# antbern/slamrs

Measured on NVIDIA B200. Metric: particle_beam_updates_per_s, higher is better.
Workload: dtype f32 geometry, f64 weights, u16x2 hit-counter cells

## Files before the change

slamrs_b200/csrc/api.cu:

```cuda
#include "../../include/slamrs_gpu.h"

#include <cuda_runtime.h>
#include <math.h>
#include <stdio.h>
#include <stdlib.h>
#include <string.h>
#include <unistd.h>

#include <algorithm>
#include <new>
#include <string>
#include <vector>

#include "comm.h"
#include "kernels.cuh"

using namespace slamrs;

struct slamrs_gpu_handle {
    slamrs_gpu_config cfg{};
    int device = 0;
    int num_sms = 148;
    cudaStream_t stream = nullptr;
    cudaStream_t side_stream = nullptr;
// ... 288 lines not shown
    if (h->h_scan_stage) cudaFreeHost(h->h_scan_stage);
    h->d_angle = h->d_dist = nullptr; h->d_valid = nullptr; h->h_scan_stage = nullptr; h->beam_cap = 0;
    h->scan_upload_pending = false;
    const uint32_t cap = (n + 255u) & ~255u;
    unsigned char* base = nullptr;
    CU_TRY(h, cudaMalloc(&base, 9u * (size_t)cap));
    h->d_angle = reinterpret_cast<float*>(base);
    h->d_dist = reinterpret_cast<float*>(base + 4u * (size_t)cap);
    h->d_valid = base + 8u * (size_t)cap;
    CU_TRY(h, cudaMallocHost(&h->h_scan_stage, 9u * (size_t)cap));
    if (!h->ev_scan_uploaded) CU_TRY(h, cudaEventCreateWithFlags(&h->ev_scan_uploaded, cudaEventDisableTiming));
    h->beam_cap = cap;
    return SLAMRS_OK;
}

constexpr uint32_t PROF_RING = 64;
constexpr uint32_t PROF_MARKS = SLAMRS_PHASE_COUNT + 1;

int prof_flush(slamrs_gpu_handle* h) {
    if (h->prof_recorded == 0) return SLAMRS_OK;
    CU_TRY(h, cudaStreamSynchronize(h->stream));
    for (uint32_t r = 0; r < h->prof_recorded; ++r) {
        for (int p = 0; p < SLAMRS_PHASE_COUNT; ++p) {
            float ms = 0.f;
            CU_TRY(h, cudaEventElapsedTime(&ms, h->prof_events[r * PROF_MARKS + p], h->prof_events[r * PROF_MARKS + p + 1]));
            h->prof_ms[p] += ms;
        }
    }
    h->prof_steps += h->prof_recorded;
    h->prof_recorded = 0;
    return SLAMRS_OK;
}

#define PROF_MARK(h, m)                                                                                   \
    do {                                                                                                  \
        if ((h)->profiling) CU_TRY(h, cudaEventRecord((h)->prof_events[(h)->prof_recorded * PROF_MARKS + (m)], (h)->stream)); \
    } while (0)

int materialize_copies(slamrs_gpu_handle* h, bool grouped) {
    launch_copy_boxed(h->stream, h->d_mat_items, grouped ? h->d_mat_leaders : nullptr, &h->d_counters->n_mat,
                      &h->d_counters->n_mat_leaders, h->n_local, h->d_jobs, h->geom, h->d_counters, h->num_sms, !grouped);
    launch_commit_boxes(h->stream, h->d_mat_items, &h->d_counters->n_mat, h->n_local, h->geom, true, h->d_counters, nullptr);
    h->launches += 3;
    return SLAMRS_OK;
}
int unshare_all(slamrs_gpu_handle* h) {
    if (!h->defer) return SLAMRS_OK;
    launch_materialize_list(h->stream, nullptr, h->n_total, h->first, h->n_local, h->d_slot[h->cur], h->d_alias, h->d_cells,
                            h->cells_per_grid, h->d_meta, h->d_bands, h->n_bands, h->d_mat_items, h->d_mat_leaders,
                            h->d_mat_roots, h->d_counters);
    h->launches++;
    int rc = materialize_copies(h, true);
    if (rc) return rc;
    CU_TRY(h, cudaStreamSynchronize(h->stream));
    h->counters_fresh = false;
    h->mirror_by_step = false;
    return SLAMRS_OK;
}

int step_barrier(slamrs_gpu_handle* h) {
    if (h->p2p_exchange) {
        launch_peer_barrier(h->stream, h->d_peer_flags, h->d_flags, h->rank, h->world, ++h->barrier_epoch,
                            h->barrier_timeout_ns, h->d_counters);
        h->launches++;
        return SLAMRS_OK;
    }
    std::string err;
    if (comm_barrier(h->comm, h->d_barrier, h->stream, &err)) return fail(h, SLAMRS_E_NCCL, err);
    return SLAMRS_OK;
}

int fetch_counters(slamrs_gpu_handle* h) {
    if (h->counters_fresh) return SLAMRS_OK;
    if (!h->mirror_by_step) {
        launch_publish_counters(h->stream, h->d_counters, h->h_counters);
        h->launches++;
    }
    CU_TRY(h, cudaStreamSynchronize(h->stream));
    CU_TRY(h, cudaGetLastError());
    h->counters_fresh = true;
    return SLAMRS_OK;
}

int loc_step_async(slamrs_gpu_handle* h, const OdomModel& od, bool caller) {
    cudaStream_t s = h->stream;
    if (h->profiling && h->prof_recorded == PROF_RING) {
        int prc = prof_flush(h);
        if (prc) return prc;
    }
    const int cur = h->cur, nxt = cur ^ 1;
    const ScanDevice scan = h->scan_external ? ScanDevice{h->ext_angle, h->ext_dist, h->ext_valid, h->n_beams, nullptr}
                                             : ScanDevice{h->d_angle, h->d_dist, h->d_valid, h->n_beams, nullptr};
    PROF_MARK(h, 0);
    launch_loc_step(s, h->geom, od, scan, h->d_pose[cur], h->d_results, h->n_total, caller ? h->d_z : nullptr, h->cfg.seed,
                    h->step, h->d_loc_terms, h->loc_outside, h->d_carry, h->d_counters);
    PROF_MARK(h, 1);
    PROF_MARK(h, 2);
    launch_weights(s, h->d_results, h->n_total, h->d_wnorm, h->d_cum, h->d_fold, (double)h->cfg.resample_threshold, h->d_counters);
    launch_resample_indices(s, h->d_results, h->d_cum, h->n_total, caller ? h->d_u : nullptr, h->cfg.seed, h->step, h->d_idx,
                            h->d_pose[nxt], 0, h->n_total, false, nullptr,
                            RayLists{nullptr, nullptr, nullptr, nullptr, nullptr, nullptr, 0u, 0u}, h->d_wnorm, h->d_carry,
                            h->d_counters);
    h->launches += 3;
    for (uint32_t m = 3; m < PROF_MARKS; ++m) PROF_MARK(h, m);
    if (h->profiling) h->prof_recorded++;
    CU_TRY(h, cudaGetLastError());
    h->cur = nxt;
    h->step++;
    h->counters_fresh = false;
    h->mirror_by_step = false;
    return SLAMRS_OK;
}

}

namespace {
template <typename T>
struct DevBuf {
    T* p = nullptr;
    cudaError_t alloc(size_t n) { return cudaMalloc(&p, sizeof(T) * (n ? n : 1)); }
    ~DevBuf() { cudaFree(p); }
};
int debug_device(int device) {
    int n = 0;
    if (cudaGetDeviceCount(&n) != cudaSuccess || n == 0) { cudaGetLastError(); return SLAMRS_E_NO_DEVICE; }
    if (device >= n) return SLAMRS_E_INVALID_ARG;
    return SLAMRS_OK;
}
#define DBG_CU(expr)                                                                     \
    do {                                                                                 \
        cudaError_t _e = (expr);                                                         \
        if (_e != cudaSuccess) return fail(nullptr, SLAMRS_E_CUDA, std::string(#expr) + ": " + cudaGetErrorString(_e)); \
    } while (0)
}

extern "C" {

int slamrs_gpu_grid_cells(float extent, float resolution, uint32_t* out_cells) {
    if (!out_cells) return SLAMRS_E_INVALID_ARG;
    const float c = ceilf(extent / resolution);
    if (!(c == c) || c <= 0.0f) { *out_cells = 0; return SLAMRS_OK; }
    if (c >= 4294967296.0f) return SLAMRS_E_INVALID_ARG;
    *out_cells = (uint32_t)c;
    return SLAMRS_OK;
}

int slamrs_gpu_nccl_unique_id(uint8_t out[SLAMRS_NCCL_ID_BYTES]) {
    if (!out) return SLAMRS_E_INVALID_ARG;
    std::string err;
    if (comm_unique_id(out, &err)) return fail(nullptr, SLAMRS_E_NCCL, err);
    return SLAMRS_OK;
}

int slamrs_gpu_create(const slamrs_gpu_config* cfg, slamrs_gpu_handle** out) {
    if (!cfg || !out) return fail(nullptr, SLAMRS_E_INVALID_ARG, "null config or output pointer");
    *out = nullptr;
    if (cfg->struct_size != sizeof(slamrs_gpu_config) || cfg->abi_version != SLAMRS_GPU_ABI_VERSION)
        return fail(nullptr, SLAMRS_E_INVALID_ARG, "slamrs_gpu_config size/ABI version mismatch");
    if (cfg->n_particles == 0)
        return fail(nullptr, SLAMRS_E_INVALID_ARG, "Must have at least one particle");
    if (cfg->world_size > PEER_MAX_WORLD) return fail(nullptr, SLAMRS_E_INVALID_ARG, "world_size above 64");
    if (cfg->world_size > 32u && (cfg->flags & SLAMRS_FLAG_NCCL_EXCHANGE) == 0)
        return fail(nullptr, SLAMRS_E_INVALID_ARG, "world_size above 32 needs SLAMRS_FLAG_NCCL_EXCHANGE (the peer-store exchange serves 32 GPUs)");
    if (cfg->world_size == 0 || cfg->rank >= cfg->world_size || cfg->n_particles % cfg->world_size != 0)
        return fail(nullptr, SLAMRS_E_INVALID_ARG, "bad rank/world_size or n_particles not divisible by world_size");
    if (cfg->n_particles > 0x7fffffffull) return fail(nullptr, SLAMRS_E_INVALID_ARG, "too many particles");
    if (cfg->grid_w == 0 || cfg->grid_w != cfg->grid_h)
        return fail(nullptr, SLAMRS_E_INVALID_ARG,
                    "grid must be square and non-empty (the reference index row*size.y+column aliases otherwise)");
    if ((uint64_t)cfg->grid_w * cfg->grid_h > 0x7fffffffull) return fail(nullptr, SLAMRS_E_INVALID_ARG, "grid too large");
    if (!(cfg->resolution > 0.0f)) return fail(nullptr, SLAMRS_E_INVALID_ARG, "resolution must be positive");
    if (cfg->rng_mode > SLAMRS_RNG_CALLER) return fail(nullptr, SLAMRS_E_INVALID_ARG, "unknown rng_mode");
    if (!(cfg->resample_threshold >= 0.0f && cfg->resample_threshold <= 1.0f))
        return fail(nullptr, SLAMRS_E_INVALID_ARG, "resample_threshold must be 0 (always resample) or in (0, 1]");
    if (cfg->slot_cells != 0 && (cfg->slot_cells < 256u || (cfg->slot_cells & (cfg->slot_cells - 1u)) != 0u))
        return fail(nullptr, SLAMRS_E_INVALID_ARG, "slot_cells must be 0 (whole grid) or a power of two >= 256");

    int n_dev = 0;
    if (cudaGetDeviceCount(&n_dev) != cudaSuccess || n_dev == 0) {
        cudaGetLastError();
        return fail(nullptr, SLAMRS_E_NO_DEVICE, "no CUDA device visible; this library has no CPU fallback");
    }
    int device = cfg->device;
    if (device < 0) cudaGetDevice(&device);
    if (device >= n_dev) return fail(nullptr, SLAMRS_E_INVALID_ARG, "device ordinal out of range");

    slamrs_gpu_handle* h = new (std::nothrow) slamrs_gpu_handle();
    if (!h) return fail(nullptr, SLAMRS_E_OUT_OF_MEMORY, "host allocation failed");
    h->cfg = *cfg;
    h->device = device;
    h->world = cfg->world_size;
    h->rank = cfg->rank;
    h->n_total = (uint32_t)cfg->n_particles;
    h->n_local = h->n_total / h->world;
    h->first = h->rank * h->n_local;
    h->n_cells = cfg->grid_w * cfg->grid_h;
    h->geom = make_map_geom(cfg->pos_x, cfg->pos_y, cfg->resolution, cfg->grid_w, cfg->grid_h, cfg->slot_cells);
    h->cells_per_grid = ((size_t)h->geom.pw * h->geom.ph + 31u) & ~(size_t)31u;

#define CREATE_TRY(expr)                                  \
    do {                                                  \
        int _rc = (expr);                                 \
        if (_rc != SLAMRS_OK) {                           \
            g_create_error = h->last_error;               \
            free_all(h);                                  \
            return _rc;                                   \
        }                                                 \
    } while (0)
#define CREATE_CU(expr)                                                                                   \
    do {                                                                                                  \
        cudaError_t _e = (expr);                                                                          \
        if (_e != cudaSuccess) {                                                                          \
            const int _code = (_e == cudaErrorMemoryAllocation) ? SLAMRS_E_OUT_OF_MEMORY : SLAMRS_E_CUDA; \
            g_create_error = std::string(#expr) + ": " + cudaGetErrorString(_e);                          \
            cudaGetLastError();                                                                           \
            free_all(h);                                                                                  \
            return _code;                                                                                 \
        }                                                                                                 \
    } while (0)

    DeviceGuard guard(device);
    cudaDeviceProp prop;
    CREATE_CU(cudaGetDeviceProperties(&prop, device));
    h->num_sms = prop.multiProcessorCount;
    if (prop.major < 10) {
        g_create_error = "this library is built for sm_100a (B200) only";
        free_all(h);
        return SLAMRS_E_NO_DEVICE;
    }
    CREATE_CU(cudaStreamCreateWithFlags(&h->stream, cudaStreamNonBlocking));
    CREATE_CU(cudaStreamCreateWithFlags(&h->side_stream, cudaStreamNonBlocking));
    CREATE_CU(cudaEventCreateWithFlags(&h->ev_indices, cudaEventDisableTiming));
    CREATE_CU(cudaEventCreateWithFlags(&h->ev_plan, cudaEventDisableTiming));
    CREATE_CU(cudaEventCreateWithFlags(&h->ev_sort, cudaEventDisableTiming));
    CREATE_CU(cudaMalloc(&h->d_order, sizeof(uint16_t) * SORT_MAX_BEAMS));
    CREATE_CU(cudaMalloc(&h->d_valid_list, sizeof(float2) * 65536));
    CREATE_CU(cudaMalloc(&h->d_n_valid, sizeof(uint32_t)));
    CREATE_CU(configure_kernels());

    const size_t grid_bytes = h->cells_per_grid * sizeof(uint32_t);
    if (h->world > 1) {
        uint32_t spare = cfg->spare_slots;
        if (spare == 0) {
            size_t free_b = 0, total_b = 0;
            CREATE_CU(cudaMemGetInfo(&free_b, &total_b));
            const size_t reserve = (size_t)2 << 30;
            const size_t live = (size_t)h->n_local * grid_bytes;
            size_t room = free_b > live + reserve ? (free_b - live - reserve) / grid_bytes : 0;
            spare = (uint32_t)(room < h->n_local ? room : h->n_local);
        }
        h->n_spare = spare;
    }
    h->n_slots = h->n_local + h->n_spare;

    h->off_results = (sizeof(SlotMeta) * 2 * (size_t)h->n_local + 255) & ~(size_t)255;
    h->off_flags = (h->off_results + 2 * sizeof(ParticleResult) * (size_t)h->n_total + 255) & ~(size_t)255;
    h->n_bands = bands_per_slot(h->geom);
    h->off_bands = (h->off_flags + sizeof(unsigned long long) * 2 * PEER_MAX_WORLD + 255) & ~(size_t)255;
    h->off_counters = (h->off_bands + sizeof(uint32_t) * 2 * (size_t)h->n_local * h->n_bands + 255) & ~(size_t)255;
    h->pool_header = (h->off_counters + sizeof(StepCounters) + 4095) & ~(size_t)4095;
    CREATE_CU(cudaMalloc(&h->d_pool, h->pool_header + (size_t)h->n_slots * grid_bytes));
    h->d_meta = (SlotMeta*)h->d_pool;
    h->d_cells = (uint32_t*)((char*)h->d_pool + h->pool_header);
    h->d_results_base = (ParticleResult*)((char*)h->d_pool + h->off_results);
    h->d_results = h->d_results_base;
    h->d_flags = (unsigned long long*)((char*)h->d_pool + h->off_flags);
    h->d_bands = (uint32_t*)((char*)h->d_pool + h->off_bands);
    h->d_counters = (StepCounters*)((char*)h->d_pool + h->off_counters);
    h->peer_counters.assign(h->world, nullptr);
    h->peer_counters[h->rank] = h->d_counters;
    h->p2p_exchange = h->world > 1 && (cfg->flags & SLAMRS_FLAG_NCCL_EXCHANGE) == 0;
    CREATE_CU(cudaMemsetAsync(h->d_pool, 0, h->pool_header + (size_t)h->n_slots * grid_bytes, h->stream));
    h->boxed_copy = (cfg->flags & SLAMRS_FLAG_FULL_GRID_COPY) == 0 && cfg->grid_w % 8u == 0u && h->geom.pw % 8u == 0u;
    h->defer = h->boxed_copy && (cfg->flags & SLAMRS_FLAG_EAGER_COPY) == 0;
    for (int i = 0; i < 2; ++i) {
        CREATE_CU(cudaMalloc(&h->d_slot[i], sizeof(int32_t) * h->n_local));
        CREATE_CU(cudaMalloc(&h->d_pose[i], sizeof(float) * 3 * h->n_local));
        CREATE_CU(cudaMemsetAsync(h->d_pose[i], 0, sizeof(float) * 3 * h->n_local, h->stream));
    }
    CREATE_CU(cudaMalloc(&h->d_wnorm, sizeof(double) * h->n_total));
    CREATE_CU(cudaMalloc(&h->d_cum, sizeof(double) * h->n_total));
    CREATE_CU(cudaMalloc(&h->d_idx, sizeof(uint32_t) * h->n_total));
    CREATE_CU(cudaMalloc(&h->d_fold, sizeof(double) * weights_scratch_doubles()));
    if (cfg->resample_threshold > 0.0f) CREATE_CU(cudaMalloc(&h->d_carry, sizeof(double) * h->n_total));
    CREATE_CU(cudaMemsetAsync(h->d_wnorm, 0, sizeof(double) * h->n_total, h->stream));
    CREATE_CU(cudaMemsetAsync(h->d_idx, 0, sizeof(uint32_t) * h->n_total, h->stream));
    if (cfg->rng_mode == SLAMRS_RNG_CALLER) {
        CREATE_CU(cudaMalloc(&h->d_z, sizeof(double) * 2 * h->n_total));
        CREATE_CU(cudaMalloc(&h->d_u, sizeof(double)));
    }
    CREATE_CU(cudaMalloc(&h->d_keep, sizeof(int32_t) * h->n_local));
    CREATE_CU(cudaMalloc(&h->d_need, sizeof(int32_t) * h->n_local));
    CREATE_CU(cudaMalloc(&h->d_free, sizeof(int32_t) * ((size_t)h->n_local + h->n_spare + 1)));
    CREATE_CU(cudaMalloc(&h->d_spare, sizeof(int32_t) * ((size_t)h->n_spare + 1)));
    CREATE_CU(cudaMalloc(&h->d_copies, sizeof(CopyItem) * h->n_local));
    CREATE_CU(cudaMalloc(&h->d_leaders, sizeof(uint32_t) * h->n_local));
    CREATE_CU(cudaMalloc(&h->d_jobs, copy_job_bytes() * h->n_local));
    CREATE_CU(cudaMalloc(&h->d_alias, sizeof(int32_t) * h->n_slots));
    CREATE_CU(cudaMalloc(&h->d_mat_items, sizeof(CopyItem) * h->n_local));
    CREATE_CU(cudaMalloc(&h->d_mat_leaders, sizeof(uint32_t) * h->n_local));
    CREATE_CU(cudaMalloc(&h->d_mat_roots, sizeof(uint32_t) * h->n_local));
    CREATE_CU(cudaMalloc(&h->d_alive, sizeof(uint32_t) * h->n_local));
    CREATE_CU(cudaMalloc(&h->d_ray_items, sizeof(RayItem) * 2 * (size_t)h->n_local));
    CREATE_CU(cudaMalloc(&h->d_readers, sizeof(uint32_t) * (2 * (size_t)h->n_slots + 2 * (size_t)h->n_local)));
    CREATE_CU(cudaMalloc(&h->d_ray_xchg, ray_half_xchg_bytes() * h->n_local));
    CREATE_CU(cudaMalloc(&h->d_ray_spill, sizeof(uint32_t) * ray_spill_scratch_words(h->num_sms)));
    CREATE_CU(cudaMallocHost(&h->h_counters, sizeof(StepCounters)));
    memset(h->h_counters, 0, sizeof(StepCounters));
    CREATE_CU(cudaMalloc(&h->d_export, sizeof(double) * h->n_cells));
    CREATE_CU(cudaStreamCreateWithFlags(&h->copy_stream, cudaStreamNonBlocking));
    for (int k = 0; k < 2; ++k) {
        CREATE_CU(cudaMalloc(&h->d_export_async[k], sizeof(double) * h->n_cells));
        CREATE_CU(cudaEventCreateWithFlags(&h->ev_exported[k], cudaEventDisableTiming));
        CREATE_CU(cudaEventCreateWithFlags(&h->ev_copied[k], cudaEventDisableTiming));
    }
    CREATE_CU(cudaMalloc(&h->d_term_table, sizeof(double) * LK_TABLE_NF * LK_TABLE_NO));
    launch_fill_term_table(h->stream, h->d_term_table);
    h->launches++;
    CREATE_CU(cudaMalloc(&h->d_history, sizeof(StepRecord) * STEP_HISTORY));
    CREATE_CU(cudaMemsetAsync(h->d_history, 0xff, sizeof(StepRecord) * STEP_HISTORY, h->stream));
    CREATE_CU(cudaMalloc(&h->d_barrier, sizeof(int)));
    CREATE_CU(cudaMemsetAsync(h->d_barrier, 0, sizeof(int), h->stream));
    launch_init_slots(h->stream, h->d_slot[0], h->n_local, h->d_spare, h->n_spare, h->d_counters, h->rank, h->d_meta, h->d_alias);
    h->launches++;
    CREATE_CU(cudaGetLastError());

    if (h->world > 1) {
        std::string err;
        h->comm = comm_create(cfg->nccl_id, (int)h->rank, (int)h->world, &err);
        if (!h->comm) {
            g_create_error = err;
            free_all(h);
            return SLAMRS_E_NCCL;
        }
        CREATE_TRY(setup_peers(h));
        if (const char* ev = getenv("SLAMRS_BARRIER_TIMEOUT_MS")) {
            const long long ms = atoll(ev);
            if (ms > 0) h->barrier_timeout_ns = (unsigned long long)ms * 1000000ull;
        }
        if (comm_barrier(h->comm, h->d_barrier, h->stream, &err)) {
            g_create_error = err;
            free_all(h);
            return SLAMRS_E_NCCL;
        }
    }
    CREATE_CU(cudaStreamSynchronize(h->stream));
    h->h_counters->est_slot = h->rank == 0 ? 0 : -1;
    h->h_counters->n_spare = h->n_spare;
#undef CREATE_TRY
#undef CREATE_CU
    *out = h;
    return SLAMRS_OK;
}

int slamrs_gpu_create_localizer(const slamrs_gpu_config* cfg, const slamrs_gpu_sensor_model* model,
                                const double* map_probability, slamrs_gpu_handle** out) {
    if (!out) return fail(nullptr, SLAMRS_E_INVALID_ARG, "null output pointer");
    *out = nullptr;
    if (!cfg) return fail(nullptr, SLAMRS_E_INVALID_ARG, "null config");
    if (!model) return fail(nullptr, SLAMRS_E_INVALID_ARG, "null sensor model");
    if (!map_probability) return fail(nullptr, SLAMRS_E_INVALID_ARG, "null map_probability");
    if (cfg->struct_size != sizeof(slamrs_gpu_config) || cfg->abi_version != SLAMRS_GPU_ABI_VERSION)
        return fail(nullptr, SLAMRS_E_INVALID_ARG, "slamrs_gpu_config size/ABI version mismatch");
    if (model->struct_size != sizeof(slamrs_gpu_sensor_model))
        return fail(nullptr, SLAMRS_E_INVALID_ARG, "slamrs_gpu_sensor_model struct_size mismatch");
    if (cfg->n_particles == 0) return fail(nullptr, SLAMRS_E_INVALID_ARG, "Must have at least one particle");
    if (cfg->n_particles > 0x7fffffffull) return fail(nullptr, SLAMRS_E_INVALID_ARG, "too many particles");
    if (cfg->world_size != 1 || cfg->rank != 0)
        return fail(nullptr, SLAMRS_E_INVALID_ARG, "world_size must be 1 and rank 0: a localizer runs on one GPU");
    if (cfg->flags != 0) return fail(nullptr, SLAMRS_E_INVALID_ARG, "flags must be 0 for a localizer");
    if (cfg->slot_cells != 0) return fail(nullptr, SLAMRS_E_INVALID_ARG, "slot_cells must be 0 for a localizer");
    if (cfg->spare_slots != 0) return fail(nullptr, SLAMRS_E_INVALID_ARG, "spare_slots must be 0 for a localizer");
    if (cfg->grid_w == 0 || cfg->grid_w != cfg->grid_h)
        return fail(nullptr, SLAMRS_E_INVALID_ARG, "grid_w and grid_h must be equal and non-zero (square grid)");
    if ((uint64_t)cfg->grid_w * cfg->grid_h > 0x7fffffffull) return fail(nullptr, SLAMRS_E_INVALID_ARG, "grid too large");
    if (!(cfg->resolution > 0.0f)) return fail(nullptr, SLAMRS_E_INVALID_ARG, "resolution must be positive");
    if (cfg->rng_mode > SLAMRS_RNG_CALLER) return fail(nullptr, SLAMRS_E_INVALID_ARG, "unknown rng_mode");
    if (!(cfg->resample_threshold >= 0.0f && cfg->resample_threshold <= 1.0f))
        return fail(nullptr, SLAMRS_E_INVALID_ARG, "resample_threshold must be 0 (always resample) or in (0, 1]");
    if (model->kind > SLAMRS_SENSOR_LIKELIHOOD_FIELD) return fail(nullptr, SLAMRS_E_INVALID_ARG, "unknown sensor model kind");
    const bool field = model->kind == SLAMRS_SENSOR_LIKELIHOOD_FIELD;
    if (field) {
        if (!(model->sigma > 0.0f) || !isfinite(model->sigma))
            return fail(nullptr, SLAMRS_E_INVALID_ARG, "sigma must be a positive finite number of metres");
        if (!(model->z_rand > 0.0f && model->z_rand < 1.0f))
            return fail(nullptr, SLAMRS_E_INVALID_ARG, "z_rand must lie in (0, 1)");
        if (!(model->occupied_above >= 0.5f && model->occupied_above < 1.0f))
            return fail(nullptr, SLAMRS_E_INVALID_ARG, "occupied_above must lie in [0.5, 1)");
    }
    const size_t n_cells = (size_t)cfg->grid_w * cfg->grid_h;
    for (size_t i = 0; i < n_cells; ++i)
        if (!(map_probability[i] >= 0.0 && map_probability[i] <= 1.0))
            return fail(nullptr, SLAMRS_E_INVALID_ARG,
                        "map_probability[" + std::to_string(i) + "] is NaN or outside [0, 1]");

    int n_dev = 0;
    if (cudaGetDeviceCount(&n_dev) != cudaSuccess || n_dev == 0) {
        cudaGetLastError();
        return fail(nullptr, SLAMRS_E_NO_DEVICE, "no CUDA device visible; this library has no CPU fallback");
    }
    int device = cfg->device;
    if (device < 0) cudaGetDevice(&device);
    if (device >= n_dev) return fail(nullptr, SLAMRS_E_INVALID_ARG, "device ordinal out of range");

    slamrs_gpu_handle* h = new (std::nothrow) slamrs_gpu_handle();
    if (!h) return fail(nullptr, SLAMRS_E_OUT_OF_MEMORY, "host allocation failed");
    h->cfg = *cfg;
    h->localizer = true;
    h->device = device;
    h->n_total = h->n_local = (uint32_t)cfg->n_particles;
    h->n_cells = (uint32_t)n_cells;
    h->geom = make_map_geom(cfg->pos_x, cfg->pos_y, cfg->resolution, cfg->grid_w, cfg->grid_h);
    h->loc_outside = field ? log((double)model->z_rand) : 0.0;

#define CREATE_CU(expr)                                                                                   \
    do {                                                                                                  \
        cudaError_t _e = (expr);                                                                          \
        if (_e != cudaSuccess) {                                                                          \
            const int _code = (_e == cudaErrorMemoryAllocation) ? SLAMRS_E_OUT_OF_MEMORY : SLAMRS_E_CUDA; \
            g_create_error = std::string(#expr) + ": " + cudaGetErrorString(_e);                          \
            cudaGetLastError();                                                                           \
            cudaFree(scratch);                                                                            \
            free_all(h);                                                                                  \
            return _code;                                                                                 \
        }                                                                                                 \
    } while (0)

    uint32_t* scratch = nullptr;
    DeviceGuard guard(device);
    cudaDeviceProp prop;
    CREATE_CU(cudaGetDeviceProperties(&prop, device));
    h->num_sms = prop.multiProcessorCount;
    if (prop.major < 10) {
        g_create_error = "this library is built for sm_100a (B200) only";
        free_all(h);
        return SLAMRS_E_NO_DEVICE;
    }
    CREATE_CU(cudaStreamCreateWithFlags(&h->stream, cudaStreamNonBlocking));
    CREATE_CU(configure_kernels());
    h->off_counters = (sizeof(ParticleResult) * (size_t)h->n_total + 255) & ~(size_t)255;
    const size_t pool_bytes = h->off_counters + sizeof(StepCounters);
    CREATE_CU(cudaMalloc(&h->d_pool, pool_bytes));
    CREATE_CU(cudaMemsetAsync(h->d_pool, 0, pool_bytes, h->stream));
    h->d_results_base = h->d_results = (ParticleResult*)h->d_pool;
    h->d_counters = (StepCounters*)((char*)h->d_pool + h->off_counters);
    for (int i = 0; i < 2; ++i) {
        CREATE_CU(cudaMalloc(&h->d_pose[i], sizeof(float) * 3 * h->n_total));
        CREATE_CU(cudaMemsetAsync(h->d_pose[i], 0, sizeof(float) * 3 * h->n_total, h->stream));
    }
    CREATE_CU(cudaMalloc(&h->d_wnorm, sizeof(double) * h->n_total));
    CREATE_CU(cudaMalloc(&h->d_cum, sizeof(double) * h->n_total));
    CREATE_CU(cudaMalloc(&h->d_idx, sizeof(uint32_t) * h->n_total));
    CREATE_CU(cudaMalloc(&h->d_fold, sizeof(double) * weights_scratch_doubles()));
    if (cfg->resample_threshold > 0.0f) CREATE_CU(cudaMalloc(&h->d_carry, sizeof(double) * h->n_total));
    CREATE_CU(cudaMemsetAsync(h->d_wnorm, 0, sizeof(double) * h->n_total, h->stream));
    CREATE_CU(cudaMemsetAsync(h->d_idx, 0, sizeof(uint32_t) * h->n_total, h->stream));
    if (cfg->rng_mode == SLAMRS_RNG_CALLER) {
        CREATE_CU(cudaMalloc(&h->d_z, sizeof(double) * 2 * h->n_total));
        CREATE_CU(cudaMalloc(&h->d_u, sizeof(double)));
    }
    CREATE_CU(cudaMallocHost(&h->h_counters, sizeof(StepCounters)));
    memset(h->h_counters, 0, sizeof(StepCounters));
    CREATE_CU(cudaMalloc(&h->d_export, sizeof(double) * n_cells));
    CREATE_CU(cudaMemcpyAsync(h->d_export, map_probability, sizeof(double) * n_cells, cudaMemcpyHostToDevice, h->stream));
    CREATE_CU(cudaMalloc(&h->d_loc_terms, sizeof(double) * n_cells));
    if (field) CREATE_CU(cudaMalloc(&scratch, sizeof(uint32_t) * n_cells));
    CREATE_CU(launch_loc_terms(h->stream, h->d_export, cfg->grid_w, field ? 1 : 0, model->sigma, model->z_rand,
                               model->occupied_above, cfg->resolution, scratch, h->d_loc_terms));
    h->launches += field ? 2 : 1;
    CREATE_CU(cudaStreamSynchronize(h->stream));
    cudaFree(scratch);
#undef CREATE_CU
    *out = h;
    return SLAMRS_OK;
}

int slamrs_gpu_get_sensor_terms(slamrs_gpu_handle* h, double* out_cells) {
    if (!h || !out_cells) return SLAMRS_E_INVALID_ARG;
    if (!h->localizer) return fail(h, SLAMRS_E_INVALID_ARG, "a SLAM handle has no sensor-term table (only a localizer has one)");
    DeviceGuard g(h->device);
    CU_TRY(h, cudaMemcpyAsync(out_cells, h->d_loc_terms, sizeof(double) * h->n_cells, cudaMemcpyDeviceToHost, h->stream));
    CU_TRY(h, cudaStreamSynchronize(h->stream));
    return SLAMRS_OK;
}

int slamrs_gpu_set_scan_match(slamrs_gpu_handle* h, const slamrs_gpu_scan_match* m) {
    if (!h) return SLAMRS_E_INVALID_ARG;
    if (h->localizer) return fail(h, SLAMRS_E_INVALID_ARG, "a localizer does not scan-match");
    if (!m) {
        h->match_on = false;
        return SLAMRS_OK;
    }
    if (m->struct_size != sizeof(slamrs_gpu_scan_match))
        return fail(h, SLAMRS_E_INVALID_ARG, "slamrs_gpu_scan_match struct_size mismatch");
    if (m->radius > 2u) return fail(h, SLAMRS_E_INVALID_ARG, "scan match radius must be 0, 1 or 2 cells");
    if (!(m->step_xy > 0.0f) || !isfinite(m->step_xy))
        return fail(h, SLAMRS_E_INVALID_ARG, "scan match step_xy must be a positive finite number of metres");
    if (!(m->step_theta > 0.0f) || !isfinite(m->step_theta))
        return fail(h, SLAMRS_E_INVALID_ARG, "scan match step_theta must be a positive finite number of radians");
    if (m->levels < 1u || m->levels > 8u) return fail(h, SLAMRS_E_INVALID_ARG, "scan match levels must lie in 1..8");
    if (m->max_moves < 1u || m->max_moves > 1024u)
        return fail(h, SLAMRS_E_INVALID_ARG, "scan match max_moves must lie in 1..1024");
    if (!h->d_match_stats) {
        DeviceGuard g(h->device);
        CU_TRY(h, cudaMalloc(&h->d_match_stats, sizeof(uint2) * h->n_local));
    }
    h->match = ScanMatchParams{m->radius, m->step_xy, m->step_theta, m->levels, m->max_moves};
    h->match_on = true;
    return SLAMRS_OK;
}

int slamrs_gpu_get_scan_match_stats(slamrs_gpu_handle* h, uint64_t out[4]) {
    if (!h || !out) return SLAMRS_E_INVALID_ARG;
    out[0] = out[1] = out[2] = out[3] = 0;
    if (!h->match_last_step) return SLAMRS_OK;
    DeviceGuard g(h->device);
    std::vector<uint2> per(h->n_local);
    CU_TRY(h, cudaMemcpyAsync(per.data(), h->d_match_stats, sizeof(uint2) * h->n_local, cudaMemcpyDeviceToHost, h->stream));
    CU_TRY(h, cudaStreamSynchronize(h->stream));
    for (const uint2& v : per) {
        out[0] += v.x > 0u;
        out[1] += v.x;
        out[2] += v.y;
        out[3] += v.x == h->match_last_max_moves;
    }
    return SLAMRS_OK;
}

void slamrs_gpu_destroy(slamrs_gpu_handle* h) {
    if (h && getenv("SLAMRS_RAY_TRACE_PRINT")) {
        unsigned long long tr[18];
        DeviceGuard g(h->device);
        cudaStreamSynchronize(h->stream);
        if (ray_trace(tr) == 0) {
            fprintf(stderr, "ray trace: items fused %llu in-place %llu; cycles pop %llu setup %llu walk %llu fused_total %llu wait %llu inplace_wb %llu\n",
                    tr[16], tr[17], tr[0], tr[1], tr[2], tr[3], tr[4], tr[5]);
            fprintf(stderr, "ray trace raw:");
            for (int k = 0; k < 18; ++k) fprintf(stderr, " [%d]%llu", k, tr[k]);
            fprintf(stderr, "\n");
        }
    }
    free_all(h);
}

int slamrs_gpu_upload_scan(slamrs_gpu_handle* h, const float* angle, const float* dist, const uint8_t* valid,
                           uint32_t n_beams) {
    if (!h) return SLAMRS_E_INVALID_ARG;
    if (n_beams > 0 && (!angle || !dist || !valid)) return fail(h, SLAMRS_E_INVALID_ARG, "null scan array");
    if (n_beams > 65535u) return fail(h, SLAMRS_E_INVALID_ARG, "at most 65535 beams per scan");
    DeviceGuard g(h->device);
    int rc = ensure_beam_capacity(h, n_beams ? n_beams : 1);
    if (rc) return rc;
    if (n_beams) {
        if (h->scan_upload_pending) CU_TRY(h, cudaEventSynchronize(h->ev_scan_uploaded));
        const size_t cap = h->beam_cap;
        memcpy(h->h_scan_stage, angle, sizeof(float) * n_beams);
        memcpy(h->h_scan_stage + 4u * cap, dist, sizeof(float) * n_beams);
        memcpy(h->h_scan_stage + 8u * cap, valid, n_beams);
        CU_TRY(h, cudaMemcpyAsync(h->d_angle, h->h_scan_stage, 8u * cap + n_beams, cudaMemcpyHostToDevice, h->stream));
        CU_TRY(h, cudaEventRecord(h->ev_scan_uploaded, h->stream));
        h->scan_upload_pending = true;
    }
    h->n_beams = n_beams;
    h->scan_external = false;
    h->order_valid = false;
    float maxd = 0.0f;
    for (uint32_t i = 0; i < n_beams; ++i) {
        const float d = fabsf(dist[i]);
        if (!isfinite(d)) { maxd = INFINITY; break; }
        if (d > maxd) maxd = d;
    }
    const float cells = ceilf(maxd / h->geom.res);
    h->radius_cells = (cells < 4096.0f ? (int)cells : 4096) + 6;
    return SLAMRS_OK;
}

int slamrs_gpu_set_scan_device(slamrs_gpu_handle* h, const float* angle_device, const float* dist_device,
                               const uint8_t* valid_device, uint32_t n_beams, float max_dist) {
    if (!h) return SLAMRS_E_INVALID_ARG;
    if (n_beams > 0 && (!angle_device || !dist_device || !valid_device)) return fail(h, SLAMRS_E_INVALID_ARG, "null scan array");
    if (n_beams > 65535u) return fail(h, SLAMRS_E_INVALID_ARG, "at most 65535 beams per scan");
    h->ext_angle = angle_device; h->ext_dist = dist_device; h->ext_valid = valid_device;
    h->n_beams = n_beams;
    h->scan_external = true;
    h->order_valid = false;
    const float cells = max_dist > 0.0f ? ceilf(max_dist / h->geom.res) : INFINITY;
    h->radius_cells = ((cells == cells && cells < 4096.0f) ? (int)cells : 4096) + 6;
    return SLAMRS_OK;
}

int slamrs_gpu_step_async(slamrs_gpu_handle* h, float dist_left, float dist_right, float wheel_dist,
                          const double* z_draws, const double* resample_u) {
    if (!h) return SLAMRS_E_INVALID_ARG;
    const bool caller = h->cfg.rng_mode == SLAMRS_RNG_CALLER;
    if (caller && (!z_draws || !resample_u))
        return fail(h, SLAMRS_E_INVALID_ARG, "rng_mode CALLER needs z_draws and resample_u");
    DeviceGuard g(h->device);
    cudaStream_t s = h->stream;
    const OdomModel od = odometry_new(dist_left, dist_right, wheel_dist);
    if (caller) {
        CU_TRY(h, cudaMemcpyAsync(h->d_z, z_draws, sizeof(double) * 2 * h->n_total, cudaMemcpyHostToDevice, s));
        CU_TRY(h, cudaMemcpyAsync(h->d_u, resample_u, sizeof(double), cudaMemcpyHostToDevice, s));
    }
    if (h->localizer) return loc_step_async(h, od, caller);
    const bool sorted = h->n_beams > 32u && h->n_beams <= SORT_MAX_BEAMS;
    const ScanDevice scan = h->scan_external
                                ? ScanDevice{h->ext_angle, h->ext_dist, h->ext_valid, h->n_beams, sorted ? h->d_order : nullptr}
                                : ScanDevice{h->d_angle, h->d_dist, h->d_valid, h->n_beams, sorted ? h->d_order : nullptr};
    if (sorted && !h->order_valid) {
        CU_TRY(h, cudaEventRecord(h->ev_indices, s));
        CU_TRY(h, cudaStreamWaitEvent(h->side_stream, h->ev_indices, 0));
        launch_sort_beams(h->side_stream, scan.dist, h->n_beams, h->d_order);
        CU_TRY(h, cudaEventRecord(h->ev_sort, h->side_stream));
        h->launches++;
        h->order_valid = true;
        h->order_pending = true;
    }
    if (h->profiling && h->prof_recorded == PROF_RING) {
        int prc = prof_flush(h);
        if (prc) return prc;
    }
    const int cur = h->cur, nxt = cur ^ 1;
    const size_t grid_bytes = h->cells_per_grid * sizeof(uint32_t);
    const bool all_particles = (h->cfg.flags & SLAMRS_FLAG_UPDATE_ALL_PARTICLES) != 0;
    const uint32_t res_off = (uint32_t)(h->step & 1ull) * h->n_total;
    h->d_results = h->d_results_base + res_off;

    const bool force_generic = (h->cfg.flags & SLAMRS_FLAG_GENERIC_RAY_KERNEL) != 0;
    const bool fuse = h->defer && !all_particles &&
                      ray_update_can_fuse(h->geom, h->n_beams, h->cells_per_grid, force_generic, h->radius_cells);
    const bool half_items = ray_update_can_fuse(h->geom, h->n_beams, h->cells_per_grid, force_generic, h->radius_cells);
    const bool flag_pulls = h->world > 1 && fuse && half_items && h->boxed_copy && h->p2p_exchange;
    const uint32_t pull_epoch = flag_pulls ? (uint32_t)(h->step + 1ull) : 0u;
    const size_t n_zero = half_items ? 2 * (size_t)h->n_slots + 2 * (size_t)h->n_local : 0;
    PROF_MARK(h, 0);
    launch_motion_likelihood(s, h->geom, od, scan, h->d_pose[cur], h->d_slot[cur], h->defer ? h->d_alias : nullptr, h->d_cells, h->d_meta, h->cells_per_grid,
                             h->d_results, h->first, h->n_local, caller ? h->d_z : nullptr, h->cfg.seed, h->step, h->d_term_table, h->d_valid_list, h->d_n_valid,
                             h->d_carry, h->d_counters, h->p2p_exchange ? h->d_peer_results : nullptr, res_off, h->rank, h->world,
                             h->d_readers, (uint32_t)n_zero, h->match_on ? &h->match : nullptr, h->d_match_stats);
    h->launches += h->match_on ? 3 : 2;
    h->match_last_step = h->match_on;
    h->match_last_max_moves = h->match.max_moves;
    PROF_MARK(h, 1);
    if (h->world > 1) {
        if (h->p2p_exchange) {
            int brc = step_barrier(h);
            if (brc) return brc;
        } else {
            std::string err;
            if (comm_all_gather(h->comm, h->d_results + h->first, h->d_results, sizeof(ParticleResult) * h->n_local, s, &err))
                return fail(h, SLAMRS_E_NCCL, err);
        }
    }
    PROF_MARK(h, 2);
    launch_weights(s, h->d_results, h->n_total, h->d_wnorm, h->d_cum, h->d_fold, (double)h->cfg.resample_threshold, h->d_counters);
    RayLists ray{nullptr, nullptr, nullptr, nullptr, nullptr, nullptr, 0u, 0u};
    if (fuse) ray = RayLists{h->d_ray_items, h->d_ray_items + h->n_local, h->d_slot[cur], h->d_alias, h->d_readers, h->d_meta,
                             h->n_local, flag_pulls ? 1u : 0u};
    launch_resample_indices(s, h->d_results, h->d_cum, h->n_total, caller ? h->d_u : nullptr, h->cfg.seed, h->step,
                            h->d_idx, h->d_pose[nxt], h->first, h->n_local, !all_particles, h->d_alive, ray, h->d_wnorm, h->d_carry,
                            h->d_counters);
    if (all_particles) {
        launch_mark_alive(s, h->d_idx, h->n_total, h->first, h->n_local, true, h->d_alive, h->d_counters);
        h->launches++;
    }
    if (h->defer && !fuse) {
        if (all_particles)
            launch_materialize_list(s, nullptr, h->n_total, h->first, h->n_local, h->d_slot[cur], h->d_alias, h->d_cells,
                                    h->cells_per_grid, h->d_meta, h->d_bands, h->n_bands, h->d_mat_items, h->d_mat_leaders,
                                    h->d_mat_roots, h->d_counters);
        else
            launch_materialize_alive(s, h->d_alive, h->n_local, h->d_slot[cur], h->d_alias, h->d_cells, h->cells_per_grid,
                                     h->d_meta, h->d_bands, h->n_bands, h->d_mat_items, h->d_counters);
        h->launches++;
    }
    CU_TRY(h, cudaEventRecord(h->ev_indices, s));
    CU_TRY(h, cudaStreamWaitEvent(h->side_stream, h->ev_indices, 0));
    PlanArgs pa{};
    pa.results = h->d_results;
    pa.idx = h->d_idx;
    pa.n_total = h->n_total; pa.n_local = h->n_local; pa.rank = h->rank; pa.world = h->world;
    pa.slot_old = h->d_slot[cur]; pa.slot_new = h->d_slot[nxt];
    pa.keep = h->d_keep; pa.need = h->d_need; pa.free_list = h->d_free; pa.spare_list = h->d_spare;
    pa.n_spare_cap = h->n_spare;
    pa.copies = h->d_copies; pa.leaders = h->d_leaders;
    pa.cells = h->d_cells; pa.cells_per_grid = h->cells_per_grid;
    pa.peer_cells = h->d_peer_cells;
    pa.meta = h->d_meta; pa.peer_meta = h->d_peer_meta;
    pa.bands = h->d_bands; pa.peer_bands = h->d_peer_bands; pa.n_bands = h->n_bands;
    pa.counters = h->d_counters;
    pa.history = h->d_history;
    pa.step = h->step;
    pa.staged = plan_can_stage(h->n_local, h->n_spare);
    pa.alias_of = h->d_alias; pa.defer = h->defer;
    launch_plan(h->side_stream, pa);
    h->launches += 3;
    if (flag_pulls) {
        launch_pull(h->side_stream, h->d_copies, h->d_leaders, &h->d_counters->n_copies, &h->d_counters->n_leaders,
                    h->n_local, h->geom, h->d_counters, h->num_sms, pull_epoch, h->barrier_timeout_ns, h->d_meta, h->d_readers,
                    h->d_readers + h->n_slots);
        h->launches++;
    }
    CU_TRY(h, cudaEventRecord(h->ev_plan, h->side_stream));
    PROF_MARK(h, 3);
    if (h->defer && !fuse) {
        int mrc = materialize_copies(h, all_particles);
        if (mrc) return mrc;
    }
    PROF_MARK(h, 4);
    if (h->order_pending) {
        CU_TRY(h, cudaStreamWaitEvent(s, h->ev_sort, 0));
        h->order_pending = false;
    }
    CU_TRY(h, launch_ray_update(s, h->geom, scan, h->d_results, h->first, h->n_local, h->d_alive,
                                fuse ? h->d_ray_items : nullptr, fuse ? h->d_ray_items + h->n_local : nullptr,
                                fuse ? h->d_readers : nullptr,
                                fuse ? h->d_readers + h->n_slots : nullptr, h->d_readers + 2 * (size_t)h->n_slots, h->d_ray_xchg,
                                h->d_ray_spill, h->d_slot[cur],
                                h->d_cells, h->d_meta, h->d_bands, h->cells_per_grid, h->radius_cells, h->d_counters, &h->window_cells,
                                force_generic, h->num_sms, h->d_readers + 2 * (size_t)h->n_slots + h->n_local, pull_epoch));
    h->launches++;
    PROF_MARK(h, 5);
    CU_TRY(h, cudaStreamWaitEvent(s, h->ev_plan, 0));
    if (h->world > 1 && !flag_pulls) {
        int brc = step_barrier(h);
        if (brc) return brc;
    }
    PROF_MARK(h, 6);
    if ((h->defer && h->world == 1) || flag_pulls) {
    } else if (h->boxed_copy) {
        launch_copy_boxed(s, h->d_copies, h->d_leaders, &h->d_counters->n_copies, &h->d_counters->n_leaders, h->n_local,
                          h->d_jobs, h->geom, h->d_counters, h->num_sms, h->defer);
        h->launches++;
    } else {
        launch_copy(s, h->d_copies, h->d_leaders, &h->d_counters->n_copies, &h->d_counters->n_leaders, h->cells_per_grid,
                    h->num_sms);
        launch_account_full_copy(s, &h->d_counters->n_copies, &h->d_counters->n_leaders, grid_bytes, h->d_counters);
        h->launches++;
    }
    if (!((h->defer && h->world == 1) || flag_pulls)) h->launches++;
    PROF_MARK(h, 7);
    launch_commit_boxes(s, h->d_copies, &h->d_counters->n_copies, (h->defer && h->world == 1) ? 1u : h->n_local, h->geom,
                        h->boxed_copy, h->d_counters, h->d_history + (h->step % STEP_HISTORY),
                        h->mirror_wanted ? h->h_counters : nullptr);
    h->launches++;
    if (h->profiling) h->prof_recorded++;
    CU_TRY(h, cudaGetLastError());
    h->cur = nxt;
    h->step++;
    h->counters_fresh = false;
    h->mirror_by_step = h->mirror_wanted;
    h->est_box_stale = false;
    return SLAMRS_OK;
}

int slamrs_gpu_sync(slamrs_gpu_handle* h) {
    if (!h) return SLAMRS_E_INVALID_ARG;
    DeviceGuard g(h->device);
    int rc = fetch_counters(h);
    if (rc) return rc;
    if (h->h_counters->barrier_timeout)
        return fail(h, SLAMRS_E_INTERNAL,
                    h->h_counters->barrier_timeout == 2ull
                        ? "a peer GPU's handle was destroyed (its step failed or its owner left); this handle can only be destroyed"
                        : "a peer GPU did not reach the step barrier within the time limit");
    if (h->h_counters->fuse_overflow)
        return fail(h, SLAMRS_E_INTERNAL, "fused ray update: more window-bypassing hits than its scratch holds");
    if (h->h_counters->window_overflow)
        return fail(h, SLAMRS_E_WINDOW,
                    "a particle's informed extent outgrew its windowed grid slot; raise slot_cells (the scan was not "
                    "integrated into that grid)");
    if (h->h_counters->staging_short)
        return fail(h, SLAMRS_E_STAGING,
                    "cross-GPU migration needed more free grid slots than available; raise spare_slots");
    return SLAMRS_OK;
}

int slamrs_gpu_update(slamrs_gpu_handle* h, const float* angle, const float* dist, const uint8_t* valid,
                      uint32_t n_beams, float dist_left, float dist_right, float wheel_dist, const double* z_draws,
                      const double* resample_u) {
    int rc = slamrs_gpu_upload_scan(h, angle, dist, valid, n_beams);
    if (rc) return rc;
    h->mirror_wanted = true;
    rc = slamrs_gpu_step_async(h, dist_left, dist_right, wheel_dist, z_draws, resample_u);
    h->mirror_wanted = false;
    if (rc) return rc;
    return slamrs_gpu_sync(h);
}

int slamrs_gpu_pose(slamrs_gpu_handle* h, float out_xyt[3]) {
    if (!h || !out_xyt) return SLAMRS_E_INVALID_ARG;
    DeviceGuard g(h->device);
    int rc = fetch_counters(h);
    if (rc) return rc;
    out_xyt[0] = h->h_counters->est_pose[0];
    out_xyt[1] = h->h_counters->est_pose[1];
    out_xyt[2] = h->h_counters->est_pose[2];
    return SLAMRS_OK;
}

namespace {
int export_window(slamrs_gpu_handle* h, uint32_t format, int x0, int y0, int x1, int y1, void* out, bool pipelined = false) {
    if (format > SLAMRS_MAP_U8) return fail(h, SLAMRS_E_INVALID_ARG, "unknown map format");
    if (x0 < 0 || y0 < 0 || x1 > (int)h->geom.gw || y1 > (int)h->geom.gh || x1 < x0 || y1 < y0)
        return fail(h, SLAMRS_E_INVALID_ARG, "map window outside the grid");
    const size_t n = (size_t)(x1 - x0) * (size_t)(y1 - y0);
    if (n == 0 && h->world == 1) return SLAMRS_OK;
    const size_t bytes = n * (format == SLAMRS_MAP_F64 ? 8u : (format == SLAMRS_MAP_F32 ? 4u : 1u));
    cudaStream_t s = h->stream;
    if (h->world > 1) {
        int rc = fetch_counters(h);
        if (rc) return rc;
        rc = step_barrier(h);
        if (rc) return rc;
        if (out == nullptr) return SLAMRS_OK;
    }
    double* dst = h->d_export;
    int k = 0;
    if (pipelined) {
        k = h->async_next;
        h->async_next ^= 1;
        if (h->async_pending[k]) CU_TRY(h, cudaStreamWaitEvent(s, h->ev_copied[k], 0));
        dst = h->d_export_async[k];
    }
    if (h->world > 1) {
        const uint32_t owner = (uint32_t)h->h_counters->est_owner;
        launch_export(s, h->host_peer_cells[owner], h->host_peer_meta[owner], h->cells_per_grid, h->peer_counters[owner], h->geom,
                      x0, y0, x1, y1, (int)format, dst);
    } else {
        launch_export(s, h->d_cells, h->d_meta, h->cells_per_grid, h->d_counters, h->geom, x0, y0, x1, y1, (int)format, dst);
    }
    h->launches++;
    if (pipelined) {
        CU_TRY(h, cudaEventRecord(h->ev_exported[k], s));
        CU_TRY(h, cudaStreamWaitEvent(h->copy_stream, h->ev_exported[k], 0));
        CU_TRY(h, cudaMemcpyAsync(out, dst, bytes, cudaMemcpyDeviceToHost, h->copy_stream));
        CU_TRY(h, cudaEventRecord(h->ev_copied[k], h->copy_stream));
        h->async_pending[k] = true;
        return SLAMRS_OK;
    }
    CU_TRY(h, cudaMemcpyAsync(out, h->d_export, bytes, cudaMemcpyDeviceToHost, s));
    CU_TRY(h, cudaStreamSynchronize(s));
    CU_TRY(h, cudaGetLastError());
    return SLAMRS_OK;
}
}

int slamrs_gpu_map_probability(slamrs_gpu_handle* h, double* out_cells) {
    if (!h || (!out_cells && h->world == 1)) return SLAMRS_E_INVALID_ARG;
    if (h->localizer) return fail(h, SLAMRS_E_INVALID_ARG, NO_GRIDS);
    DeviceGuard g(h->device);
    return export_window(h, SLAMRS_MAP_F64, 0, 0, (int)h->geom.gw, (int)h->geom.gh, out_cells);
}

int slamrs_gpu_map_probability_async(slamrs_gpu_handle* h, double* out_cells) {
    if (!h || (!out_cells && h->world == 1)) return SLAMRS_E_INVALID_ARG;
    if (h->localizer) return fail(h, SLAMRS_E_INVALID_ARG, NO_GRIDS);
    DeviceGuard g(h->device);
    return export_window(h, SLAMRS_MAP_F64, 0, 0, (int)h->geom.gw, (int)h->geom.gh, out_cells, true);
}

int slamrs_gpu_map_wait(slamrs_gpu_handle* h) {
    if (!h) return SLAMRS_E_INVALID_ARG;
    DeviceGuard g(h->device);
    for (int k = 0; k < 2; ++k) {
        if (!h->async_pending[k]) continue;
        CU_TRY(h, cudaEventSynchronize(h->ev_copied[k]));
        h->async_pending[k] = false;
    }
    CU_TRY(h, cudaGetLastError());
    return SLAMRS_OK;
}

int slamrs_gpu_map_extent(slamrs_gpu_handle* h, int32_t out_x0y0x1y1[4]) {
    if (!h || !out_x0y0x1y1) return SLAMRS_E_INVALID_ARG;
    if (h->localizer) return fail(h, SLAMRS_E_INVALID_ARG, NO_GRIDS);
    DeviceGuard g(h->device);
    if (h->world == 1 && h->step > 0 && !h->est_box_stale) {
        int rc = fetch_counters(h);
        if (rc) return rc;
        for (int i = 0; i < 4; ++i) out_x0y0x1y1[i] = h->h_counters->est_box[i];
        return SLAMRS_OK;
    }
    cudaStream_t s = h->stream;
    int* d4 = reinterpret_cast<int*>(h->d_export);
    if (h->world > 1) {
        int rc = fetch_counters(h);
        if (rc) return rc;
        rc = step_barrier(h);
        if (rc) return rc;
        const uint32_t owner = (uint32_t)h->h_counters->est_owner;
        launch_estimate_extent(s, h->host_peer_meta[owner], h->peer_counters[owner], d4);
    } else {
        launch_estimate_extent(s, h->d_meta, h->d_counters, d4);
    }
    h->launches++;
    CU_TRY(h, cudaMemcpyAsync(out_x0y0x1y1, d4, 4 * sizeof(int), cudaMemcpyDeviceToHost, s));
    CU_TRY(h, cudaStreamSynchronize(s));
    return SLAMRS_OK;
}

int slamrs_gpu_map_window(slamrs_gpu_handle* h, uint32_t format, int32_t x0, int32_t y0, int32_t x1, int32_t y1,
                          void* out) {
    if (!h || (!out && h->world == 1)) return SLAMRS_E_INVALID_ARG;
    if (h->localizer) return fail(h, SLAMRS_E_INVALID_ARG, NO_GRIDS);
    DeviceGuard g(h->device);
    return export_window(h, format, x0, y0, x1, y1, out);
}

int slamrs_gpu_effective_particles(slamrs_gpu_handle* h, double* out) {
    if (!h || !out) return SLAMRS_E_INVALID_ARG;
    DeviceGuard g(h->device);
    int rc = fetch_counters(h);
    if (rc) return rc;
    *out = h->step == 0 ? (double)h->n_total : h->h_counters->n_eff;
    return SLAMRS_OK;
}

int slamrs_gpu_sim_scan(slamrs_gpu_handle* h, const float* segments_xyxy, uint32_t n_segments, const float pose_xyt[3],
                        uint32_t n_beams, float scanner_range, uint32_t* out_n) {
    if (!h || !pose_xyt || (n_segments && !segments_xyxy)) return SLAMRS_E_INVALID_ARG;
    if (n_beams > 65535u) return fail(h, SLAMRS_E_INVALID_ARG, "at most 65535 beams per scan");
    DeviceGuard g(h->device);
    int rc = ensure_beam_capacity(h, n_beams ? n_beams : 1);
    if (rc) return rc;
    cudaStream_t s = h->stream;
    float* d_seg = reinterpret_cast<float*>(h->d_export);
    if ((size_t)n_segments * 16u + 16u > sizeof(double) * (size_t)h->n_cells)
        return fail(h, SLAMRS_E_INVALID_ARG, "too many scene segments for the scratch buffer");
    uint32_t* d_cnt = reinterpret_cast<uint32_t*>(d_seg + 4 * (size_t)n_segments);
    if (n_segments)
        CU_TRY(h, cudaMemcpyAsync(d_seg, segments_xyxy, 16 * (size_t)n_segments, cudaMemcpyHostToDevice, s));
    CU_TRY(h, cudaMemsetAsync(d_cnt, 0, 2 * sizeof(uint32_t), s));
    launch_sim_scan(s, d_seg, n_segments, pose_xyt[0], pose_xyt[1], pose_xyt[2], n_beams, scanner_range, h->d_angle,
                    h->d_dist, h->d_valid, d_cnt);
    h->launches++;
    uint32_t res[2] = {0, 0};
    CU_TRY(h, cudaMemcpyAsync(res, d_cnt, sizeof(res), cudaMemcpyDeviceToHost, s));
    CU_TRY(h, cudaStreamSynchronize(s));
    CU_TRY(h, cudaGetLastError());
    h->n_beams = res[0];
    h->scan_external = false;
    h->order_valid = false;
    float maxd;
    memcpy(&maxd, &res[1], 4);
    const float cells = ceilf(maxd / h->geom.res);
    h->radius_cells = ((cells == cells && cells < 4096.0f) ? (int)cells : 4096) + 6;
    if (out_n) *out_n = res[0];
    return SLAMRS_OK;
}

int slamrs_gpu_get_scan(slamrs_gpu_handle* h, float* out_angle, float* out_dist, uint8_t* out_valid, uint32_t cap,
                        uint32_t* out_n) {
    if (!h || !out_n) return SLAMRS_E_INVALID_ARG;
    if (h->scan_external) return fail(h, SLAMRS_E_INVALID_ARG, "the current scan lives in caller-owned device memory");
    DeviceGuard g(h->device);
    *out_n = h->n_beams;
    const uint32_t n = h->n_beams < cap ? h->n_beams : cap;
    if (n && out_angle) CU_TRY(h, cudaMemcpyAsync(out_angle, h->d_angle, sizeof(float) * n, cudaMemcpyDeviceToHost, h->stream));
    if (n && out_dist) CU_TRY(h, cudaMemcpyAsync(out_dist, h->d_dist, sizeof(float) * n, cudaMemcpyDeviceToHost, h->stream));
    if (n && out_valid) CU_TRY(h, cudaMemcpyAsync(out_valid, h->d_valid, n, cudaMemcpyDeviceToHost, h->stream));
    CU_TRY(h, cudaStreamSynchronize(h->stream));
    return SLAMRS_OK;
}

const char* slamrs_gpu_last_error(const slamrs_gpu_handle* h) { return h ? h->last_error.c_str() : g_create_error.c_str(); }

int slamrs_gpu_get_stats(slamrs_gpu_handle* h, slamrs_gpu_stats* out) {
    if (!h || !out) return SLAMRS_E_INVALID_ARG;
    DeviceGuard g(h->device);
    int rc = fetch_counters(h);
    if (rc) return rc;
    const StepCounters& c = *h->h_counters;
    out->step = h->step;
    out->grids_copied = c.n_copies + c.n_mat;
    out->grids_pulled = c.n_pulls;
    out->distinct_sources = c.distinct;
    out->resample_clamped = c.clamped;
    out->counter_saturated = c.saturated;
    out->spilled_cells = c.spilled;
    out->window_cells = h->window_cells;
    out->particles_integrated = c.n_alive;
    out->bytes_per_grid = h->localizer ? 0 : h->cells_per_grid * sizeof(uint32_t);
    out->window_overflow = c.window_overflow;
    out->copy_bytes = c.copy_bytes;
    out->resample_exact_fallback = c.fold_fallback;
    out->resample_fold_rounds = c.fold_rounds;
    out->resampled = h->step == 0 ? 0 : c.do_resample;
    return SLAMRS_OK;
}

int slamrs_gpu_set_profiling(slamrs_gpu_handle* h, int enabled) {
    if (!h) return SLAMRS_E_INVALID_ARG;
    DeviceGuard g(h->device);
    if (enabled && h->prof_events.empty()) {
        h->prof_events.resize((size_t)PROF_RING * PROF_MARKS);
        for (auto& e : h->prof_events) CU_TRY(h, cudaEventCreate(&e));
    }
    if (!enabled) {
        int rc = prof_flush(h);
        if (rc) return rc;
    }
    h->profiling = enabled != 0;
    return SLAMRS_OK;
}

int slamrs_gpu_get_phase_ms(slamrs_gpu_handle* h, double out_ms[SLAMRS_PHASE_COUNT], uint64_t* out_steps) {
    if (!h || !out_ms || !out_steps) return SLAMRS_E_INVALID_ARG;
    DeviceGuard g(h->device);
    int rc = prof_flush(h);
    if (rc) return rc;
    for (int p = 0; p < SLAMRS_PHASE_COUNT; ++p) { out_ms[p] = h->prof_ms[p]; h->prof_ms[p] = 0.0; }
    *out_steps = h->prof_steps;
    h->prof_steps = 0;
    return SLAMRS_OK;
}

int slamrs_gpu_get_step_history(slamrs_gpu_handle* h, uint64_t first_step, uint32_t count, uint64_t* out_triples) {
    if (!h || !out_triples || count > STEP_HISTORY) return SLAMRS_E_INVALID_ARG;
    if (h->localizer) return fail(h, SLAMRS_E_INVALID_ARG, NO_GRIDS);
    DeviceGuard g(h->device);
    std::vector<StepRecord> ring(STEP_HISTORY);
    CU_TRY(h, cudaMemcpyAsync(ring.data(), h->d_history, sizeof(StepRecord) * STEP_HISTORY, cudaMemcpyDeviceToHost, h->stream));
// ... 324 lines not shown
```

slamrs_b200/csrc/kernels.cuh:

```cuda
#pragma once
#include <cuda_runtime.h>
#include <stdint.h>
#include "slam_device.cuh"

namespace slamrs {

struct alignas(8) ParticleResult {
    double weight;
    float x, y, theta;
    int32_t slot;
};
static_assert(sizeof(ParticleResult) == 24, "ParticleResult is exchanged between GPUs as 24 bytes");

struct StepCounters {
    unsigned long long max_particle;
    unsigned long long n_copies;
    unsigned long long n_leaders;
    unsigned long long n_pulls;
    unsigned long long distinct;
    unsigned long long clamped;
    unsigned long long saturated;
    unsigned long long spilled;
    unsigned long long staging_short;
    long long est_slot;
    unsigned long long est_owner;
    unsigned long long n_spare;
    unsigned long long n_alive;
    unsigned long long copy_bytes;
    unsigned long long copy_max_rows;
    unsigned long long barrier_timeout;
    unsigned long long window_overflow;
    unsigned long long est_meta_ptr;
    unsigned long long n_mat;
    unsigned long long n_mat_leaders;
    unsigned long long ray_cell_steps;
    unsigned long long ray_copy_bytes;
    unsigned long long ray_work_head;
    unsigned long long ray_items_front;
    unsigned long long ray_items_back;
    unsigned long long ray_items_front_local;
    unsigned long long ray_items_back_local;
    unsigned long long fuse_overflow;
    unsigned long long do_resample;
    unsigned long long carry_active;
    unsigned long long fold_rounds;
    unsigned long long fold_heads;
    unsigned long long fold_fallback;
    int est_box[4];
    double sum;
    double n_eff;
    float est_pose[3];
    float pad;
};

struct StepRecord {
    unsigned long long step, n_copies, n_pulls, distinct, n_leaders, n_alive, copy_bytes, ray_cell_steps, ray_copy_bytes;
};
constexpr uint32_t STEP_HISTORY = 256;
constexpr uint32_t COPY_FAN = 16;

struct ScanDevice {
    const float* angle;
    const float* dist;
    const uint8_t* valid;
    uint32_t n_beams;
    const uint16_t* order;
};
constexpr uint32_t SORT_MAX_BEAMS = 2048;
void launch_sort_beams(cudaStream_t stream, const float* dist, uint32_t n_beams, uint16_t* order);

struct alignas(32) SlotMeta {
    int x0, y0, x1, y1;
    int pad0, pad1, pad2, pad3;
};
static_assert(sizeof(SlotMeta) == 32, "SlotMeta is read by peers as 32 bytes");

struct CopyItem {
    const uint32_t* src;
    uint32_t* dst;
    const SlotMeta* src_meta;
    SlotMeta* dst_meta;
    const uint32_t* src_bands;
    uint32_t* dst_bands;
};

struct RayItem {
    uint32_t particle;
    int32_t slot, root;
    int32_t old_y0, old_y1;
    uint32_t pad;
};
struct RayLists {
    RayItem* clones;
    RayItem* owners;
    const int32_t* slot_of;
    int32_t* alias_of;
    uint32_t* readers;
    SlotMeta* meta;
    uint32_t n_local;
    uint32_t mark_remote;
};
__device__ __forceinline__ RayItem ray_item_at(const RayItem* __restrict__ clones, const RayItem* __restrict__ owners,
                                               uint32_t n_local, const StepCounters* counters, unsigned long long k) {
    const unsigned long long n_rc = counters->ray_items_front, n_lc = counters->ray_items_front_local;
    if (k < n_rc) return clones[k];
    k -= n_rc;
    if (k < n_lc) return clones[n_local - 1u - k];
    k -= n_lc;
    const unsigned long long n_ro = counters->ray_items_back;
    if (k < n_ro) return owners[k];
    return owners[n_local - 1u - (k - n_ro)];
}
struct ScanMatchParams {
    uint32_t radius;
    float step_xy, step_theta;
    uint32_t levels, max_moves;
};
void launch_motion_likelihood(cudaStream_t stream, MapGeom geom, OdomModel od, ScanDevice scan,
                              const float* pose_cur, const int32_t* slot_of, const int32_t* alias_of ,
                              const uint32_t* cells,
                              const SlotMeta* meta, size_t cells_per_grid, ParticleResult* results, uint32_t first_particle,
                              uint32_t n_local, const double* z_draws, uint64_t seed, uint64_t step,
                              const double* term_table ,
                              float2* valid_beams , uint32_t* n_valid ,
                              const double* carry ,
                              const StepCounters* counters,
                              ParticleResult* const* peer_results ,
                              uint32_t peer_offset , uint32_t rank,
                              uint32_t world, uint32_t* zero_words ,
                              uint32_t n_zero, const ScanMatchParams* match ,
                              uint2* match_stats );
void launch_fill_term_table(cudaStream_t stream, double* table);
void launch_scan_match(cudaStream_t stream, MapGeom geom, ScanMatchParams mp, OdomModel od, const float* pose_cur,
                       const int32_t* alias_of , const uint32_t* cells, const SlotMeta* meta,
                       size_t cells_per_grid, ParticleResult* results, uint32_t first_particle, uint32_t n_local,
                       const float2* valid_beams, const uint32_t* n_valid,
                       uint2* stats );
constexpr uint32_t PEER_MAX_WORLD = 64;
void launch_peer_barrier(cudaStream_t stream, unsigned long long* const* peer_flags, unsigned long long* my_flags,
                         uint32_t rank, uint32_t world, unsigned long long epoch, unsigned long long timeout_ns,
                         StepCounters* counters);
void launch_peer_goodbye(cudaStream_t stream, unsigned long long* const* peer_flags, unsigned long long* my_flags,
                         uint32_t rank, uint32_t world, unsigned long long timeout_ns, StepCounters* counters);

bool ray_update_can_fuse(const MapGeom& geom, uint32_t n_beams, size_t cells_per_grid, bool force_generic, int radius_cells);
size_t ray_spill_scratch_words(int num_sms);
size_t ray_half_xchg_bytes();
int ray_trace(unsigned long long* out18);
cudaError_t launch_ray_update(cudaStream_t stream, MapGeom geom, ScanDevice scan, const ParticleResult* results,
                              uint32_t first_particle, uint32_t n_local, const uint32_t* alive_list,
                              const RayItem* clones, const RayItem* owners, const uint32_t* readers, uint32_t* done,
                              uint32_t* xflag , void* xchg ,
                              uint32_t* spill_scratch,
                              const int32_t* slot_of, uint32_t* cells, SlotMeta* meta, uint32_t* bands,
                              size_t cells_per_grid, int radius_cells, StepCounters* counters,
                              uint64_t* window_cells, bool force_generic, int num_sms,
                              uint32_t* xdone ,

                              uint32_t signal_epoch );

struct WeightsShape { uint32_t cluster, threads, chunk; bool regs; };
WeightsShape weights_shape(uint32_t n_total);
void launch_weights(cudaStream_t stream, const ParticleResult* results, uint32_t n_total, double* w_norm,
                    double* cum, double* fold_scratch, double resample_tau, StepCounters* counters);
size_t weights_scratch_doubles();
int weights_trace(long long* out64);

void launch_resample_indices(cudaStream_t stream, const ParticleResult* results, const double* cum,
                             uint32_t n_total, const double* u01_caller, uint64_t seed, uint64_t step,
                             uint32_t* idx, float* pose_next, uint32_t first_particle, uint32_t n_local,
                             bool build_alive ,
                             uint32_t* alive_list, RayLists ray, const double* w_norm, double* carry ,
                             StepCounters* counters);

struct PlanArgs {
    const ParticleResult* results;
    const uint32_t* idx;
    uint32_t n_total, n_local, rank, world;
    const int32_t* slot_old;
    int32_t* slot_new;
    int32_t* keep;
    int32_t* need;
    int32_t* free_list;
    int32_t* spare_list;
    uint32_t n_spare_cap;
    CopyItem* copies;
    uint32_t* leaders;
    uint32_t* cells;
    size_t cells_per_grid;
    uint32_t* const* peer_cells;
    SlotMeta* meta;
    SlotMeta* const* peer_meta;
    uint32_t* bands;
    uint32_t* const* peer_bands;
    uint32_t n_bands;
    StepCounters* counters;
    StepRecord* history;
    unsigned long long step;
    bool staged;
    int32_t* alias_of;
    bool defer;
};
void launch_plan(cudaStream_t stream, const PlanArgs& a);
void launch_materialize_list(cudaStream_t stream, const uint32_t* idx, uint32_t n_total, uint32_t first_particle,
                             uint32_t n_local, const int32_t* slot_of, int32_t* alias_of, uint32_t* cells,
                             size_t cells_per_grid, SlotMeta* meta, uint32_t* bands, uint32_t n_bands, CopyItem* items,
                             uint32_t* leaders, uint32_t* roots_scratch , StepCounters* counters);
bool plan_can_stage(uint32_t n_local, uint32_t n_spare_cap);

void launch_materialize_alive(cudaStream_t stream, const uint32_t* alive_list, uint32_t n_local, const int32_t* slot_of,
                              int32_t* alias_of, uint32_t* cells, size_t cells_per_grid, SlotMeta* meta, uint32_t* bands,
                              uint32_t n_bands, CopyItem* items, StepCounters* counters);

void launch_mark_alive(cudaStream_t stream, const uint32_t* idx, uint32_t n_total, uint32_t first_particle,
                       uint32_t n_local, bool all_particles, uint32_t* alive_list, StepCounters* counters);

void launch_copy(cudaStream_t stream, const CopyItem* items, const uint32_t* leaders,
                 const unsigned long long* n_items, const unsigned long long* n_leaders, size_t cells_per_grid,
                 int num_sms);

void launch_export(cudaStream_t stream, const uint32_t* cells, const SlotMeta* meta, size_t cells_per_grid,
                   const StepCounters* counters, MapGeom geom, int x0, int y0, int x1, int y1, int format, void* out);
void launch_estimate_extent(cudaStream_t stream, const SlotMeta* meta, const StepCounters* counters, int* out4);
void launch_publish_counters(cudaStream_t stream, const StepCounters* counters, StepCounters* host_mirror);
void launch_export_slot(cudaStream_t stream, const uint32_t* grid, const SlotMeta* slot_meta, MapGeom geom,
                        bool as_log_odds, void* out);

void launch_import_slot(cudaStream_t stream, const uint32_t* image, uint32_t* grid, SlotMeta m, MapGeom geom);
void launch_init_slots(cudaStream_t stream, int32_t* slot_of, uint32_t n_local, int32_t* spare_list, uint32_t n_spare,
                       StepCounters* counters, uint32_t rank, SlotMeta* meta, int32_t* alias_of);

void launch_copy_boxed(cudaStream_t stream, const CopyItem* items, const uint32_t* leaders,
                       const unsigned long long* n_items, const unsigned long long* n_leaders, uint32_t max_items,
                       void* jobs , MapGeom geom,
                       StepCounters* counters, int num_sms, bool short_list = false ,
                       uint32_t wait_epoch = 0 ,
                       unsigned long long timeout_ns = 0);
size_t copy_job_bytes();
void launch_pull(cudaStream_t stream, const CopyItem* items, const uint32_t* leaders, const unsigned long long* n_items,
                 const unsigned long long* n_leaders, uint32_t max_items, MapGeom geom, StepCounters* counters, int num_sms,
                 uint32_t wait_epoch, unsigned long long timeout_ns, const SlotMeta* meta_base ,
                 const uint32_t* readers, const uint32_t* done );
void launch_commit_boxes(cudaStream_t stream, const CopyItem* items, const unsigned long long* n_items, uint32_t max_items,
                         MapGeom geom, bool realign, StepCounters* counters, StepRecord* record,
                         StepCounters* host_mirror = nullptr );
void launch_account_full_copy(cudaStream_t stream, const unsigned long long* n_items, const unsigned long long* n_leaders,
                              size_t bytes_per_grid, StepCounters* counters);
void launch_init_uniform(cudaStream_t stream, uint64_t seed, uint32_t first_particle, uint32_t n_local, float x0, float y0,
                         float x1, float y1, float* pose);
void launch_sim_scan(cudaStream_t stream, const float* segments, uint32_t n_seg, float px, float py, float ptheta,
                     uint32_t n_beams, float scanner_range, float* angle, float* dist, uint8_t* valid,
                     uint32_t* out_count_maxbits);
cudaError_t configure_kernels();

cudaError_t launch_loc_terms(cudaStream_t stream, const double* prob, uint32_t w, int field, float sigma, float z_rand,
                             float occupied_above, float res, uint32_t* scratch, double* terms);
void launch_loc_step(cudaStream_t stream, MapGeom geom, OdomModel od, ScanDevice scan, const float* pose_cur,
                     ParticleResult* results, uint32_t n, const double* z_draws, uint64_t seed, uint64_t step,
                     const double* terms, double outside, const double* carry ,
                     const StepCounters* counters);

void launch_debug_raycast(cudaStream_t stream, const float* x0, const float* y0, const float* x1, const float* y1,
                          uint32_t n_rays, uint32_t gw, uint32_t gh, uint32_t extra, int32_t* out_xy, uint32_t cap,
                          uint32_t* out_count);
void launch_debug_sincos(cudaStream_t stream, const float* x, uint32_t n, float* s, float* c);
void launch_debug_stream(cudaStream_t stream, uint64_t seed, uint64_t step, uint64_t first, uint64_t count, double* z,
                         double* u);

}
```

slamrs_b200/csrc/kernels_ray.cu:

```cuda
#include "kernels_common.cuh"
#include <cstdio>
#include <cstdlib>
#include <string>
#include <vector>

namespace slamrs {


constexpr int RAY_MAX_SMEM = 220 * 1024;

__device__ __forceinline__ void global_cell_add(uint32_t* addr, uint32_t inc, bool* saturated) {
    uint32_t old = *addr;
    for (;;) {
        const uint32_t nv = cell_sat_add(old, inc, saturated);
        if (nv == old) return;
        const uint32_t seen = atomicCAS(addr, old, nv);
        if (seen == old) return;
        old = seen;
    }
}

constexpr int RAY_MAX_THREADS = 512;

__device__ __forceinline__ void ext_init(int* s_ext) {
    if (threadIdx.x == 0) { s_ext[0] = 0x7fffffff; s_ext[1] = 0x7fffffff; s_ext[2] = -1; s_ext[3] = -1; }
}
__device__ __forceinline__ void ext_add(int* s_ext, int xmin, int ymin, int xmax, int ymax) {
    if (xmax < xmin) return;
    atomicMin(&s_ext[0], xmin); atomicMin(&s_ext[1], ymin);
    atomicMax(&s_ext[2], xmax); atomicMax(&s_ext[3], ymax);
}
constexpr int BOX_ALIGN = 8;
__device__ __forceinline__ bool window_would_overflow(const MapGeom& geom, const SlotMeta* meta, int cx0, int cy0, int reach) {
    if (!geom.windowed) return false;
    const SlotMeta m = *meta;
    int x0 = max(0, cx0 - reach) & ~7, x1 = min((int)geom.gw, (min((int)geom.gw, cx0 + reach + 1) + 7) & ~7);
    int y0 = max(0, cy0 - reach), y1 = min((int)geom.gh, cy0 + reach + 1);
    if (m.x1 > m.x0 && m.y1 > m.y0) { x0 = min(x0, m.x0); x1 = max(x1, m.x1); y0 = min(y0, m.y0); y1 = max(y1, m.y1); }
    return (uint32_t)(x1 - x0) > geom.pw || (uint32_t)(y1 - y0) > geom.ph;
}

__device__ __forceinline__ void ext_commit(const int* s_ext, SlotMeta* meta, int gw) {
    if (s_ext[2] < s_ext[0]) return;
    SlotMeta b = *meta;
    const int am = BOX_ALIGN - 1;
    const int x0 = s_ext[0] & ~am, x1 = min(gw, (s_ext[2] + 1 + am) & ~am), y0 = s_ext[1], y1 = s_ext[3] + 1;
    if (b.x1 <= b.x0) { b.x0 = x0; b.y0 = y0; b.x1 = x1; b.y1 = y1; }
    else { b.x0 = min(b.x0, x0); b.y0 = min(b.y0, y0); b.x1 = max(b.x1, x1); b.y1 = max(b.y1, y1); }
    *meta = b;
}
constexpr int RAY_MAX_BANDS = (2 * 150 + 1) / BAND_ROWS + 2;
__device__ __forceinline__ void band_init(int* s_blo, int* s_bhi) {
    for (int i = threadIdx.x; i < RAY_MAX_BANDS; i += blockDim.x) { s_blo[i] = 0x7fffffff; s_bhi[i] = -1; }
}
__device__ __forceinline__ void band_add(int* s_blo, int* s_bhi, int band0, int y, int xlo, int xhi) {
    const int lb = y / BAND_ROWS - band0;
    if ((unsigned)lb < (unsigned)RAY_MAX_BANDS) { atomicMin(&s_blo[lb], xlo); atomicMax(&s_bhi[lb], xhi); }
}
__device__ __forceinline__ void band_commit(const int* s_blo, const int* s_bhi, int band0, uint32_t* bands,
                                            const MapGeom& geom) {
    for (int lb = threadIdx.x; lb < RAY_MAX_BANDS; lb += blockDim.x) {
        if (s_bhi[lb] < s_blo[lb]) continue;
        const uint32_t y = (uint32_t)(band0 + lb) * BAND_ROWS;
        if (y >= geom.gh) continue;
        uint32_t* e = &bands[phys_band(geom, y)];
        const uint32_t old = *e;
        uint32_t x0 = (uint32_t)s_blo[lb] & ~7u, x1 = min(geom.gw, ((uint32_t)s_bhi[lb] + 8u) & ~7u);
        if (old != 0u) { x0 = min(x0, old & 0xffffu); x1 = max(x1, old >> 16); }
        *e = x0 | (x1 << 16);
    }
}
__device__ __forceinline__ void band_add_global(uint32_t* bands, const MapGeom& geom, int band0, int x, int y) {
    const int lb = y / BAND_ROWS - band0;
    if ((unsigned)lb < (unsigned)RAY_MAX_BANDS) return;
    uint32_t* e = &bands[phys_band(geom, (uint32_t)y)];
    const uint32_t x0n = (uint32_t)x & ~7u, x1n = min(geom.gw, ((uint32_t)x + 8u) & ~7u);
    uint32_t old = *e;
    for (;;) {
        const uint32_t x0 = old ? min(x0n, old & 0xffffu) : x0n, x1 = old ? max(x1n, old >> 16) : x1n;
        const uint32_t nv = x0 | (x1 << 16);
        if (nv == old) return;
        const uint32_t seen = atomicCAS(e, old, nv);
        if (seen == old) return;
        old = seen;
    }
}

constexpr int RAY_MAX_RADIUS = 150;
constexpr int RAY_MAX_ROWS = 2 * RAY_MAX_RADIUS + 1;
constexpr int RAY_WB_BATCH = 6;

__host__ __device__ inline int isqrt_small(int v) {
    int r = (int)sqrtf((float)v);
    while (r * r > v) r--;
    while ((r + 1) * (r + 1) <= v) r++;
    return r;
}

__host__ __device__ inline int ray_window_cells_upper_bound(int radius, bool vec) {
    int total = 0;
    for (int dy = -radius; dy <= radius; ++dy) total += 2 * isqrt_small(radius * radius - dy * dy) + 1 + (vec ? 6 : 0);
    return total;
}

struct ZeroLengthHits {
    uint32_t free_hits = 0u, occ_hits = 0u;
    __device__ __forceinline__ void tally(const RayClassifier& cls, float acc) {
        const uint32_t inc = classify_cell(cls, acc);
        free_hits += inc == CELL_FREE_INC ? 3u : 0u;
        occ_hits += inc == CELL_OCC_INC ? 3u : 0u;
    }
    template <class ExactAdd>
    __device__ __forceinline__ uint32_t flush(int cx0, int cy0, ExactAdd& exact_add, int* s_ext, int* s_blo, int* s_bhi,
                                              int band0) const {
        if (free_hits + occ_hits == 0u) return 0u;
        for (uint32_t k = 0; k < free_hits; ++k) exact_add(cx0, cy0, CELL_FREE_INC);
        for (uint32_t k = 0; k < occ_hits; ++k) exact_add(cx0, cy0, CELL_OCC_INC);
        ext_add(s_ext, cx0, cy0, cx0, cy0);
        band_add(s_blo, s_bhi, band0, cy0, cx0, cx0);
        return free_hits + occ_hits;
    }
};

template <bool kVector>
__global__ void __launch_bounds__(RAY_MAX_THREADS)
k_ray_update(MapGeom geom, ScanDevice scan, const ParticleResult* __restrict__ results, uint32_t first_particle,
             const uint32_t* __restrict__ alive_list,
             const int32_t* __restrict__ slot_of, uint32_t* __restrict__ cells, SlotMeta* __restrict__ meta,
             uint32_t* __restrict__ bands_all, size_t cells_per_grid, int radius, int reach, StepCounters* counters) {
    extern __shared__ __align__(16) uint32_t s_win[];
    __shared__ int s_blo[RAY_MAX_BANDS], s_bhi[RAY_MAX_BANDS];
    __shared__ int s_row_off[RAY_MAX_ROWS + 1];
    __shared__ int s_row_x[RAY_MAX_ROWS];
    __shared__ int s_ext[4];
    if ((unsigned long long)blockIdx.x >= counters->n_alive) return;
    const uint32_t p = alive_list[blockIdx.x];
    ext_init(s_ext);
    const ParticleResult r = results[first_particle + p];
    const float px = r.x, py = r.y, ptheta = r.theta;
    uint32_t* grid = cells + (size_t)slot_of[p] * cells_per_grid;

    const float sx = world_to_grid(px, geom.pos_x, geom.res);
    const float sy = world_to_grid(py, geom.pos_y, geom.res);
    const long long lcx = f32_as_isize(floorf(sx)), lcy = f32_as_isize(floorf(sy));
    if (lcx < 0 || lcx >= (long long)geom.gw || lcy < 0 || lcy >= (long long)geom.gh) return;
    const int cx = (int)lcx, cy = (int)lcy;
    if (window_would_overflow(geom, &meta[slot_of[p]], cx, cy, reach)) {
        if (threadIdx.x == 0) atomicAdd(&counters->window_overflow, 1ull);
        return;
    }
    uint32_t* bands = bands_all + (size_t)slot_of[p] * bands_per_slot(geom);
    band_init(s_blo, s_bhi);

    const int wy0 = max(0, cy - radius), wy1 = min((int)geom.gh, cy + radius + 1);
    const int band0 = wy0 / BAND_ROWS;
    const int wh = wy1 - wy0;
    for (int ly = threadIdx.x; ly < wh; ly += blockDim.x) {
        const int dy = wy0 + ly - cy;
        const int hw = isqrt_small(radius * radius - dy * dy);
        int x0 = max(0, cx - hw), x1 = min((int)geom.gw, cx + hw + 1);
        if (kVector) {
            x0 &= ~3;
            x1 = min((int)geom.gw, (x1 + 3) & ~3);
        }
        s_row_x[ly] = x0 | ((x1 - x0) << 16);
    }
    __syncthreads();
    if (threadIdx.x < 32) {
        int carry = 0;
        for (int base = 0; base < wh; base += 32) {
            const int ly = base + (int)threadIdx.x;
            const int w = ly < wh ? (s_row_x[ly] >> 16) : 0;
            int inc = w;
#pragma unroll
            for (int o = 1; o < 32; o <<= 1) {
                const int t = __shfl_up_sync(0xffffffffu, inc, o);
                if ((int)threadIdx.x >= o) inc += t;
            }
            if (ly < wh) s_row_off[ly] = carry + inc - w;
            carry += __shfl_sync(0xffffffffu, inc, 31);
        }
        if (threadIdx.x == 0) s_row_off[wh] = carry;
    }
    __syncthreads();
    const int wcells = s_row_off[wh];

    if (kVector) {
        uint4* w4 = reinterpret_cast<uint4*>(s_win);
        for (int i = threadIdx.x; i < (wcells >> 2); i += blockDim.x) w4[i] = make_uint4(0u, 0u, 0u, 0u);
    } else {
        for (int i = threadIdx.x; i < wcells; i += blockDim.x) s_win[i] = 0u;
    }
    __syncthreads();

    bool saturated = false;
    uint32_t spilled = 0;
    ZeroLengthHits zero_length;
    for (uint32_t t = threadIdx.x; t < scan.n_beams; t += blockDim.x) {
        const uint32_t b = scan.order ? scan.order[t] : t;
        const float dist = scan.dist[b];
        float ex, ey;
        beam_endpoint(px, py, ptheta, scan.angle[b], dist, &ex, &ey);
        const float gx = world_to_grid(ex, geom.pos_x, geom.res);
        const float gy = world_to_grid(ey, geom.pos_y, geom.res);
        const RayClassifier cls = make_ray_classifier(__fdiv_rn(dist, geom.res), scan.valid[b] != 0);
        if (fabsf(__fsub_rn(gx, sx)) == 0.0f && fabsf(__fsub_rn(gy, sy)) == 0.0f) {
            const float dxs = __fsub_rn(sx, __fadd_rn((float)cx, 0.5f)), dys = __fsub_rn(sy, __fadd_rn((float)cy, 0.5f));
            zero_length.tally(cls, __fadd_rn(__fmul_rn(dxs, dxs), __fmul_rn(dys, dys)));
            continue;
        }
        ray_walk_acc(sx, sy, gx, gy, geom.gw, geom.gh, 2u, [&](int x, int y, float acc) {
            const uint32_t inc = classify_cell(cls, acc);
            if (inc != 0u) {
                const int ly = y - wy0;
                bool in_window = false;
                if ((unsigned)ly < (unsigned)wh) {
                    const int rx = s_row_x[ly];
                    const int lx = x - (rx & 0xffff);
                    if ((unsigned)lx < (unsigned)(rx >> 16)) {
                        atomicAdd(&s_win[s_row_off[ly] + lx], inc);
                        in_window = true;
                    }
                }
                if (!in_window) {
                    global_cell_add(&grid[phys_index(geom, (uint32_t)x, (uint32_t)y)], inc, &saturated);
                    ext_add(s_ext, x, y, x, y);
                    band_add(s_blo, s_bhi, band0, y, x, x);
                    band_add_global(bands, geom, band0, x, y);
                    spilled++;
                }
            }
        });
    }
    {
        auto exact_add = [&](int x, int y, uint32_t inc) {
            global_cell_add(&grid[phys_index(geom, (uint32_t)x, (uint32_t)y)], inc, &saturated);
        };
        spilled += zero_length.flush(cx, cy, exact_add, s_ext, s_blo, s_bhi, band0);
    }
    __syncthreads();

    int exmin = 0x7fffffff, eymin = 0x7fffffff, exmax = -1, eymax = -1;
    if (kVector) {
        const int total4 = wcells >> 2;
        const uint4* win4 = reinterpret_cast<const uint4*>(s_win);
        for (int base = threadIdx.x; base < total4; base += blockDim.x * RAY_WB_BATCH) {
            uint4 d[RAY_WB_BATCH], v[RAY_WB_BATCH];
            uint4* gp[RAY_WB_BATCH];
            bool nz[RAY_WB_BATCH];
#pragma unroll
            for (int j = 0; j < RAY_WB_BATCH; ++j) {
                const int i = base + j * (int)blockDim.x;
                nz[j] = false;
                if (i < total4) {
                    d[j] = win4[i];
                    nz[j] = (d[j].x | d[j].y | d[j].z | d[j].w) != 0u;
                    if (nz[j]) {
                        int lo = 0, hi = wh;
                        while (hi - lo > 1) {
                            const int mid = (lo + hi) >> 1;
                            if (s_row_off[mid] <= 4 * i) lo = mid; else hi = mid;
                        }
                        const int lx = 4 * i - s_row_off[lo];
                        const int gx0 = (s_row_x[lo] & 0xffff) + lx;
                        exmin = min(exmin, gx0); exmax = max(exmax, gx0 + 3);
                        eymin = min(eymin, wy0 + lo); eymax = max(eymax, wy0 + lo);
                        band_add(s_blo, s_bhi, band0, wy0 + lo, gx0, gx0 + 3);
                        gp[j] = reinterpret_cast<uint4*>(grid + phys_index(geom, (uint32_t)gx0, (uint32_t)(wy0 + lo)));
                    }
                }
            }
#pragma unroll
            for (int j = 0; j < RAY_WB_BATCH; ++j)
                if (nz[j]) v[j] = *gp[j];
#pragma unroll
            for (int j = 0; j < RAY_WB_BATCH; ++j) {
                if (nz[j]) {
                    v[j].x = cell_sat_add(v[j].x, d[j].x, &saturated);
                    v[j].y = cell_sat_add(v[j].y, d[j].y, &saturated);
                    v[j].z = cell_sat_add(v[j].z, d[j].z, &saturated);
                    v[j].w = cell_sat_add(v[j].w, d[j].w, &saturated);
                    *gp[j] = v[j];
                }
            }
        }
    } else {
        for (int ly = threadIdx.x >> 5; ly < wh; ly += blockDim.x >> 5) {
            const int rx = s_row_x[ly], x0 = rx & 0xffff, w = rx >> 16, off = s_row_off[ly];
            for (int c = threadIdx.x & 31; c < w; c += 32) {
                const uint32_t d = s_win[off + c];
                if (d != 0u) {
                    uint32_t* g = grid + phys_index(geom, (uint32_t)(x0 + c), (uint32_t)(wy0 + ly));
                    *g = cell_sat_add(*g, d, &saturated);
                    exmin = min(exmin, x0 + c); exmax = max(exmax, x0 + c);
                    eymin = min(eymin, wy0 + ly); eymax = max(eymax, wy0 + ly);
                    band_add(s_blo, s_bhi, band0, wy0 + ly, x0 + c, x0 + c);
                }
            }
        }
    }
    ext_add(s_ext, exmin, eymin, exmax, eymax);
    __syncthreads();
    band_commit(s_blo, s_bhi, band0, bands, geom);
// ... 212 lines not shown
                        error = __fadd_rn(error, delta_y);
                        cxf = __fadd_rn(cxf, x_step);
                        dxs = __fsub_rn(sx, cxf);
                        dx2 = __fmul_rn(dxs, dxs);
                        x2 += x_inc2;
                    }
                    remaining -= 1;
                }
            }
            continue;
        }

        int x = cx0, y = cy0;
        int ly = y - wy0;
        int2 row = s_row[ly];
        int lx = x - (row.y & 0xffff);
        int row_w = row.y >> 16;
        bool inside = true;
        while (remaining > 0 && inside) {
            const float acc = __fadd_rn(dx2, dy2);
            const bool is_free = acc < cls.free_below;
            const bool is_mid = !is_free && !(acc > cls.prior_above) && (cls.mid_inc != 0u);
            if (is_free | is_mid) {
                const bool in_win = (unsigned)lx < (unsigned)row_w;
                const int cell = row.x + lx;
                const uint32_t addr = win_base + ((uint32_t)(cell >> 1) << 2);
                const uint32_t shift = (cell & 1) << 4;
                if (is_free & in_win) {
                    asm volatile("red.shared.add.u32 [%0], %1;" ::"r"(addr), "r"(1u << shift) : "memory");
                } else {
                    bool done_here = false;
                    if (in_win) {
                        uint32_t* wp = &s_win[cell >> 1];
                        uint32_t old = *wp;
                        for (;;) {
                            if (((old >> (shift + PK_FREE_BITS)) & PK_OCC_MAX) == PK_OCC_MAX) break;
                            const uint32_t seen = atomicCAS(wp, old, old + (1u << (shift + PK_FREE_BITS)));
                            if (seen == old) { done_here = true; break; }
                            old = seen;
                        }
                    }
                    if (!done_here) {
                        exact_add(x, y, is_free ? CELL_FREE_INC : CELL_OCC_INC);
                        ext_add(s_ext, x, y, x, y);
                        band_add(s_blo, s_bhi, band0, y, x, x);
                        if constexpr (!kParkBypass) band_add_global(bands, geom, band0, x, y);
                        spilled++;
                    }
                }
            }
            if (error > 0.0f) {
                y += y_inc;
                error = __fsub_rn(error, delta_x);
                cyf = __fadd_rn(cyf, y_step);
                dys = __fsub_rn(sy, cyf);
                dy2 = __fmul_rn(dys, dys);
                inside = (unsigned)y < (unsigned)gh;
                ly += y_inc;
                if ((unsigned)ly < (unsigned)wh) {
                    row = s_row[ly];
                    row_w = row.y >> 16;
                    lx = x - (row.y & 0xffff);
                } else {
                    row_w = 0;
                }
            } else {
                x += x_inc;
                error = __fadd_rn(error, delta_y);
                cxf = __fadd_rn(cxf, x_step);
                dxs = __fsub_rn(sx, cxf);
                dx2 = __fmul_rn(dxs, dxs);
                inside = (unsigned)x < (unsigned)gw;
                lx += x_inc;
            }
            remaining -= 1;
        }
        cell_steps -= (uint32_t)remaining;
    }
    spilled += zero_length.flush(cx0, cy0, exact_add, s_ext, s_blo, s_bhi, band0);
    if (saturated) *saturated_p = true;
    *spilled_p += spilled;
    *cell_steps_p += cell_steps;
}

__device__ __forceinline__ uint32_t unpack_window_cell(uint32_t packed16) {
    return (packed16 & PK_FREE_MASK) | ((packed16 >> PK_FREE_BITS) << 16);
}
__device__ __forceinline__ void merge_window_group(uint4& va, uint4& vb, const uint4& d, bool* saturated) {
    const uint32_t high_any = (va.x | va.y | va.z | va.w | vb.x | vb.y | vb.z | vb.w) & 0x80008000u;
    if (high_any == 0u) {
        va.x += unpack_window_cell(d.x & 0xffffu); va.y += unpack_window_cell(d.x >> 16);
        va.z += unpack_window_cell(d.y & 0xffffu); va.w += unpack_window_cell(d.y >> 16);
        vb.x += unpack_window_cell(d.z & 0xffffu); vb.y += unpack_window_cell(d.z >> 16);
        vb.z += unpack_window_cell(d.w & 0xffffu); vb.w += unpack_window_cell(d.w >> 16);
    } else {
        va.x = cell_sat_add(va.x, unpack_window_cell(d.x & 0xffffu), saturated); va.y = cell_sat_add(va.y, unpack_window_cell(d.x >> 16), saturated);
        va.z = cell_sat_add(va.z, unpack_window_cell(d.y & 0xffffu), saturated); va.w = cell_sat_add(va.w, unpack_window_cell(d.y >> 16), saturated);
        vb.x = cell_sat_add(vb.x, unpack_window_cell(d.z & 0xffffu), saturated); vb.y = cell_sat_add(vb.y, unpack_window_cell(d.z >> 16), saturated);
        vb.z = cell_sat_add(vb.z, unpack_window_cell(d.w & 0xffffu), saturated); vb.w = cell_sat_add(vb.w, unpack_window_cell(d.w >> 16), saturated);
    }
}

__global__ void __maxnreg__(80)
k_ray_update_packed(MapGeom geom, ScanDevice scan, const ParticleResult* __restrict__ results, uint32_t first_particle,
                    const uint32_t* __restrict__ alive_list, const int32_t* __restrict__ slot_of, uint32_t* __restrict__ cells,
                    SlotMeta* __restrict__ meta, uint32_t* __restrict__ bands_all, size_t cells_per_grid, int radius, int reach,
                    StepCounters* counters) {
    extern __shared__ __align__(16) uint32_t s_win[];
    __shared__ int s_blo[RAY_MAX_BANDS], s_bhi[RAY_MAX_BANDS];
    __shared__ int2 s_row[RAY_MAX_ROWS + 1];
    __shared__ uint32_t s_rowb[RAY_MAX_ROWS];
    __shared__ int s_ext[4];
    __shared__ unsigned long long s_next;
    const unsigned long long n_items = counters->n_alive;
    const int gw = (int)geom.gw, gh = (int)geom.gh;
    const uint32_t win_base = (uint32_t)__cvta_generic_to_shared(s_win);
    const int lane = threadIdx.x & 31, warp = threadIdx.x >> 5, n_warps = blockDim.x >> 5;
    const uint32_t n_bands_slot = bands_per_slot(geom);
    bool saturated = false;
    uint32_t spilled = 0;
    uint32_t cell_steps = 0;

#ifdef SLAMRS_RAY_TRACE
    long long t_prev = clock64();
#endif
    for (;;) {
        __syncthreads();
        RAY_STAMP(0);
        if (threadIdx.x == 0) s_next = atomicAdd(&counters->ray_work_head, 1ull);
        __syncthreads();
        const unsigned long long item = s_next;
        if (item >= n_items) break;
        const uint32_t p = alive_list[item];
        const int32_t slot = slot_of[p];
        uint32_t* grid = cells + (size_t)slot * cells_per_grid;
        ext_init(s_ext);
        const ParticleResult r = results[first_particle + p];
        const float px = r.x, py = r.y, ptheta = r.theta;

        const float sx = world_to_grid(px, geom.pos_x, geom.res);
        const float sy = world_to_grid(py, geom.pos_y, geom.res);
        const long long lcx = f32_as_isize(floorf(sx)), lcy = f32_as_isize(floorf(sy));
        const bool start_inside = !(lcx < 0 || lcx >= (long long)geom.gw || lcy < 0 || lcy >= (long long)geom.gh);
        if (!start_inside) continue;
        const int cx0 = (int)lcx, cy0 = (int)lcy;
        if (window_would_overflow(geom, &meta[slot], cx0, cy0, reach)) {
            if (threadIdx.x == 0) atomicAdd(&counters->window_overflow, 1ull);
            continue;
        }
        uint32_t* bands = bands_all + (size_t)slot * n_bands_slot;
        band_init(s_blo, s_bhi);

        const int wy0 = max(0, cy0 - radius), wy1 = min(gh, cy0 + radius + 1);
        const int band0 = wy0 / BAND_ROWS;
        const int wh = wy1 - wy0;
        for (int ly = threadIdx.x; ly < wh; ly += blockDim.x) {
            const int dy = wy0 + ly - cy0;
            const int hw = isqrt_small(radius * radius - dy * dy);
            const int x0 = max(0, cx0 - hw) & ~7;
            const int x1 = min(gw, (min(gw, cx0 + hw + 1) + 7) & ~7);
            s_row[ly].y = x0 | ((x1 - x0) << 16);
        }
        __syncthreads();
        if (threadIdx.x < 32) {
            int carry = 0;
            for (int base = 0; base < wh; base += 32) {
                const int ly = base + (int)threadIdx.x;
                const int w = ly < wh ? (s_row[ly].y >> 16) : 0;
                int inc = w;
#pragma unroll
                for (int o = 1; o < 32; o <<= 1) {
                    const int t = __shfl_up_sync(0xffffffffu, inc, o);
                    if ((int)threadIdx.x >= o) inc += t;
                }
                if (ly < wh) {
                    const int first = carry + inc - w;
                    s_row[ly].x = first;
                    s_rowb[ly] = win_base + 2u * (uint32_t)(first - (s_row[ly].y & 0xffff));
                }
                carry += __shfl_sync(0xffffffffu, inc, 31);
            }
            if (threadIdx.x == 0) s_row[wh] = make_int2(carry, 0);
        }
        __syncthreads();
        const int wcells = s_row[wh].x;
        {
            uint4* w4 = reinterpret_cast<uint4*>(s_win);
            for (int i = threadIdx.x; i < (wcells >> 3); i += blockDim.x) w4[i] = make_uint4(0u, 0u, 0u, 0u);
        }
        __syncthreads();

        RAY_STAMP(1);
        const bool disc_in_grid = cx0 - radius >= 0 && cx0 + radius < gw && cy0 - radius >= 0 && cy0 + radius < gh;
        ray_walk_packed<false>(geom, scan, scan.order, scan.n_beams, px, py, ptheta, sx, sy, cx0, cy0, radius, disc_in_grid, wy0,
                               wh, band0, s_win, s_row, s_rowb, s_blo, s_bhi, s_ext, grid, bands, nullptr, nullptr, &saturated,
                               &spilled, &cell_steps);
        __syncthreads();
        RAY_STAMP(2);

        const uint4* win4 = reinterpret_cast<const uint4*>(s_win);
        constexpr int RAY_WB_ROWS = 2;
        int exmin = 0x7fffffff, eymin = 0x7fffffff, exmax = -1, eymax = -1;
        for (int ly0 = warp; ly0 < wh; ly0 += n_warps * RAY_WB_ROWS) {
            uint4 d[RAY_WB_ROWS], va[RAY_WB_ROWS], vb[RAY_WB_ROWS];
            uint4* gp[RAY_WB_ROWS];
            bool nz[RAY_WB_ROWS];
#pragma unroll
            for (int j = 0; j < RAY_WB_ROWS; ++j) {
                const int ly = ly0 + j * n_warps;
                nz[j] = false;
                if (ly < wh) {
                    const int2 row = s_row[ly];
                    if (lane < (row.y >> 19)) {
                        d[j] = win4[(row.x >> 3) + lane];
                        nz[j] = (d[j].x | d[j].y | d[j].z | d[j].w) != 0u;
                        if (nz[j]) {
                            const int gx0 = (row.y & 0xffff) + 8 * lane;
                            exmin = min(exmin, gx0); exmax = max(exmax, gx0 + 7);
                            eymin = min(eymin, wy0 + ly); eymax = max(eymax, wy0 + ly);
                            gp[j] = reinterpret_cast<uint4*>(grid + phys_index(geom, (uint32_t)gx0, (uint32_t)(wy0 + ly)));
                        }
                    }
                }
            }
#pragma unroll
            for (int j = 0; j < RAY_WB_ROWS; ++j)
                if (nz[j]) ld_group_v8(gp[j], va[j], vb[j]);
#pragma unroll
            for (int j = 0; j < RAY_WB_ROWS; ++j) {
                const unsigned mnz = __ballot_sync(0xffffffffu, nz[j]);
                const int ly = ly0 + j * n_warps;
                if (mnz != 0u && lane == 0) {
                    const int rx0 = s_row[ly].y & 0xffff;
                    band_add(s_blo, s_bhi, band0, wy0 + ly, rx0 + 8 * (__ffs(mnz) - 1), rx0 + 8 * (31 - __clz(mnz)) + 7);
                }
            }
#pragma unroll
            for (int j = 0; j < RAY_WB_ROWS; ++j) {
                if (nz[j]) {
                    merge_window_group(va[j], vb[j], d[j], &saturated);
                    st_group_v8(gp[j], va[j], vb[j]);
                }
            }
        }
        for (int ly = threadIdx.x; ly < wh; ly += blockDim.x) {
            const int2 row = s_row[ly];
            for (int g = 32; g < (row.y >> 19); ++g) {
                const uint4 dd = win4[(row.x >> 3) + g];
                if ((dd.x | dd.y | dd.z | dd.w) == 0u) continue;
                const int gx0 = (row.y & 0xffff) + 8 * g;
                exmin = min(exmin, gx0); exmax = max(exmax, gx0 + 7);
                eymin = min(eymin, wy0 + ly); eymax = max(eymax, wy0 + ly);
                band_add(s_blo, s_bhi, band0, wy0 + ly, gx0, gx0 + 7);
                uint4* gpt = reinterpret_cast<uint4*>(grid + phys_index(geom, (uint32_t)gx0, (uint32_t)(wy0 + ly)));
                uint4 ta = gpt[0], tb = gpt[1];
                merge_window_group(ta, tb, dd, &saturated);
                gpt[0] = ta;
                gpt[1] = tb;
            }
        }
        ext_add(s_ext, exmin, eymin, exmax, eymax);
        __syncthreads();
        band_commit(s_blo, s_bhi, band0, bands, geom);
        if (threadIdx.x == 0) ext_commit(s_ext, &meta[slot], (int)geom.gw);
        RAY_STAMP(5);
#ifdef SLAMRS_RAY_TRACE
        if (threadIdx.x == 0) atomicAdd(&g_ray_trace_items[1], 1ull);
#endif
    }
    if (saturated) atomicAdd(&counters->saturated, 1ull);
    if (spilled) atomicAdd(&counters->spilled, (unsigned long long)spilled);
#pragma unroll
    for (int o = 16; o > 0; o >>= 1) cell_steps += __shfl_down_sync(0xffffffffu, cell_steps, o);
    if ((threadIdx.x & 31) == 0 && cell_steps) atomicAdd(&counters->ray_cell_steps, (unsigned long long)cell_steps);
}

constexpr int HALF_MAX_ROWS = RAY_MAX_RADIUS + 1;
constexpr int HALF_MAX_BANDS = HALF_MAX_ROWS / BAND_ROWS + 2;
constexpr uint32_t HALF_XCHG_GROUPS = 36;
constexpr uint32_t HALF_XCHG_HITS = 60;
struct alignas(16) HalfXchg {
    uint4 row[HALF_XCHG_GROUPS];
    int band_lo, band_hi;
    uint32_t n_hits;
    uint32_t pad;
    int ext[4];
    uint32_t hits[HALF_XCHG_HITS];
};
static_assert(sizeof(HalfXchg) % 16 == 0, "exchange records are accessed as 16-byte pieces");

__host__ __device__ inline int ray_window_cells_upper_bound_half(int radius) {
    int worst = 0;
    for (int a = 0; a < 8; ++a) {
        int total = 0;
        for (int dy = 0; dy <= radius; ++dy) {
            const int hw = isqrt_small(radius * radius - dy * dy), cx = 4096 + a;
            total += ((cx + hw + 1 + 7) & ~7) - ((cx - hw) & ~7);
        }
        worst = total > worst ? total : worst;
    }
    return worst;
}

__device__ __noinline__ void ray_half_writeback(const MapGeom& geom, const RayItem& it, bool upper, int cy0, bool walked,
                                                uint32_t* __restrict__ cells, SlotMeta* __restrict__ meta,
                                                uint32_t* __restrict__ bands_all, size_t cells_per_grid, const uint32_t* s_win,
                                                const int2* s_row, int* s_blo, int* s_bhi, int* s_ext, const uint4* s_lrow,
                                                const int* s_xinfo ,
                                                uint32_t eo_shared, int wy0, int wh, int band0, bool* saturated_p,
                                                uint32_t* moved_p) {
    const int lane = threadIdx.x & 31, warp = threadIdx.x >> 5, n_warps = blockDim.x >> 5;
    const uint32_t n_bands_slot = bands_per_slot(geom);
    const bool fused = it.root != it.slot;
    uint32_t* grid = cells + (size_t)it.slot * cells_per_grid;
    uint32_t* bands = bands_all + (size_t)it.slot * n_bands_slot;
    const uint32_t* src = cells + (size_t)it.root * cells_per_grid;
    const uint32_t* src_bands = bands_all + (size_t)it.root * n_bands_slot;
    bool saturated = false;
    uint32_t moved = 0;
    const uint4* win4 = reinterpret_cast<const uint4*>(s_win);
    const int own_lo = upper ? cy0 : 0, own_hi = upper ? (int)geom.gh : cy0;
    if (own_hi <= own_lo) { *moved_p += 0; return; }
    const int shared_band = (cy0 % BAND_ROWS) ? cy0 / BAND_ROWS : -1;
    const SlotMeta sm = meta[it.root];
    int y_lo = 0x7fffffff, y_hi = -1;
    if (sm.x1 > sm.x0 && sm.y1 > sm.y0) { y_lo = min(y_lo, sm.y0); y_hi = max(y_hi, sm.y1 - 1); }
    if (fused && it.old_y1 > it.old_y0) { y_lo = min(y_lo, it.old_y0); y_hi = max(y_hi, it.old_y1 - 1); }
    if (s_ext[3] >= s_ext[1] && s_ext[2] >= s_ext[0]) { y_lo = min(y_lo, s_ext[1]); y_hi = max(y_hi, s_ext[3]); }
    y_lo = max(y_lo, own_lo); y_hi = min(y_hi, own_hi - 1);
    if (y_hi < y_lo) { return; }
    const int by0 = y_lo / BAND_ROWS, by1 = y_hi / BAND_ROWS;
    const uint32_t tpr = geom.tiles_per_row;
    constexpr int DEPTH = 2;
    const int rr = lane >> 2, uu = lane & 3;
    for (int bnd = by0 + warp; bnd <= by1; bnd += n_warps) {
        const bool is_shared = bnd == shared_band;
        const uint32_t es = src_bands[bnd];
        const uint32_t eo = fused ? ((is_shared && !upper) ? eo_shared : bands[bnd]) : es;
        const int lb = bnd - band0;
        bool touched = (unsigned)lb < (unsigned)HALF_MAX_BANDS && s_bhi[lb] >= s_blo[lb];
        uint32_t t0x = touched ? ((uint32_t)s_blo[lb] & ~7u) : 0xffffu, t1x = touched ? min(geom.gw, ((uint32_t)s_bhi[lb] + 8u) & ~7u) : 0u;
        uint32_t n0 = t0x, n1 = t1x;
        if (is_shared && upper && s_xinfo[1] >= s_xinfo[0]) { n0 = min(n0, (uint32_t)s_xinfo[0] & ~7u); n1 = max(n1, min(geom.gw, ((uint32_t)s_xinfo[1] + 8u) & ~7u)); }
        if (es) { n0 = min(n0, es & 0xffffu); n1 = max(n1, es >> 16); }
        uint32_t u0 = t0x, u1 = t1x;
        if (fused) { if (es) { u0 = min(u0, es & 0xffffu); u1 = max(u1, es >> 16); } if (eo) { u0 = min(u0, eo & 0xffffu); u1 = max(u1, eo >> 16); } }
        __syncwarp();
        if (lane == 0 && (upper || !is_shared)) bands[bnd] = n1 > n0 ? (n0 | (n1 << 16)) : 0u;
        if (u1 <= u0) continue;
        const int t_lo = (int)(u0 / TILE_COLS), t_hi = (int)((u1 + TILE_COLS - 1u) / TILE_COLS);
        const int y = bnd * BAND_ROWS + rr, ly = y - wy0;
        const bool own_row = y >= own_lo && y < own_hi;
        int wfirst = 0, wx0 = 0, ww = 0;
        if (walked && touched && (unsigned)ly < (unsigned)wh) { const int2 row = s_row[ly]; wfirst = row.x; wx0 = row.y & 0xffff; ww = row.y >> 16; }
        const bool start_row = upper && walked && y == cy0;
        const uint32_t sx0 = es & 0xffffu, sx1 = es >> 16;
        const size_t band_off = (size_t)bnd * tpr * TILE_CELLS + 8u * (uint32_t)lane;
        for (int tt = t_lo; tt < t_hi; tt += DEPTH) {
            uint4 va[DEPTH], vb[DEPTH], d[DEPTH];
            bool need[DEPTH];
#pragma unroll
            for (int k = 0; k < DEPTH; ++k) {
                const int t = tt + k;
                const int lx = t * (int)TILE_COLS + 8 * uu - wx0;
                d[k] = make_uint4(0u, 0u, 0u, 0u);
                bool lower_too = false;
                if (t < t_hi && own_row && (unsigned)lx < (unsigned)ww) {
                    d[k] = win4[(wfirst + lx) >> 3];
                    if (start_row && (uint32_t)(lx >> 3) < HALF_XCHG_GROUPS) {
                        const uint4 dl = s_lrow[lx >> 3];
                        lower_too = (dl.x | dl.y | dl.z | dl.w) != 0u;
                    }
                }
                need[k] = t < t_hi && own_row && (fused || lower_too || (d[k].x | d[k].y | d[k].z | d[k].w) != 0u);
            }
#pragma unroll
            for (int k = 0; k < DEPTH; ++k) {
                const int t = tt + k;
                const uint32_t x = (uint32_t)t * TILE_COLS + 8u * (uint32_t)uu;
                va[k] = make_uint4(0u, 0u, 0u, 0u); vb[k] = va[k];
                if (need[k] && x >= sx0 && x < sx1) {
                    const V8 s8 = ld_stream_v8(reinterpret_cast<const V8*>(src + band_off + (size_t)t * TILE_CELLS));
                    va[k] = s8.a; vb[k] = s8.b;
                    moved += fused ? 1u : 0u;
                }
            }
#pragma unroll
            for (int k = 0; k < DEPTH; ++k) {
                if (!need[k]) continue;
                const int t = tt + k;
                if ((d[k].x | d[k].y | d[k].z | d[k].w) != 0u) merge_window_group(va[k], vb[k], d[k], &saturated);
                if (start_row) {
                    const int lx = t * (int)TILE_COLS + 8 * uu - wx0;
                    if ((unsigned)lx < (unsigned)ww && (uint32_t)(lx >> 3) < HALF_XCHG_GROUPS) {
                        const uint4 dl = s_lrow[lx >> 3];
                        if ((dl.x | dl.y | dl.z | dl.w) != 0u) merge_window_group(va[k], vb[k], dl, &saturated);
                    }
                }
                V8 o8; o8.a = va[k]; o8.b = vb[k];
                st_stream_v8(reinterpret_cast<V8*>(grid + band_off + (size_t)t * TILE_CELLS), o8);
                moved += fused ? 1u : 0u;
            }
        }
    }
    if (saturated) *saturated_p = true;
    *moved_p += moved;
}

__global__ void __maxnreg__(80)
k_ray_update_half(MapGeom geom, ScanDevice scan, const ParticleResult* __restrict__ results, uint32_t first_particle,
                  const uint32_t* __restrict__ alive_list, const RayItem* __restrict__ clones, const RayItem* __restrict__ owners,
                  const uint32_t* __restrict__ readers, uint32_t* __restrict__ done, uint32_t* __restrict__ xflag,
                  HalfXchg* __restrict__ xchg, uint32_t* __restrict__ spill_scratch, const int32_t* __restrict__ slot_of,
                  uint32_t* __restrict__ cells, SlotMeta* __restrict__ meta, uint32_t* __restrict__ bands_all,
                  size_t cells_per_grid, int radius, uint32_t window_bytes, StepCounters* counters,
                  uint32_t* __restrict__ xdone, uint32_t n_local, uint32_t signal_epoch) {
    extern __shared__ __align__(16) uint32_t s_win[];
    uint16_t* s_beam = reinterpret_cast<uint16_t*>(reinterpret_cast<unsigned char*>(s_win) + window_bytes);
    __shared__ uint32_t s_nspill, s_nmine, s_eo_shared;
    __shared__ int s_blo[HALF_MAX_BANDS], s_bhi[HALF_MAX_BANDS];
    __shared__ int2 s_row[HALF_MAX_ROWS + 1];
    __shared__ uint32_t s_rowb[HALF_MAX_ROWS];
    __shared__ int s_ext[4], s_xinfo[2], s_lext[4];
    __shared__ unsigned long long s_next;
    __shared__ RayItem s_item;
    __shared__ float s_pose[3];
    __shared__ uint4 s_lrow[HALF_XCHG_GROUPS];
    const unsigned long long n_items = counters->n_alive;
    const int gw = (int)geom.gw, gh = (int)geom.gh;
    const uint32_t win_base = (uint32_t)__cvta_generic_to_shared(s_win);
    const int lane = threadIdx.x & 31, warp = threadIdx.x >> 5, n_warps = blockDim.x >> 5;
    const uint32_t n_bands_slot = bands_per_slot(geom);
    bool saturated = false;
    uint32_t spilled = 0, cell_steps = 0, moved = 0;
    uint32_t* my_spill = spill_scratch + (size_t)blockIdx.x * RAY_SPILL_CAP;
    const bool helper = threadIdx.x == blockDim.x - 32u;
    SlotMeta* pend_meta = nullptr;
    uint32_t* pend_done = nullptr;
    int pend_ext[4] = {0, 0, -1, -1};
    uint32_t* pend_sig = nullptr;
    SlotMeta* pend_sig_meta = nullptr;
    auto flush_pending = [&]() {
        if (pend_meta != nullptr) {
            SlotMeta b = *pend_meta;
            const int am = BOX_ALIGN - 1;
            const int x0 = pend_ext[0] & ~am, x1 = min(gw, (pend_ext[2] + 1 + am) & ~am), y0 = pend_ext[1], y1 = pend_ext[3] + 1;
            if (b.x1 <= b.x0) { b.x0 = x0; b.y0 = y0; b.x1 = x1; b.y1 = y1; }
            else { b.x0 = min(b.x0, x0); b.y0 = min(b.y0, y0); b.x1 = max(b.x1, x1); b.y1 = max(b.y1, y1); }
            *pend_meta = b;
            pend_meta = nullptr;
        }
        if (pend_done != nullptr) {
            __threadfence();
            atomicAdd(pend_done, 1u);
            pend_done = nullptr;
        }
        if (pend_sig != nullptr) {
            __threadfence_system();
            if (atomicAdd(pend_sig, 1u) == 1u) {
                __threadfence_system();
                asm volatile("st.release.sys.global.u32 [%0], %1;" ::"l"(&pend_sig_meta->pad0), "r"(signal_epoch) : "memory");
            }
            pend_sig = nullptr;
        }
    };
    auto pop_next = [&]() {
        const unsigned long long w = atomicAdd(&counters->ray_work_head, 1ull);
        if (w < 2ull * n_items) {
            RayItem nit;
            if (clones) nit = ray_item_at(clones, owners, n_local, counters, w >> 1);
            else { nit.particle = alive_list[w >> 1]; nit.slot = slot_of[nit.particle]; nit.root = nit.slot; nit.old_y0 = nit.old_y1 = 0; nit.pad = 0u; }
            const ParticleResult r = results[first_particle + nit.particle];
            s_item = nit;
            s_pose[0] = r.x; s_pose[1] = r.y; s_pose[2] = r.theta;
        }
        s_next = w;
    };
    if (threadIdx.x == 0) pop_next();
#ifdef SLAMRS_RAY_TRACE
    long long t_prev = clock64();
#endif

    for (;;) {
        __syncthreads();
        const unsigned long long work = s_next;
        if (work >= 2ull * n_items) break;
        RAY_STAMP(0);
        RAY_LOG(work, 0);
        const unsigned long long item = work >> 1;
        const bool upper = (work & 1ull) != 0ull;
        const RayItem it = s_item;
        const bool fused = it.root != it.slot;
        uint32_t* grid = cells + (size_t)it.slot * cells_per_grid;
        uint32_t* bands = bands_all + (size_t)it.slot * n_bands_slot;
        const float px = s_pose[0], py = s_pose[1], ptheta = s_pose[2];
        const float sx = world_to_grid(px, geom.pos_x, geom.res);
        const float sy = world_to_grid(py, geom.pos_y, geom.res);
        const long long lcx = f32_as_isize(floorf(sx)), lcy = f32_as_isize(floorf(sy));
        const bool walked = !(lcx < 0 || lcx >= (long long)geom.gw || lcy < 0 || lcy >= (long long)geom.gh);
        if (!walked && !fused) {
            __syncthreads();
            if (helper) {
                flush_pending();
                pop_next();
                if (signal_epoch != 0u && it.pad != 0u) { pend_sig = xdone + item; pend_sig_meta = &meta[it.slot]; }
            }
            continue;
        }
        const int cx0 = walked ? (int)lcx : 0, cy0 = walked ? (int)lcy : 0;
        const int rad = walked ? radius : 0;
        ext_init(s_ext);
        if (threadIdx.x == 0) {
            s_nspill = 0u; s_nmine = 0u; s_xinfo[0] = 0x7fffffff; s_xinfo[1] = -1; s_eo_shared = 0u;
            s_lext[0] = s_lext[1] = 0x7fffffff; s_lext[2] = s_lext[3] = -1;
        }
        for (int i = threadIdx.x; i < HALF_MAX_BANDS; i += blockDim.x) { s_blo[i] = 0x7fffffff; s_bhi[i] = -1; }
        if (threadIdx.x < HALF_XCHG_GROUPS) s_lrow[threadIdx.x] = make_uint4(0u, 0u, 0u, 0u);

        const int wy0 = upper ? cy0 : max(0, cy0 - rad), wy1 = upper ? min(gh, cy0 + rad + 1) : cy0 + 1;
        const int band0 = wy0 / BAND_ROWS;
        const int wh = walked ? wy1 - wy0 : 0;
        for (int ly = threadIdx.x; ly < wh; ly += blockDim.x) {
            const int dy = wy0 + ly - cy0;
            const int hw = isqrt_small(rad * rad - dy * dy);
            const int x0 = max(0, cx0 - hw) & ~7;
            const int x1 = min(gw, (min(gw, cx0 + hw + 1) + 7) & ~7);
            s_row[ly].y = x0 | ((x1 - x0) << 16);
        }
        __syncthreads();
        if (threadIdx.x >= 32) {
            uint4* w4 = reinterpret_cast<uint4*>(s_win);
            for (int i = threadIdx.x - 32; i < (int)(window_bytes >> 4); i += blockDim.x - 32) w4[i] = make_uint4(0u, 0u, 0u, 0u);
        }
        if (threadIdx.x < 32) {
            int carry = 0;
            for (int base = 0; base < wh; base += 32) {
                const int ly = base + (int)threadIdx.x;
                const int w = ly < wh ? (s_row[ly].y >> 16) : 0;
                int inc = w;
#pragma unroll
                for (int o = 1; o < 32; o <<= 1) {
                    const int t = __shfl_up_sync(0xffffffffu, inc, o);
                    if ((int)threadIdx.x >= o) inc += t;
                }
                if (ly < wh) {
                    const int first = carry + inc - w;
                    s_row[ly].x = first;
                    s_rowb[ly] = win_base + 2u * (uint32_t)(first - (s_row[ly].y & 0xffff));
                }
                carry += __shfl_sync(0xffffffffu, inc, 31);
            }
            if (threadIdx.x == 0) s_row[wh] = make_int2(carry, 0);
        }
        __syncthreads();
        RAY_STAMP(1);
        RAY_LOG(work, 1);
        if (walked) {
            for (uint32_t t0 = 0; t0 < scan.n_beams; t0 += blockDim.x) {
                const uint32_t t = t0 + threadIdx.x;
                bool mine = false;
                uint32_t b = 0u;
                if (t < scan.n_beams) {
                    b = scan.order ? scan.order[t] : t;
                    const float dist = scan.dist[b];
                    const float a = __fadd_rn(ptheta, scan.angle[b]);
                    const float dyq = __fmul_rn(sinf(a), dist);
                    const float margin = 1.0e-4f * (fabsf(py) + fabsf(geom.pos_y) + fabsf(dist) + geom.res);
                    bool up;
                    if (dyq > margin) up = true;
                    else if (dyq < -margin) up = false;
                    else {
                        float ex, ey;
                        beam_endpoint(px, py, ptheta, scan.angle[b], dist, &ex, &ey);
                        const float y1 = world_to_grid(ey, geom.pos_y, geom.res);
                        up = fabsf(__fsub_rn(y1, sy)) == 0.0f || y1 > sy;
                    }
                    mine = up == upper;
                }
                const unsigned m = __ballot_sync(0xffffffffu, mine);
                if (m) {
                    uint32_t base = 0u;
                    if (lane == 0) base = atomicAdd(&s_nmine, (uint32_t)__popc(m));
                    base = __shfl_sync(0xffffffffu, base, 0);
                    if (mine) s_beam[base + __popc(m & ((1u << lane) - 1u))] = (uint16_t)b;
                }
            }
        }
        __syncthreads();
        RAY_STAMP(2);
        RAY_LOG(work, 2);
        if (helper) {
            flush_pending();
            pop_next();
        }
        if (walked) {
            const bool disc_in_grid = cx0 - rad >= 0 && cx0 + rad < gw && (upper ? cy0 + rad < gh : cy0 - rad >= 0);
            ray_walk_packed<true>(geom, scan, s_beam, s_nmine, px, py, ptheta, sx, sy, cx0, cy0, rad, disc_in_grid, wy0, wh, band0,
                                  s_win, s_row, s_rowb, s_blo, s_bhi, s_ext, nullptr, nullptr, &s_nspill, my_spill, nullptr,
                                  &spilled, &cell_steps);
        }
#ifdef SLAMRS_RAY_TRACE
        if (threadIdx.x == 0) atomicAdd(&g_ray_trace[12], (unsigned long long)(clock64() - t_prev));
#endif
        __syncthreads();
        RAY_STAMP(3);
        RAY_LOG(work, 3);

        const uint4* win4 = reinterpret_cast<const uint4*>(s_win);
        {
            const int rr = lane & 7, bq = lane >> 3;
            int wxmin = 0x7fffffff, wymin = 0x7fffffff, wxmax = -1, wymax = -1;
            const int n_wbands = wh > 0 ? (wy0 + wh - 1) / BAND_ROWS - band0 + 1 : 0;
            for (int q = warp; 4 * q < n_wbands; q += n_warps) {
                const int lb = 4 * q + bq;
                const int y = (band0 + lb) * BAND_ROWS + rr, ly = y - wy0;
                int first = 0x7fffffff, last = -1, rx0 = 0;
                int2 row = make_int2(0, 0);
                if (lb < n_wbands && (unsigned)ly < (unsigned)wh && (upper || y != cy0)) { row = s_row[ly]; rx0 = row.y & 0xffff; }
                const int groups = row.y >> 19;
                for (int g = 0; g < 34; ++g) {
                    if (__all_sync(0xffffffffu, g >= groups)) break;
                    if (g < groups) {
                        const uint4 d = win4[(row.x >> 3) + g];
                        if ((d.x | d.y | d.z | d.w) != 0u) { first = min(first, g); last = g; }
                    }
                }
                int xlo = last >= 0 ? rx0 + 8 * first : 0x7fffffff, xhi = last >= 0 ? rx0 + 8 * last + 7 : -1;
                if (last >= 0) { wymin = min(wymin, y); wymax = max(wymax, y); }
#pragma unroll
                for (int o = 1; o < 8; o <<= 1) {
                    xlo = min(xlo, __shfl_xor_sync(0xffffffffu, xlo, o));
                    xhi = max(xhi, __shfl_xor_sync(0xffffffffu, xhi, o));
                }
                wxmin = min(wxmin, xlo); wxmax = max(wxmax, xhi);
                if (rr == 0 && xhi >= xlo && (unsigned)lb < (unsigned)HALF_MAX_BANDS) { atomicMin(&s_blo[lb], xlo); atomicMax(&s_bhi[lb], xhi); }
            }
#pragma unroll
            for (int o = 16; o > 0; o >>= 1) {
                wxmin = min(wxmin, __shfl_xor_sync(0xffffffffu, wxmin, o)); wxmax = max(wxmax, __shfl_xor_sync(0xffffffffu, wxmax, o));
                wymin = min(wymin, __shfl_xor_sync(0xffffffffu, wymin, o)); wymax = max(wymax, __shfl_xor_sync(0xffffffffu, wymax, o));
            }
            if (lane == 0) ext_add(s_ext, wxmin, wymin, wxmax, wymax);
        }
        __syncthreads();
        RAY_STAMP(4);
        RAY_LOG(work, 4);

        const int shared_band = (cy0 % BAND_ROWS) ? cy0 / BAND_ROWS : -1;
        if (walked && !upper) {
            HalfXchg* x = xchg + item;
            const int2 row = s_row[wh - 1];
            const int groups = row.y >> 19;
            if (threadIdx.x < HALF_XCHG_GROUPS)
                x->row[threadIdx.x] = (int)threadIdx.x < groups ? win4[(row.x >> 3) + threadIdx.x] : make_uint4(0u, 0u, 0u, 0u);
            if (threadIdx.x == 0) {
                const int lb = shared_band - band0;
                const bool any = shared_band >= 0 && (unsigned)lb < (unsigned)HALF_MAX_BANDS && s_bhi[lb] >= s_blo[lb];
                x->band_lo = any ? s_blo[lb] : 0x7fffffff;
                x->band_hi = any ? s_bhi[lb] : -1;
                x->ext[0] = s_ext[0]; x->ext[1] = s_ext[1]; x->ext[2] = s_ext[2]; x->ext[3] = s_ext[3];
                uint32_t nh = 0u;
                const uint32_t ns = min(s_nspill, RAY_SPILL_CAP);
                for (uint32_t k = 0; k < ns; ++k) {
                    const uint32_t e = my_spill[k];
                    if ((int)((e >> 15) & 0x7fffu) == cy0) { if (nh < HALF_XCHG_HITS) x->hits[nh] = e; nh++; }
                }
                if (nh > HALF_XCHG_HITS) atomicAdd(&counters->fuse_overflow, 1ull);
                x->n_hits = min(nh, HALF_XCHG_HITS);
                s_eo_shared = (fused && shared_band >= 0) ? bands[shared_band] : 0u;
            }
            __threadfence();
            __syncthreads();
            if (threadIdx.x == 0) asm volatile("st.release.gpu.global.u32 [%0], %1;" ::"l"(xflag + item), "r"(1u) : "memory");
        }
        if (walked && upper) {
            if (threadIdx.x == 0) {
                uint32_t seen;
                for (;;) {
                    asm volatile("ld.acquire.gpu.global.u32 %0, [%1];" : "=r"(seen) : "l"(xflag + item) : "memory");
                    if (seen != 0u) break;
                    __nanosleep(100);
                }
            }
            __syncthreads();
            const HalfXchg* x = xchg + item;
            if (threadIdx.x < HALF_XCHG_GROUPS) s_lrow[threadIdx.x] = __ldcg(&x->row[threadIdx.x]);
            if (threadIdx.x == 0) {
                s_xinfo[0] = __ldcg(&x->band_lo); s_xinfo[1] = __ldcg(&x->band_hi);
                s_lext[0] = __ldcg(&x->ext[0]); s_lext[1] = __ldcg(&x->ext[1]); s_lext[2] = __ldcg(&x->ext[2]); s_lext[3] = __ldcg(&x->ext[3]);
                const uint32_t nh = __ldcg(&x->n_hits);
                for (uint32_t k = 0; k < nh; ++k) {
                    const uint32_t at = atomicAdd(&s_nspill, 1u);
                    if (at < RAY_SPILL_CAP) my_spill[at] = __ldcg(&x->hits[k]);
                }
            }
            __syncthreads();
            if (warp == 0) {
                const int2 row = s_row[0];
                const int rx0 = row.y & 0xffff;
                int first = 0x7fffffff, last = -1;
                for (int g = lane; g < (int)HALF_XCHG_GROUPS; g += 32) {
                    const uint4 d = s_lrow[g];
                    if ((d.x | d.y | d.z | d.w) != 0u) { first = min(first, g); last = max(last, g); }
                }
#pragma unroll
                for (int o = 16; o > 0; o >>= 1) {
                    first = min(first, __shfl_xor_sync(0xffffffffu, first, o));
                    last = max(last, __shfl_xor_sync(0xffffffffu, last, o));
                }
                if (lane == 0 && last >= 0) {
                    ext_add(s_ext, rx0 + 8 * first, cy0, rx0 + 8 * last + 7, cy0);
                    band_add(s_blo, s_bhi, band0, cy0, rx0 + 8 * first, rx0 + 8 * last + 7);
                }
            }
            __syncthreads();
        }
        RAY_STAMP(5);
        RAY_LOG(work, 5);
        if (!fused && readers != nullptr) {
            if (threadIdx.x == 0) {
                const uint32_t want = readers[it.slot];
                if (want != 0u) {
                    uint32_t seen;
                    for (;;) {
                        asm volatile("ld.acquire.gpu.global.u32 %0, [%1];" : "=r"(seen) : "l"(done + it.slot) : "memory");
                        if (seen >= want) break;
                        __nanosleep(100);
                    }
                }
            }
            __syncthreads();
        }
        RAY_STAMP(6);
        RAY_LOG(work, 6);
        ray_half_writeback(geom, it, upper, cy0, walked, cells, meta, bands_all, cells_per_grid, s_win, s_row, s_blo, s_bhi, s_ext,
                           s_lrow, s_xinfo, s_eo_shared, wy0, wh, band0, &saturated, &moved);
#ifdef SLAMRS_RAY_TRACE
        if (threadIdx.x == 0) atomicAdd(&g_ray_trace[13], (unsigned long long)(clock64() - t_prev));
#endif
        __syncthreads();
        RAY_STAMP(fused ? 7 : 11);
        RAY_LOG(work, 7);
        RAY_LOG_V(work, 9, (unsigned long long)ray_smid() | ((unsigned long long)blockIdx.x << 16) | (fused ? 1ull << 40 : 0ull) | (upper ? 1ull << 41 : 0ull) | (it.pad ? 1ull << 42 : 0ull) | ((unsigned long long)s_nmine << 44));
#ifdef SLAMRS_RAY_TRACE
        if (threadIdx.x == 0) atomicAdd(&g_ray_trace_items[fused ? 0 : 1], 1ull);
#endif
        {
            const uint32_t ns = s_nspill;
            if (ns > RAY_SPILL_CAP && threadIdx.x == 0) atomicAdd(&counters->fuse_overflow, 1ull);
            for (uint32_t k = threadIdx.x; k < min(ns, RAY_SPILL_CAP); k += blockDim.x) {
                const uint32_t e = my_spill[k];
                const uint32_t x = e & 0x7fffu, y = (e >> 15) & 0x7fffu;
                if (!upper && (int)y == cy0) continue;
                global_cell_add(&grid[phys_index(geom, x, y)], (e & 0x40000000u) ? CELL_OCC_INC : CELL_FREE_INC, &saturated);
            }
        }
        if (helper) {
            if (upper && walked) {
                const int e0 = min(s_ext[0], s_lext[0]), e1 = min(s_ext[1], s_lext[1]), e2 = max(s_ext[2], s_lext[2]), e3 = max(s_ext[3], s_lext[3]);
                if (e2 >= e0 && e3 >= e1) { pend_meta = &meta[it.slot]; pend_ext[0] = e0; pend_ext[1] = e1; pend_ext[2] = e2; pend_ext[3] = e3; }
            }
            if (fused) pend_done = &done[it.root];
            if (signal_epoch != 0u && it.pad != 0u) { pend_sig = xdone + item; pend_sig_meta = &meta[it.slot]; }
        }
        RAY_STAMP(14);
        RAY_LOG(work, 8);
    }
    if (helper) flush_pending();
#ifdef SLAMRS_RAY_TRACE
    if (threadIdx.x == 0) { atomicAdd(&g_ray_trace[15], (unsigned long long)(clock64() - t_prev)); }
#endif
    if (saturated) atomicAdd(&counters->saturated, 1ull);
    if (spilled) atomicAdd(&counters->spilled, (unsigned long long)spilled);
#pragma unroll
    for (int o = 16; o > 0; o >>= 1) { cell_steps += __shfl_down_sync(0xffffffffu, cell_steps, o); moved += __shfl_down_sync(0xffffffffu, moved, o); }
    if ((threadIdx.x & 31) == 0 && cell_steps) atomicAdd(&counters->ray_cell_steps, (unsigned long long)cell_steps);
    if ((threadIdx.x & 31) == 0 && moved) {
        atomicAdd(&counters->copy_bytes, (unsigned long long)moved * 32ull);
        atomicAdd(&counters->ray_copy_bytes, (unsigned long long)moved * 32ull);
    }
}

__global__ void __launch_bounds__(1024)
k_sort_beams(const float* __restrict__ dist, uint32_t n, uint16_t* __restrict__ order) {
    __shared__ float s_key[SORT_MAX_BEAMS];
    __shared__ uint16_t s_idx[SORT_MAX_BEAMS];
    for (uint32_t i = threadIdx.x; i < SORT_MAX_BEAMS; i += blockDim.x) {
        float k = -1.0f;
        if (i < n) { const float d = fabsf(dist[i]); if (d == d) k = d; }
        s_key[i] = k;
        s_idx[i] = (uint16_t)i;
    }
    __syncthreads();
    for (uint32_t size = 2; size <= SORT_MAX_BEAMS; size <<= 1) {
        for (uint32_t stride = size >> 1; stride > 0; stride >>= 1) {
            for (uint32_t t = threadIdx.x; t < SORT_MAX_BEAMS / 2; t += blockDim.x) {
                const uint32_t lo = 2 * t - (t & (stride - 1));
                const uint32_t hi = lo + stride;
                const bool descending = (lo & size) == 0;
                const float a = s_key[lo], b = s_key[hi];
                const bool a_first = a > b || (a == b && s_idx[lo] < s_idx[hi]);
                if (a_first != descending) {
                    s_key[lo] = b; s_key[hi] = a;
                    const uint16_t ti = s_idx[lo]; s_idx[lo] = s_idx[hi]; s_idx[hi] = ti;
                }
            }
            __syncthreads();
        }
    }
    for (uint32_t i = threadIdx.x; i < n; i += blockDim.x) order[i] = s_idx[i];
}
void launch_sort_beams(cudaStream_t stream, const float* dist, uint32_t n_beams, uint16_t* order) {
    k_sort_beams<<<1, 1024, 0, stream>>>(dist, n_beams, order);
}

static int ray_packed_radius(int radius_cells) {
    int radius = radius_cells < 1 ? 1 : (radius_cells > RAY_MAX_RADIUS ? RAY_MAX_RADIUS : radius_cells);
    while (radius > 1 && (size_t)ray_window_cells_upper_bound_packed(radius) * 2 > (size_t)RAY_MAX_SMEM) radius--;
    return radius;
}
bool ray_update_can_fuse(const MapGeom& geom, uint32_t n_beams, size_t cells_per_grid, bool force_generic, int radius_cells) {
    return !force_generic && geom.gw % 8u == 0u && cells_per_grid % 8u == 0u && n_beams <= RAY_PACKED_MAX_BEAMS &&
           geom.tiled != 0u && geom.windowed == 0u && geom.gw < 32768u && geom.gh < 32768u &&
           ray_packed_radius(radius_cells) >= radius_cells;
}
#ifdef SLAMRS_RAY_TRACE
static void ray_log_dump_after_launch(cudaStream_t stream) {
    static int launches = 0;
    const char* path = getenv("SLAMRS_RAY_TRACE_LOG");
    const char* which = getenv("SLAMRS_RAY_TRACE_LAUNCH");
    const int first = which ? atoi(which) : 20;
    ++launches;
    if (!path || launches < first || launches >= first + 4) return;
    int dev = 0;
    cudaGetDevice(&dev);
    const std::string name = std::string(path) + ".d" + std::to_string(dev) + "." + std::to_string(launches - first);
    path = name.c_str();
    cudaStreamSynchronize(stream);
    std::vector<unsigned long long> log((size_t)RAY_LOG_ITEMS * RAY_LOG_COLS);
    if (cudaMemcpyFromSymbol(log.data(), g_ray_log, log.size() * sizeof(unsigned long long)) == cudaSuccess) {
        if (FILE* f = fopen(path, "wb")) { fwrite(log.data(), sizeof(unsigned long long), log.size(), f); fclose(f); }
    }
}
#endif
int ray_trace(unsigned long long* out18) {
#ifdef SLAMRS_RAY_TRACE
    cudaError_t e = cudaMemcpyFromSymbol(out18, g_ray_trace, sizeof(unsigned long long) * 16);
    if (e == cudaSuccess) e = cudaMemcpyFromSymbol(out18 + 16, g_ray_trace_items, sizeof(unsigned long long) * 2);
    unsigned long long z[18] = {0};
    cudaMemcpyToSymbol(g_ray_trace, z, sizeof(unsigned long long) * 16);
    cudaMemcpyToSymbol(g_ray_trace_items, z, sizeof(unsigned long long) * 2);
    return (int)e;
#else
    (void)out18;
    return -1;
#endif
}
size_t ray_spill_scratch_words(int num_sms) { return (size_t)num_sms * 4u * RAY_SPILL_CAP; }

size_t ray_half_xchg_bytes() { return sizeof(HalfXchg); }

cudaError_t launch_ray_update(cudaStream_t stream, MapGeom geom, ScanDevice scan, const ParticleResult* results,
                              uint32_t first_particle, uint32_t n_local, const uint32_t* alive_list,
                              const RayItem* clones, const RayItem* owners, const uint32_t* readers, uint32_t* done,
                              uint32_t* xflag, void* xchg, uint32_t* spill_scratch, const int32_t* slot_of, uint32_t* cells,
                              SlotMeta* meta, uint32_t* bands, size_t cells_per_grid, int radius_cells, StepCounters* counters,
                              uint64_t* window_cells, bool force_generic, int num_sms, uint32_t* xdone, uint32_t signal_epoch) {
    if (ray_update_can_fuse(geom, scan.n_beams, cells_per_grid, force_generic, radius_cells)) {
        const int radius = ray_packed_radius(radius_cells);
        const size_t wcells = (size_t)ray_window_cells_upper_bound_half(radius);
        const size_t wbytes = (wcells * 2 + 15) & ~(size_t)15;
        const size_t smem = wbytes + (((size_t)scan.n_beams * 2 + 15) & ~(size_t)15);
        int threads = (int)(((scan.n_beams + 1u) / 2u + 31u) / 32u * 32u) + 0;
        threads = threads < 128 ? 128 : (threads > RAY_MAX_THREADS ? RAY_MAX_THREADS : threads);
        *window_cells = 2 * wcells;
        int per_sm = 0;
        cudaError_t e = cudaOccupancyMaxActiveBlocksPerMultiprocessor(&per_sm, k_ray_update_half, threads, smem);
        if (e != cudaSuccess) return e;
        if (per_sm < 1) per_sm = 1;
        if (per_sm > 4) per_sm = 4;
        uint32_t grid = (uint32_t)(per_sm * num_sms);
        if (grid > 2u * n_local) grid = 2u * n_local;
        k_ray_update_half<<<grid, threads, smem, stream>>>(geom, scan, results, first_particle, alive_list, clones, owners, readers, done,
                                                           xflag, (HalfXchg*)xchg, spill_scratch, slot_of, cells, meta, bands,
                                                           cells_per_grid, radius, (uint32_t)wbytes, counters, xdone, n_local, signal_epoch);
#ifdef SLAMRS_RAY_TRACE
        ray_log_dump_after_launch(stream);
#endif
        return cudaSuccess;
    }
    int threads = (int)((scan.n_beams + 31u) / 32u * 32u);
    threads = threads < 128 ? 128 : (threads > RAY_MAX_THREADS ? RAY_MAX_THREADS : threads);
    if (!force_generic && geom.gw % 8u == 0u && cells_per_grid % 8u == 0u && scan.n_beams <= RAY_PACKED_MAX_BEAMS) {
        const int radius = ray_packed_radius(radius_cells);
        const size_t wmax = (size_t)ray_window_cells_upper_bound_packed(radius);
        *window_cells = wmax;
        int per_sm = 0;
        cudaError_t e = cudaOccupancyMaxActiveBlocksPerMultiprocessor(&per_sm, k_ray_update_packed, threads, wmax * 2);
        if (e != cudaSuccess) return e;
        if (per_sm < 1) per_sm = 1;
        if (per_sm > 4) per_sm = 4;
        uint32_t grid = (uint32_t)(per_sm * num_sms);
        if (grid > n_local) grid = n_local;
        k_ray_update_packed<<<grid, threads, wmax * 2, stream>>>(geom, scan, results, first_particle, alive_list, slot_of, cells, meta,
                                                                 bands, cells_per_grid, radius, radius_cells, counters);
        return cudaSuccess;
    }
    const bool vec = (geom.gw % 4u == 0u) && (cells_per_grid % 4u == 0u);
    int radius = radius_cells < 1 ? 1 : (radius_cells > RAY_MAX_RADIUS ? RAY_MAX_RADIUS : radius_cells);
    while (radius > 1 && (size_t)ray_window_cells_upper_bound(radius, vec) * 4 > (size_t)RAY_MAX_SMEM) radius--;
    const size_t wmax = (size_t)ray_window_cells_upper_bound(radius, vec);
    const size_t smem = wmax * 4;
    *window_cells = wmax;
    if (vec)
        k_ray_update<true><<<n_local, threads, smem, stream>>>(geom, scan, results, first_particle, alive_list, slot_of, cells, meta, bands,
                                                               cells_per_grid, radius, radius_cells, counters);
    else
        k_ray_update<false><<<n_local, threads, smem, stream>>>(geom, scan, results, first_particle, alive_list, slot_of, cells, meta, bands,
                                                                cells_per_grid, radius, radius_cells, counters);
    return cudaSuccess;
}

cudaError_t configure_ray_kernels() {
    cudaError_t e = cudaFuncSetAttribute(k_ray_update<true>, cudaFuncAttributeMaxDynamicSharedMemorySize, RAY_MAX_SMEM);
    if (e != cudaSuccess) return e;
    e = cudaFuncSetAttribute(k_ray_update_packed, cudaFuncAttributeMaxDynamicSharedMemorySize, RAY_MAX_SMEM);
    if (e != cudaSuccess) return e;
    e = cudaFuncSetAttribute(k_ray_update_half, cudaFuncAttributeMaxDynamicSharedMemorySize, RAY_MAX_SMEM / 2 + 8192);
    if (e != cudaSuccess) return e;
    return cudaFuncSetAttribute(k_ray_update<false>, cudaFuncAttributeMaxDynamicSharedMemorySize, RAY_MAX_SMEM);
}

}
```

slamrs_b200/csrc/kernels_resample.cu:

```cuda
#include "kernels_common.cuh"

namespace slamrs {


constexpr int W_CLUSTER = 8;

constexpr uint32_t FOLD_HEADS_PER_CTA = 32;
constexpr uint32_t FOLD_HEADS_MAX = FOLD_HEADS_PER_CTA * W_CLUSTER;
constexpr uint32_t FOLD_STAGE = 2048;
constexpr int FOLD_MAX_ROUNDS = 4;
constexpr int FOLD_MARGIN_BITS = 40;
constexpr int FOLD_LREG = 16;
constexpr int FOLD_THREADS = 512;
constexpr int FOLD_GENERIC_THREADS = 1024;
constexpr uint32_t FOLD_MAX_CHUNKS = FOLD_GENERIC_THREADS * W_CLUSTER;

struct FoldTd {
    double d0, d1;
    uint32_t qc;
};
template <int LREG>
struct FoldRec {
    double d0, d1;
    uint32_t q_prev;
// ... 363 lines not shown
                                    &info_sum, 8);
    FOLD_STAMP(3);
    if (!ok) {
        info_sum.fallback = 1u;
        if (threadIdx.x == 0) {
            double s = 0.0;
            for (uint32_t i = 0; i < n; ++i) s = __dadd_rn(s, results[i].weight);
            s_seq[0] = s;
        }
        __syncthreads();
        sum = s_seq[0];
    }

    double sqpart = 0.0;
    long long best_key = (long long)0x8000000000000000ull;
    uint32_t best_i = 0;
    bool have = false;
    all_zero = true;
    auto norm_one = [&](uint32_t j, double x) {
        const double w = __ddiv_rn(x, sum);
        if (LREG) s_tile[threadIdx.x * (LREG + 1) + j] = w; else w_norm[lo + j] = w;
        sqpart = __dadd_rn(sqpart, __dmul_rn(w, w));
        all_zero = all_zero && w == 0.0;
        const long long k = total_order_key(w);
        if (!have || k >= best_key) { best_key = k; best_i = lo + j; have = true; }
        return w;
    };
    if (LREG) {
#pragma unroll
        for (int j = 0; j < (LREG ? LREG : 1); ++j) v[j] = (uint32_t)j < cnt ? norm_one(j, v[j]) : 0.0;
        flush_tile(w_norm);
    } else {
        for (uint32_t j = 0; j < cnt; ++j) norm_one(j, results[lo + j].weight);
    }
    FOLD_STAMP(4);
    double cta_sq;
    const double sq_offset = block_excl_scan_f64(sqpart, sh.warp_f64, &cta_sq);

    const int lane = threadIdx.x & 31, wid = threadIdx.x >> 5;
    auto argmax_warp = [&]() {
#pragma unroll
        for (int o = 16; o > 0; o >>= 1) {
            const long long okey = __shfl_down_sync(0xffffffffu, best_key, o);
            const uint32_t oi = __shfl_down_sync(0xffffffffu, best_i, o);
            const bool ohave = __shfl_down_sync(0xffffffffu, (int)have, o) != 0;
            if (ohave && (!have || okey > best_key || (okey == best_key && oi > best_i))) { best_key = okey; best_i = oi; have = true; }
        }
    };
    argmax_warp();
    if (lane == 0) { s_key[wid] = best_key; s_arg[wid] = have ? best_i : 0xffffffffu; }
    __syncthreads();
    if (wid == 0) {
        have = lane < (THREADS >> 5) && s_arg[lane] != 0xffffffffu;
        best_key = have ? s_key[lane] : (long long)0x8000000000000000ull;
        best_i = have ? s_arg[lane] : 0u;
        argmax_warp();
        if (lane == 0) {
            if (C == 1u) { s_ckey[0] = best_key; s_carg[0] = have ? best_i : 0xffffffffu; s_sq[0] = cta_sq; }
            else {
                cluster.map_shared_rank(&s_ckey[0], 0)[crank] = best_key;
                cluster.map_shared_rank(&s_carg[0], 0)[crank] = have ? best_i : 0xffffffffu;
                cluster.map_shared_rank(&s_sq[0], 0)[crank] = cta_sq;
            }
        }
    }
    FOLD_STAMP(5);

    if (ok) {
        double c_in, c_out, c_total;
        ok = exact_left_fold<LREG>(cluster, sh, n, L, cnt, all_zero, __ddiv_rn(r_in, sum), __ddiv_rn(r_out, sum), v,
                                   [&](uint32_t j, double s) { if (LREG) s_tile[threadIdx.x * (LREG + 1) + j] = s; else cum[lo + j] = s; },
                                   [&](uint32_t i) { return __ldcg(&w_norm[i]); }, true, fold_scratch, &c_in, &c_out, &c_total,
                                   &info_cum, 16);
        if (!ok) info_cum.fallback = 1u;
        else if (LREG) flush_tile(cum);
    } else {
        info_cum.rounds = 0u; info_cum.heads = 0u; info_cum.fallback = 1u;
    }
    FOLD_STAMP(6);
    if (!ok) {
        fold_sync(cluster, C);
        if (gt == 0) {
            double c = 0.0;
            for (uint32_t i = 0; i < n; ++i) { const double w = __ldcg(&w_norm[i]); c = i ? __dadd_rn(c, w) : w; cum[i] = c; }
        }
        fold_sync(cluster, C);
    }

    FoldInfo info_sq = {0u, 0u, 0u};
    double sq_exact = 0.0;
    if (resample_tau > 0.0) {
        double q_in = sq_offset;
        if (C > 1u) {
            if (threadIdx.x < C) cluster.map_shared_rank(&sh.cta_part[0], threadIdx.x)[crank] = cta_sq;
            cluster.sync();
            q_in = 0.0;
            for (uint32_t r = 0; r < crank; ++r) q_in = __dadd_rn(q_in, sh.cta_part[r]);
            q_in = __dadd_rn(q_in, sq_offset);
        }
        if (LREG) {
#pragma unroll
            for (int j = 0; j < (LREG ? LREG : 1); ++j) v[j] = __dmul_rn(v[j], v[j]);
        }
        double q_lo, q_hi;
        const bool sq_ok = exact_left_fold<LREG>(cluster, sh, n, L, cnt, all_zero, q_in, __dadd_rn(q_in, sqpart), v,
                                                 [](uint32_t, double) {},
                                                 [&](uint32_t i) { const double w = __ldcg(&w_norm[i]); return __dmul_rn(w, w); },
                                                 false, fold_scratch, &q_lo, &q_hi, &sq_exact, &info_sq, 24);
        if (!sq_ok) {
            info_sq.fallback = 1u;
            if (gt == 0) {
                double s = 0.0;
                for (uint32_t i = 0; i < n; ++i) { const double w = __ldcg(&w_norm[i]); s = __dadd_rn(s, __dmul_rn(w, w)); }
                sq_exact = s;
            }
        }
    }
    if (gt == 0) {
        long long bk = 0; uint32_t bi = 0; bool h = false;
        for (uint32_t r = 0; r < C; ++r) {
            if (s_carg[r] == 0xffffffffu) continue;
            if (!h || s_ckey[r] > bk || (s_ckey[r] == bk && s_carg[r] > bi)) { bk = s_ckey[r]; bi = s_carg[r]; h = true; }
        }
        counters->max_particle = bi;
        counters->sum = sum;
        double sq = sq_exact;
        if (!(resample_tau > 0.0)) {
            sq = 0.0;
            for (uint32_t r = 0; r < C; ++r) sq = __dadd_rn(sq, s_sq[r]);
        }
        counters->n_eff = __ddiv_rn(1.0, sq);
        counters->do_resample = (resample_tau > 0.0 && !(__ddiv_rn(1.0, sq) < __dmul_rn(resample_tau, (double)n))) ? 0ull : 1ull;
        counters->fold_rounds = (unsigned long long)max(max(info_sum.rounds, info_cum.rounds), info_sq.rounds);
        counters->fold_heads = (unsigned long long)max(max(info_sum.heads, info_cum.heads), info_sq.heads);
        counters->fold_fallback = (unsigned long long)(info_sum.fallback | (info_cum.fallback << 1) | (info_sq.fallback << 2));
    }
    FOLD_STAMP(7);
}

static size_t weights_tile_bytes() { return sizeof(double) * FOLD_THREADS * (FOLD_LREG + 1); }
WeightsShape weights_shape(uint32_t n_total) {
    uint32_t c = 1u;
    while (c < (uint32_t)W_CLUSTER && (uint64_t)c * FOLD_THREADS * FOLD_LREG < n_total) c <<= 1;
    WeightsShape s;
    s.cluster = c;
    s.regs = (uint64_t)c * FOLD_THREADS * FOLD_LREG >= n_total;
    s.threads = s.regs ? (uint32_t)FOLD_THREADS : (uint32_t)FOLD_GENERIC_THREADS;
    s.chunk = s.regs ? (uint32_t)FOLD_LREG : (uint32_t)(((uint64_t)n_total + c * s.threads - 1u) / (c * s.threads));
    return s;
}
void launch_weights(cudaStream_t stream, const ParticleResult* results, uint32_t n_total, double* w_norm,
                    double* cum, double* fold_scratch, double resample_tau, StepCounters* counters) {
    const WeightsShape shape = weights_shape(n_total);
    const uint32_t c = shape.cluster;
    const bool regs = shape.regs;
    cudaLaunchConfig_t cfg = {};
    cfg.gridDim = dim3(c, 1, 1);
    cfg.blockDim = dim3(shape.threads, 1, 1);
    cfg.dynamicSmemBytes = regs ? weights_tile_bytes() : 0;
    cfg.stream = stream;
    cudaLaunchAttribute attr[2];
    attr[0].id = cudaLaunchAttributeClusterDimension;
    attr[0].val.clusterDim.x = c; attr[0].val.clusterDim.y = 1; attr[0].val.clusterDim.z = 1;
    attr[1].id = cudaLaunchAttributeProgrammaticStreamSerialization;
    attr[1].val.programmaticStreamSerializationAllowed = 1;
    cfg.attrs = attr;
    cfg.numAttrs = 2;
    if (regs) cudaLaunchKernelEx(&cfg, k_weights<FOLD_LREG, FOLD_THREADS>, results, n_total, w_norm, cum, fold_scratch, resample_tau, counters);
    else cudaLaunchKernelEx(&cfg, k_weights<0, FOLD_GENERIC_THREADS>, results, n_total, w_norm, cum, fold_scratch, resample_tau, counters);
}
size_t weights_scratch_doubles() { return 2u * FOLD_MAX_CHUNKS; }
int weights_trace(long long* out64) {
#ifdef SLAMRS_FOLD_TRACE
    return (int)cudaMemcpyFromSymbol(out64, g_fold_trace, sizeof(long long) * 64);
#else
    (void)out64;
    return -1;
#endif
}


__device__ __forceinline__ double resample_threshold(uint32_t n, double U, uint32_t m0) {
    const double num = (double)n;
    const double r = __ddiv_rn(__dmul_rn(U, 1.0), num);
    return __dadd_rn(r, __ddiv_rn(__dmul_rn(__dsub_rn((double)(m0 + 1u), 1.0), 1.0), num));
}
__device__ __forceinline__ uint32_t first_not_below(const double* __restrict__ cum, uint32_t lo, uint32_t hi, double u) {
    while (lo < hi) {
        const uint32_t mid = lo + ((hi - lo) >> 1);
        if (u > cum[mid]) lo = mid + 1; else hi = mid;
    }
    return lo;
}

constexpr uint32_t RS_COARSE = 2048;

__global__ void __launch_bounds__(256)
k_resample_indices(const ParticleResult* __restrict__ results, const double* __restrict__ cum, uint32_t n,
                   const double* __restrict__ u01_caller, uint64_t seed, uint64_t step, uint32_t* __restrict__ idx,
                   float* __restrict__ pose_next, uint32_t first_particle, uint32_t n_local, bool build_alive,
                   uint32_t* __restrict__ alive_list, RayLists ray, const double* __restrict__ w_norm,
                   double* __restrict__ carry, StepCounters* counters) {
    __shared__ double s_coarse[RS_COARSE];
    pdl_wait();
    const bool resample = counters->do_resample != 0ull;
    const uint32_t stride = (n + RS_COARSE - 1u) / RS_COARSE;
    const uint32_t n_coarse = (n + stride - 1u) / stride;
    for (uint32_t j = threadIdx.x; j < n_coarse; j += blockDim.x) s_coarse[j] = cum[min(n, (j + 1u) * stride) - 1u];
    __syncthreads();
    const uint32_t m0 = blockIdx.x * blockDim.x + threadIdx.x;
    const double U = u01_caller ? *u01_caller : slamrs_stream::resample_uniform(seed, step);
    const int lane = threadIdx.x & 31;
    auto source_of = [&](uint32_t m, bool* ran_off) {
        const double u = resample_threshold(n, U, m);
        const uint32_t blk = first_not_below(s_coarse, 0u, n_coarse, u);
        *ran_off = blk >= n_coarse;
        if (blk >= n_coarse) return n - 1u;
        return first_not_below(cum, blk * stride, min(n, (blk + 1u) * stride) - 1u, u);
    };
    bool ran_off = false;
    uint32_t src_idx = 0xffffffffu;
    if (m0 < n) {
        if (resample) src_idx = source_of(m0, &ran_off); else src_idx = m0;
        if (carry != nullptr) carry[m0] = w_norm[m0];
        if (m0 == 0u) counters->carry_active = resample ? 0ull : 1ull;
        if (ran_off) atomicAdd(&counters->clamped, 1ull);
        idx[m0] = src_idx;
        const ParticleResult src = results[src_idx];
        if (m0 >= first_particle && m0 < first_particle + n_local) {
            float* q = pose_next + 3 * (size_t)(m0 - first_particle);
            q[0] = src.x; q[1] = src.y; q[2] = src.theta;
        }
        if ((unsigned long long)m0 == counters->max_particle) {
            counters->est_pose[0] = src.x; counters->est_pose[1] = src.y; counters->est_pose[2] = src.theta;
        }
    }
    if (!build_alive) return;
    uint32_t prev = __shfl_up_sync(0xffffffffu, src_idx, 1);
    if (lane == 0 && m0 > 0 && m0 < n) {
        bool dummy;
        prev = resample ? source_of(m0 - 1u, &dummy) : m0 - 1u;
    }
    const bool alive = m0 < n && (m0 == 0 || prev != src_idx) && src_idx >= first_particle &&
                       src_idx < first_particle + n_local;
    if (ray.clones == nullptr) {
        const unsigned mask = __ballot_sync(0xffffffffu, alive);
        if (mask) {
            const int leader = __ffs(mask) - 1;
            unsigned long long base = 0;
            if (lane == leader) base = atomicAdd(&counters->n_alive, (unsigned long long)__popc(mask));
            base = __shfl_sync(0xffffffffu, base, leader);
            if (alive) alive_list[base + __popc(mask & ((1u << lane) - 1u))] = src_idx - first_particle;
        }
        return;
    }
    RayItem it{0u, 0, 0, 0, 0, 0u};
    bool clone = false, remote = false;
    if (alive && ray.mark_remote != 0u) {
        const uint32_t end = first_particle + n_local;
        remote = !(m0 >= first_particle && m0 < end);
        if (!remote && end < n) {
            bool dummy;
            remote = (resample ? source_of(end, &dummy) : end) == src_idx;
        }
    }
    if (alive) {
        it.pad = remote ? 1u : 0u;
        it.particle = src_idx - first_particle;
        it.slot = ray.slot_of[it.particle];
        it.root = ray.alias_of[it.slot];
        clone = it.root != it.slot;
        if (clone) {
            atomicAdd(&ray.readers[it.root], 2u);
            ray.alias_of[it.slot] = it.slot;
            const SlotMeta old = ray.meta[it.slot];
            if (old.x1 > old.x0 && old.y1 > old.y0) { it.old_y0 = old.y0; it.old_y1 = old.y1; }
            SlotMeta src = ray.meta[it.root];
            src.pad0 = 0;
            ray.meta[it.slot] = src;
        }
    }
    const unsigned mcr = __ballot_sync(0xffffffffu, alive && clone && remote), mcl = __ballot_sync(0xffffffffu, alive && clone && !remote);
    const unsigned mor = __ballot_sync(0xffffffffu, alive && !clone && remote), mol = __ballot_sync(0xffffffffu, alive && !clone && !remote);
    unsigned long long bcr = 0, bcl = 0, bor = 0, bol = 0;
    if (lane == 0) {
        const unsigned mc = mcr | mcl, all = mc | mor | mol;
        if (all) atomicAdd(&counters->n_alive, (unsigned long long)__popc(all));
        if (mc) {
            atomicAdd(&counters->n_mat, (unsigned long long)__popc(mc));
            atomicAdd(&counters->n_mat_leaders, (unsigned long long)__popc(mc));
        }
        if (mcr) bcr = atomicAdd(&counters->ray_items_front, (unsigned long long)__popc(mcr));
        if (mcl) bcl = atomicAdd(&counters->ray_items_front_local, (unsigned long long)__popc(mcl));
        if (mor) bor = atomicAdd(&counters->ray_items_back, (unsigned long long)__popc(mor));
        if (mol) bol = atomicAdd(&counters->ray_items_back_local, (unsigned long long)__popc(mol));
    }
    bcr = __shfl_sync(0xffffffffu, bcr, 0); bcl = __shfl_sync(0xffffffffu, bcl, 0);
    bor = __shfl_sync(0xffffffffu, bor, 0); bol = __shfl_sync(0xffffffffu, bol, 0);
    const unsigned below = (1u << lane) - 1u;
    if (alive && clone && remote) ray.clones[bcr + __popc(mcr & below)] = it;
    if (alive && clone && !remote) ray.clones[ray.n_local - 1u - (bcl + __popc(mcl & below))] = it;
    if (alive && !clone && remote) ray.owners[bor + __popc(mor & below)] = it;
    if (alive && !clone && !remote) ray.owners[ray.n_local - 1u - (bol + __popc(mol & below))] = it;
}

void launch_resample_indices(cudaStream_t stream, const ParticleResult* results, const double* cum,
                             uint32_t n_total, const double* u01_caller, uint64_t seed, uint64_t step,
                             uint32_t* idx, float* pose_next, uint32_t first_particle, uint32_t n_local,
                             bool build_alive, uint32_t* alive_list, RayLists ray, const double* w_norm, double* carry,
                             StepCounters* counters) {
    launch_pdl(k_resample_indices, dim3((n_total + 255) / 256), dim3(256), 0, stream, results, cum, n_total, u01_caller, seed, step, idx,
               pose_next, first_particle, n_local, build_alive, alive_list, ray, w_norm, carry, counters);
}

__global__ void __launch_bounds__(256)
k_mark_alive(const uint32_t* __restrict__ idx, uint32_t n_total, uint32_t first_particle, uint32_t n_local,
             bool all_particles, uint32_t* __restrict__ alive_list, StepCounters* counters) {
    const uint32_t j = blockIdx.x * blockDim.x + threadIdx.x;
    bool alive = false;
    if (j < n_local) {
        if (all_particles) {
            alive = true;
        } else {
            const uint32_t v = first_particle + j;
            uint32_t lo = 0, hi = n_total;
            while (lo < hi) {
                const uint32_t mid = lo + ((hi - lo) >> 1);
                if (idx[mid] < v) lo = mid + 1; else hi = mid;
            }
            alive = lo < n_total && idx[lo] == v;
        }
    }
    const unsigned m = __ballot_sync(0xffffffffu, alive);
    if (m) {
        const int lane = threadIdx.x & 31, leader = __ffs(m) - 1;
        unsigned long long base = 0;
        if (lane == leader) base = atomicAdd(&counters->n_alive, (unsigned long long)__popc(m));
        base = __shfl_sync(0xffffffffu, base, leader);
        if (alive) alive_list[base + __popc(m & ((1u << lane) - 1u))] = j;
    }
}

void launch_mark_alive(cudaStream_t stream, const uint32_t* idx, uint32_t n_total, uint32_t first_particle,
                       uint32_t n_local, bool all_particles, uint32_t* alive_list, StepCounters* counters) {
    k_mark_alive<<<(n_local + 255) / 256, 256, 0, stream>>>(idx, n_total, first_particle, n_local, all_particles,
                                                           alive_list, counters);
}


__device__ __forceinline__ uint32_t lower_bound_u32(const uint32_t* a, uint32_t lo, uint32_t hi, uint32_t v) {
    while (lo < hi) {
        const uint32_t mid = lo + ((hi - lo) >> 1);
        if (a[mid] < v) lo = mid + 1; else hi = mid;
    }
    return lo;
}

constexpr uint32_t PLAN_STAGED_MAX_S = 8192;
__host__ __device__ inline size_t plan_staged_bytes(uint32_t S) { return (size_t)S * 22u + 64u; }

__global__ void __launch_bounds__(1024) k_plan(PlanArgs a) {
    extern __shared__ __align__(16) unsigned char s_dyn[];
    __shared__ uint32_t s_warp[33];
    const uint32_t S = a.n_local, lo = a.rank * a.n_local, hi = lo + S;
    const uint32_t T = blockDim.x, t = threadIdx.x;
    const uint32_t chunk = (S + T - 1) / T;
    const uint32_t c0 = min(S, t * chunk), c1 = min(S, c0 + chunk);
    const uint32_t E = (uint32_t)a.counters->n_spare;

    uint32_t* idx_l;
    int32_t* slot_old;
    int32_t* slot_new;
    int32_t* free_list;
    uint8_t* keep;
    uint8_t* need;
    if (a.staged) {
        idx_l = reinterpret_cast<uint32_t*>(s_dyn);
        slot_old = reinterpret_cast<int32_t*>(idx_l + S);
        slot_new = slot_old + S;
        free_list = slot_new + S;
        keep = reinterpret_cast<uint8_t*>(free_list + 2 * (size_t)S + 4);
        need = keep + S;
        for (uint32_t j = t; j < S; j += T) { idx_l[j] = a.idx[lo + j]; slot_old[j] = a.slot_old[j]; keep[j] = 0; }
    } else {
        idx_l = const_cast<uint32_t*>(a.idx) + lo;
        slot_old = const_cast<int32_t*>(a.slot_old);
        slot_new = a.slot_new;
        free_list = a.free_list;
        keep = reinterpret_cast<uint8_t*>(a.keep);
        need = reinterpret_cast<uint8_t*>(a.need);
        for (uint32_t j = t; j < S; j += T) keep[j] = 0;
    }
    __syncthreads();

    uint32_t nA = 0, nR = 0;
    for (uint32_t m = t; m < S; m += T) {
        const uint32_t src = idx_l[m];
        const bool first = (m == 0) || (idx_l[m - 1] != src);
        const bool local = (src >= lo && src < hi);
        int cls;
        if (local && first) {
            cls = 0;
            keep[src - lo] = 1;
            slot_new[m] = slot_old[src - lo];
        } else if (local) cls = 1;
        else if (first) cls = 2;
        else cls = 3;
        need[m] = (uint8_t)cls;
        nA += (first ? 1u : 0u);
        nR += (cls == 2 ? 1u : 0u);
    }
    __syncthreads();

    const uint32_t idx_first = idx_l[0], idx_last = idx_l[S - 1];
    for (uint32_t j = t; j < S; j += T) {
        int f = 0;
        if (!keep[j]) {
            f = 1;
            if (a.world > 1) {
                const uint32_t v = lo + j;
                if (v < idx_first && lo > 0) {
                    const uint32_t p = lower_bound_u32(a.idx, 0, lo, v);
                    if (p < lo && a.idx[p] == v) f = 2;
                } else if (v > idx_last && hi < a.n_total) {
                    const uint32_t p = lower_bound_u32(a.idx, hi, a.n_total, v);
                    if (p < a.n_total && a.idx[p] == v) f = 2;
                }
            }
        }
        keep[j] = (uint8_t)f;
    }
    __syncthreads();

    uint32_t n_safe_c = 0, n_unsafe_c = 0;
    for (uint32_t j = c0; j < c1; ++j) { n_safe_c += (keep[j] == 1); n_unsafe_c += (keep[j] == 2); }
    uint32_t n_safe, n_unsafe;
    uint32_t ps = block_excl_scan_u32(n_safe_c, s_warp, &n_safe);
    uint32_t pu = block_excl_scan_u32(n_unsafe_c, s_warp, &n_unsafe);
    for (uint32_t j = c0; j < c1; ++j) {
        if (keep[j] == 1) free_list[ps++] = slot_old[j];
        else if (keep[j] == 2) free_list[n_safe + E + pu++] = slot_old[j];
    }
    for (uint32_t e = t; e < E; e += T) free_list[n_safe + e] = a.spare_list[e];
    const uint32_t usable = n_safe + E;

    uint32_t n_cons_c = 0, n_item_c = 0;
    for (uint32_t m = c0; m < c1; ++m) { n_cons_c += (need[m] != 0); n_item_c += (need[m] == 2); }
    uint32_t n_cons, n_items = 0;
    uint32_t pos = block_excl_scan_u32(n_cons_c, s_warp, &n_cons);
    uint32_t ipos = a.defer ? block_excl_scan_u32(n_item_c, s_warp, &n_items) : pos;
    __syncthreads();

    const uint32_t ipos_start = ipos;
    uint32_t n_lead_c = 0;
    const unsigned long long est_m = a.counters->max_particle - lo;
    if (t == 0 && est_m >= S) a.counters->est_meta_ptr = 0ull;
    uint32_t run_first = c0 < c1 ? lower_bound_u32(idx_l, 0, S, idx_l[c0]) : 0u;
    for (uint32_t m = c0; m < c1; ++m) {
        const int cls = need[m];
        const uint32_t src = idx_l[m];
        if (m > c0 && idx_l[m - 1] != src) run_first = m;
        if (cls == 0) {
            if (m == est_m) a.counters->est_meta_ptr = (unsigned long long)(uintptr_t)(a.meta + slot_new[m]);
            continue;
        }
        if (pos < usable && a.defer && cls != 2) {
            slot_new[m] = free_list[pos];
            need[m] = (uint8_t)(cls == 1 ? 11 : 12);
            if (m == est_m && cls == 1) a.counters->est_meta_ptr = (unsigned long long)(uintptr_t)(a.meta + slot_old[src - lo]);
        } else if (pos < usable) {
            const int32_t dslot = free_list[pos];
            slot_new[m] = dslot;
            CopyItem it;
            if (cls == 1) {
                const int32_t sslot = slot_old[src - lo];
                it.src = a.cells + (size_t)sslot * a.cells_per_grid;
                it.src_meta = a.meta + sslot;
                it.src_bands = a.bands + (size_t)sslot * a.n_bands;
            } else {
                const uint32_t owner = src / S;
                const int32_t sslot = a.results[src].slot;
                it.src = a.peer_cells[owner] + (size_t)sslot * a.cells_per_grid;
                it.src_meta = a.peer_meta[owner] + sslot;
                it.src_bands = a.peer_bands[owner] + (size_t)sslot * a.n_bands;
            }
            it.dst = a.cells + (size_t)dslot * a.cells_per_grid;
            it.dst_meta = a.meta + dslot;
            it.dst_bands = a.bands + (size_t)dslot * a.n_bands;
            a.copies[ipos] = it;
            if (m == est_m) a.counters->est_meta_ptr = (unsigned long long)(uintptr_t)it.src_meta;
            const uint32_t k = (cls == 1) ? (m - run_first - 1u) : (m - run_first);
            const bool lead = a.defer || (k % COPY_FAN) == 0u;
            need[m] = (uint8_t)(lead ? 9 : 8);
            n_lead_c += lead;
            if (a.defer) ipos++;
        } else {
            slot_new[m] = (cls == 1) ? slot_old[src - lo] : slot_old[0];
            need[m] = 10;
        }
        pos++;
        if (!a.defer) ipos = pos;
    }
    uint32_t n_lead;
    uint32_t pl = block_excl_scan_u32(n_lead_c, s_warp, &n_lead);
    ipos = ipos_start;
    for (uint32_t m = c0; m < c1; ++m) {
        const int cls = need[m];
        if (cls == 9) a.leaders[pl++] = ipos;
        if (cls == 8 || cls == 9 || (!a.defer && cls == 10)) ipos++;
    }
    __syncthreads();
    long long est_root = -1ll;
    if (a.defer) {
        for (uint32_t m = c0; m < c1; ++m) {
            const int cls = need[m];
            int32_t root = slot_new[m];
            if (cls == 11) root = slot_old[idx_l[m] - lo];
            else if (cls == 12) root = slot_new[lower_bound_u32(idx_l, 0, S, idx_l[m])];
            if (cls == 8 || cls == 9 || cls == 11 || cls == 12) a.alias_of[slot_new[m]] = root;
            if (m == est_m) {
                est_root = root;
                if (cls == 12) a.counters->est_meta_ptr = (unsigned long long)(uintptr_t)(a.meta + root);
            }
        }
        if (est_root >= 0) a.counters->est_slot = est_root;
    }
    __syncthreads();
    const uint32_t used = min(n_cons, usable);
    for (uint32_t e = t; e < E; e += T) {
        const uint32_t left = usable - used;
        a.spare_list[e] = e < left ? free_list[used + e] : free_list[usable + (e - left)];
    }
    if (a.staged)
        for (uint32_t m = t; m < S; m += T) a.slot_new[m] = slot_new[m];

    uint32_t distinct, n_remote;
    block_excl_scan_u32(nA, s_warp, &distinct);
    block_excl_scan_u32(nR, s_warp, &n_remote);
    if (t == 0) {
        const bool short_of_slots = n_cons > usable;
        const uint32_t n_copied = a.defer ? n_items : used;
        a.counters->n_copies = short_of_slots ? 0u : n_copied;
        a.counters->n_leaders = short_of_slots ? 0u : n_lead;
        a.counters->n_pulls = n_remote;
        a.counters->distinct = distinct;
        a.counters->staging_short = (n_cons > usable) ? (unsigned long long)(n_cons - usable) : 0ull;
        const unsigned long long mp = a.counters->max_particle;
        a.counters->est_owner = mp / S;
        if (!a.defer || !(mp >= lo && mp < hi))
            a.counters->est_slot = (mp >= lo && mp < hi) ? (long long)slot_new[mp - lo] : -1ll;
        if (a.history) {
            StepRecord r;
            r.step = a.step; r.n_copies = n_copied; r.n_pulls = n_remote; r.distinct = distinct; r.n_leaders = n_lead;
            r.n_alive = 0; r.copy_bytes = 0; r.ray_cell_steps = 0; r.ray_copy_bytes = 0;
            a.history[a.step % STEP_HISTORY] = r;
        }
    }
}

__device__ __forceinline__ uint32_t block_excl_scan_max_u32(uint32_t v, uint32_t* warp_tot ) {
    const int lane = threadIdx.x & 31, wid = threadIdx.x >> 5, nw = (blockDim.x + 31) >> 5;
    uint32_t inc = v;
#pragma unroll
    for (int o = 1; o < 32; o <<= 1) {
        const uint32_t t = __shfl_up_sync(0xffffffffu, inc, o);
        if (lane >= o) inc = max(inc, t);
    }
    __syncthreads();
    if (lane == 31) warp_tot[wid] = inc;
    __syncthreads();
    if (wid == 0) {
        const uint32_t w = lane < nw ? warp_tot[lane] : 0u;
        uint32_t winc = w;
#pragma unroll
        for (int o = 1; o < 32; o <<= 1) {
            const uint32_t t = __shfl_up_sync(0xffffffffu, winc, o);
            if (lane >= o) winc = max(winc, t);
        }
        const uint32_t excl = __shfl_up_sync(0xffffffffu, winc, 1);
        warp_tot[lane] = lane == 0 ? 0u : excl;
    }
    __syncthreads();
    const uint32_t within = __shfl_up_sync(0xffffffffu, inc, 1);
    return max(warp_tot[wid], lane == 0 ? 0u : within);
}

__global__ void __launch_bounds__(1024)
k_materialize_list(const uint32_t* __restrict__ idx, uint32_t n_total, uint32_t first_particle, uint32_t S,
                   const int32_t* __restrict__ slot_of, int32_t* alias_of, uint32_t* cells, size_t cells_per_grid,
                   SlotMeta* meta, uint32_t* bands, uint32_t n_bands, CopyItem* __restrict__ items,
                   uint32_t* __restrict__ leaders, uint32_t* roots, StepCounters* counters) {
    __shared__ uint32_t s_warp[33];
    const uint32_t T = blockDim.x, t = threadIdx.x;
    const uint32_t chunk = (S + T - 1) / T;
    const uint32_t c0 = min(S, t * chunk), c1 = min(S, c0 + chunk);
    auto shared_and_written = [&](uint32_t j, int32_t* slot, int32_t* root) {
        if (idx != nullptr) {
            const uint32_t v = first_particle + j;
            const uint32_t q = lower_bound_u32(idx, 0, n_total, v);
            if (q >= n_total || idx[q] != v) return false;
        }
        *slot = slot_of[j];
        *root = alias_of[*slot];
        return *root != *slot;
    };
    uint32_t cnt = 0;
// ... 104 lines not shown
```

Before: 15.42 billion.

## Rework half-ray writeback into tile-unit work list with prefetched band headers

Restructures the half-ray writeback so band headers are computed once per 64-band chunk, prefix-summed into a flat list of tile units, and distributed evenly across warps instead of one band per warp. Band extents are prefetched with cp.async while row geometry is computed. The window is now cleared incrementally as groups are consumed rather than by a full memset each iteration. Work items are also reordered by an 'owned' flag built during resampling, which needs an extra per-slot scratch array and adds ballot/popc overhead per unit.

Result: faster. 15.69 billion (median of 6 runs) (+1.7%).

```diff
diff --git a/slamrs_b200/csrc/api.cu b/slamrs_b200/csrc/api.cu
--- a/slamrs_b200/csrc/api.cu
+++ b/slamrs_b200/csrc/api.cu
@@ -614,7 +614,7 @@
     CREATE_CU(cudaMalloc(&h->d_mat_roots, sizeof(uint32_t) * h->n_local));
     CREATE_CU(cudaMalloc(&h->d_alive, sizeof(uint32_t) * h->n_local));
     CREATE_CU(cudaMalloc(&h->d_ray_items, sizeof(RayItem) * 2 * (size_t)h->n_local));
-    CREATE_CU(cudaMalloc(&h->d_readers, sizeof(uint32_t) * (2 * (size_t)h->n_slots + 2 * (size_t)h->n_local)));
+    CREATE_CU(cudaMalloc(&h->d_readers, sizeof(uint32_t) * (3 * (size_t)h->n_slots + 2 * (size_t)h->n_local)));
     CREATE_CU(cudaMalloc(&h->d_ray_xchg, ray_half_xchg_bytes() * h->n_local));
     CREATE_CU(cudaMalloc(&h->d_ray_spill, sizeof(uint32_t) * ray_spill_scratch_words(h->num_sms)));
     CREATE_CU(cudaMallocHost(&h->h_counters, sizeof(StepCounters)));
@@ -944,7 +944,8 @@
     const bool half_items = ray_update_can_fuse(h->geom, h->n_beams, h->cells_per_grid, force_generic, h->radius_cells);
     const bool flag_pulls = h->world > 1 && fuse && half_items && h->boxed_copy && h->p2p_exchange;
     const uint32_t pull_epoch = flag_pulls ? (uint32_t)(h->step + 1ull) : 0u;
-    const size_t n_zero = half_items ? 2 * (size_t)h->n_slots + 2 * (size_t)h->n_local : 0;
+    const size_t n_zero = half_items ? 3 * (size_t)h->n_slots + 2 * (size_t)h->n_local : 0;
+    uint32_t* d_owned = h->d_readers + 2 * (size_t)h->n_slots + 2 * (size_t)h->n_local;
     PROF_MARK(h, 0);
     launch_motion_likelihood(s, h->geom, od, scan, h->d_pose[cur], h->d_slot[cur], h->defer ? h->d_alias : nullptr, h->d_cells, h->d_meta, h->cells_per_grid,
                              h->d_results, h->first, h->n_local, caller ? h->d_z : nullptr, h->cfg.seed, h->step, h->d_term_table, h->d_valid_list, h->d_n_valid,
@@ -966,9 +967,9 @@
     }
     PROF_MARK(h, 2);
     launch_weights(s, h->d_results, h->n_total, h->d_wnorm, h->d_cum, h->d_fold, (double)h->cfg.resample_threshold, h->d_counters);
-    RayLists ray{nullptr, nullptr, nullptr, nullptr, nullptr, nullptr, 0u, 0u};
+    RayLists ray{nullptr, nullptr, nullptr, nullptr, nullptr, nullptr, 0u, 0u, nullptr};
     if (fuse) ray = RayLists{h->d_ray_items, h->d_ray_items + h->n_local, h->d_slot[cur], h->d_alias, h->d_readers, h->d_meta,
-                             h->n_local, flag_pulls ? 1u : 0u};
+                             h->n_local, flag_pulls ? 1u : 0u, d_owned};
     launch_resample_indices(s, h->d_results, h->d_cum, h->n_total, caller ? h->d_u : nullptr, h->cfg.seed, h->step,
                             h->d_idx, h->d_pose[nxt], h->first, h->n_local, !all_particles, h->d_alive, ray, h->d_wnorm, h->d_carry,
                             h->d_counters);
@@ -1030,7 +1031,8 @@
                                 fuse ? h->d_readers + h->n_slots : nullptr, h->d_readers + 2 * (size_t)h->n_slots, h->d_ray_xchg,
                                 h->d_ray_spill, h->d_slot[cur],
                                 h->d_cells, h->d_meta, h->d_bands, h->cells_per_grid, h->radius_cells, h->d_counters, &h->window_cells,
-                                force_generic, h->num_sms, h->d_readers + 2 * (size_t)h->n_slots + h->n_local, pull_epoch));
+                                force_generic, h->num_sms, h->d_readers + 2 * (size_t)h->n_slots + h->n_local,
+                                fuse ? d_owned : nullptr, pull_epoch));
     h->launches++;
     PROF_MARK(h, 5);
     CU_TRY(h, cudaStreamWaitEvent(s, h->ev_plan, 0));
diff --git a/slamrs_b200/csrc/kernels.cuh b/slamrs_b200/csrc/kernels.cuh
--- a/slamrs_b200/csrc/kernels.cuh
+++ b/slamrs_b200/csrc/kernels.cuh
@@ -99,6 +99,7 @@
     SlotMeta* meta;
     uint32_t n_local;
     uint32_t mark_remote;
+    uint32_t* owned;
 };
 __device__ __forceinline__ RayItem ray_item_at(const RayItem* __restrict__ clones, const RayItem* __restrict__ owners,
                                                uint32_t n_local, const StepCounters* counters, unsigned long long k) {
@@ -156,6 +157,7 @@
                               size_t cells_per_grid, int radius_cells, StepCounters* counters,
                               uint64_t* window_cells, bool force_generic, int num_sms,
                               uint32_t* xdone ,
+                              const uint32_t* owned ,
 
                               uint32_t signal_epoch );
 
diff --git a/slamrs_b200/csrc/kernels_ray.cu b/slamrs_b200/csrc/kernels_ray.cu
--- a/slamrs_b200/csrc/kernels_ray.cu
+++ b/slamrs_b200/csrc/kernels_ray.cu
@@ -1,4 +1,5 @@
 #include "kernels_common.cuh"
+#include <cassert>
 #include <cstdio>
 #include <cstdlib>
 #include <string>
@@ -817,13 +818,32 @@
     return worst;
 }
 
-__device__ __noinline__ void ray_half_writeback(const MapGeom& geom, const RayItem& it, bool upper, int cy0, bool walked,
-                                                uint32_t* __restrict__ cells, SlotMeta* __restrict__ meta,
-                                                uint32_t* __restrict__ bands_all, size_t cells_per_grid, const uint32_t* s_win,
-                                                const int2* s_row, int* s_blo, int* s_bhi, int* s_ext, const uint4* s_lrow,
+constexpr int HALF_WB_BANDS = 64;
+constexpr int HALF_WB_UNITS = 2;
+struct HalfWbShared {
+    uint2 e[HALF_WB_BANDS];
+    int pre[HALF_WB_BANDS];
+    int wtot[HALF_WB_BANDS / 32];
+    int pf0, npf;
+    int rbox[2];
+};
+static_assert(HALF_WB_BANDS == 64, "the header pass scans two warps' worth of bands; units find their band in two ballots");
+
+__device__ __forceinline__ int2 half_wb_rows(const int* s_rbox, const RayItem& it, bool fused, int ey0, int ey1, int own_lo,
+                                             int own_hi) {
+    int y_lo = s_rbox[0], y_hi = s_rbox[1];
+    if (fused && it.old_y1 > it.old_y0) { y_lo = min(y_lo, it.old_y0); y_hi = max(y_hi, it.old_y1 - 1); }
+    if (ey1 >= ey0) { y_lo = min(y_lo, ey0); y_hi = max(y_hi, ey1); }
+    return make_int2(max(y_lo, own_lo), min(y_hi, own_hi - 1));
+}
+
+__device__ __noinline__ void ray_half_writeback(const MapGeom& geom, const RayItem& it, bool upper, int cy0,
+                                                uint32_t* __restrict__ cells, uint32_t* __restrict__ bands_all,
+                                                size_t cells_per_grid, uint32_t* s_win, const int2* s_row, const int* s_blo,
+                                                const int* s_bhi, const int* s_ext, const uint4* s_lrow,
                                                 const int* s_xinfo ,
-                                                uint32_t eo_shared, int wy0, int wh, int band0, bool* saturated_p,
-                                                uint32_t* moved_p) {
+                                                HalfWbShared& hb, uint32_t eo_shared, int wy0, int wh,
+                                                int band0, bool* saturated_p, uint32_t* moved_p) {
     const int lane = threadIdx.x & 31, warp = threadIdx.x >> 5, n_warps = blockDim.x >> 5;
     const uint32_t n_bands_slot = bands_per_slot(geom);
     const bool fused = it.root != it.slot;
@@ -833,87 +853,117 @@
     const uint32_t* src_bands = bands_all + (size_t)it.root * n_bands_slot;
     bool saturated = false;
     uint32_t moved = 0;
-    const uint4* win4 = reinterpret_cast<const uint4*>(s_win);
+    uint4* win4 = reinterpret_cast<uint4*>(s_win);
     const int own_lo = upper ? cy0 : 0, own_hi = upper ? (int)geom.gh : cy0;
-    if (own_hi <= own_lo) { *moved_p += 0; return; }
+    if (own_hi <= own_lo) return;
     const int shared_band = (cy0 % BAND_ROWS) ? cy0 / BAND_ROWS : -1;
-    const SlotMeta sm = meta[it.root];
-    int y_lo = 0x7fffffff, y_hi = -1;
-    if (sm.x1 > sm.x0 && sm.y1 > sm.y0) { y_lo = min(y_lo, sm.y0); y_hi = max(y_hi, sm.y1 - 1); }
-    if (fused && it.old_y1 > it.old_y0) { y_lo = min(y_lo, it.old_y0); y_hi = max(y_hi, it.old_y1 - 1); }
-    if (s_ext[3] >= s_ext[1] && s_ext[2] >= s_ext[0]) { y_lo = min(y_lo, s_ext[1]); y_hi = max(y_hi, s_ext[3]); }
-    y_lo = max(y_lo, own_lo); y_hi = min(y_hi, own_hi - 1);
-    if (y_hi < y_lo) { return; }
-    const int by0 = y_lo / BAND_ROWS, by1 = y_hi / BAND_ROWS;
+    const bool ext_any = s_ext[3] >= s_ext[1] && s_ext[2] >= s_ext[0];
+    const int2 yr = half_wb_rows(hb.rbox, it, fused, ext_any ? s_ext[1] : 0, ext_any ? s_ext[3] : -1, own_lo, own_hi);
+    if (yr.y < yr.x) return;
+    const int by0 = yr.x / BAND_ROWS, by1 = yr.y / BAND_ROWS;
     const uint32_t tpr = geom.tiles_per_row;
-    constexpr int DEPTH = 2;
     const int rr = lane >> 2, uu = lane & 3;
-    for (int bnd = by0 + warp; bnd <= by1; bnd += n_warps) {
-        const bool is_shared = bnd == shared_band;
-        const uint32_t es = src_bands[bnd];
-        const uint32_t eo = fused ? ((is_shared && !upper) ? eo_shared : bands[bnd]) : es;
-        const int lb = bnd - band0;
-        bool touched = (unsigned)lb < (unsigned)HALF_MAX_BANDS && s_bhi[lb] >= s_blo[lb];
-        uint32_t t0x = touched ? ((uint32_t)s_blo[lb] & ~7u) : 0xffffu, t1x = touched ? min(geom.gw, ((uint32_t)s_bhi[lb] + 8u) & ~7u) : 0u;
-        uint32_t n0 = t0x, n1 = t1x;
-        if (is_shared && upper && s_xinfo[1] >= s_xinfo[0]) { n0 = min(n0, (uint32_t)s_xinfo[0] & ~7u); n1 = max(n1, min(geom.gw, ((uint32_t)s_xinfo[1] + 8u) & ~7u)); }
-        if (es) { n0 = min(n0, es & 0xffffu); n1 = max(n1, es >> 16); }
-        uint32_t u0 = t0x, u1 = t1x;
-        if (fused) { if (es) { u0 = min(u0, es & 0xffffu); u1 = max(u1, es >> 16); } if (eo) { u0 = min(u0, eo & 0xffffu); u1 = max(u1, eo >> 16); } }
-        __syncwarp();
-        if (lane == 0 && (upper || !is_shared)) bands[bnd] = n1 > n0 ? (n0 | (n1 << 16)) : 0u;
-        if (u1 <= u0) continue;
-        const int t_lo = (int)(u0 / TILE_COLS), t_hi = (int)((u1 + TILE_COLS - 1u) / TILE_COLS);
-        const int y = bnd * BAND_ROWS + rr, ly = y - wy0;
-        const bool own_row = y >= own_lo && y < own_hi;
-        int wfirst = 0, wx0 = 0, ww = 0;
-        if (walked && touched && (unsigned)ly < (unsigned)wh) { const int2 row = s_row[ly]; wfirst = row.x; wx0 = row.y & 0xffff; ww = row.y >> 16; }
-        const bool start_row = upper && walked && y == cy0;
-        const uint32_t sx0 = es & 0xffffu, sx1 = es >> 16;
-        const size_t band_off = (size_t)bnd * tpr * TILE_CELLS + 8u * (uint32_t)lane;
-        for (int tt = t_lo; tt < t_hi; tt += DEPTH) {
-            uint4 va[DEPTH], vb[DEPTH], d[DEPTH];
-            bool need[DEPTH];
-#pragma unroll
-            for (int k = 0; k < DEPTH; ++k) {
-                const int t = tt + k;
-                const int lx = t * (int)TILE_COLS + 8 * uu - wx0;
+    for (int cb0 = by0; cb0 <= by1; cb0 += HALF_WB_BANDS) {
+        const int nb = min(HALF_WB_BANDS, by1 - cb0 + 1);
+        int n_tiles = 0, first_unit = 0, t_lo = 0;
+        uint32_t es = 0u;
+        if (threadIdx.x < HALF_WB_BANDS) {
+            const int i = (int)threadIdx.x, bnd = cb0 + i;
+            if (i < nb) {
+                const bool is_shared = bnd == shared_band;
+                const int pi = bnd - hb.pf0;
+                const bool fetched = cb0 == by0 && (unsigned)pi < (unsigned)hb.npf;
+                es = fetched ? hb.e[pi].x : src_bands[bnd];
+                uint32_t eo = es;
+                if (fused) eo = (is_shared && !upper) ? eo_shared : (fetched ? hb.e[pi].y : bands[bnd]);
+                const int lb = bnd - band0;
+                const bool touched = (unsigned)lb < (unsigned)HALF_MAX_BANDS && s_bhi[lb] >= s_blo[lb];
+                const uint32_t t0x = touched ? ((uint32_t)s_blo[lb] & ~7u) : 0xffffu;
+                const uint32_t t1x = touched ? min(geom.gw, ((uint32_t)s_bhi[lb] + 8u) & ~7u) : 0u;
+                uint32_t n0 = t0x, n1 = t1x;
+                if (is_shared && upper && s_xinfo[1] >= s_xinfo[0]) { n0 = min(n0, (uint32_t)s_xinfo[0] & ~7u); n1 = max(n1, min(geom.gw, ((uint32_t)s_xinfo[1] + 8u) & ~7u)); }
+                if (es) { n0 = min(n0, es & 0xffffu); n1 = max(n1, es >> 16); }
+                if (upper || !is_shared) bands[bnd] = n1 > n0 ? (n0 | (n1 << 16)) : 0u;
+                uint32_t u0 = t0x, u1 = t1x;
+                if (fused) { if (es) { u0 = min(u0, es & 0xffffu); u1 = max(u1, es >> 16); } if (eo) { u0 = min(u0, eo & 0xffffu); u1 = max(u1, eo >> 16); } }
+                if (u1 > u0) {
+                    t_lo = (int)(u0 / TILE_COLS);
+                    n_tiles = (int)((u1 + TILE_COLS - 1u) / TILE_COLS) - t_lo;
+                }
+            }
+            int incl = n_tiles;
+#pragma unroll
+            for (int o = 1; o < 32; o <<= 1) {
+                const int t = __shfl_up_sync(0xffffffffu, incl, o);
+                if (lane >= o) incl += t;
+            }
+            first_unit = incl - n_tiles;
+            if (lane == 31) hb.wtot[warp] = incl;
+        }
+        __syncthreads();
+        if (threadIdx.x < HALF_WB_BANDS) {
+            const int i = (int)threadIdx.x;
+            first_unit += warp == 1 ? hb.wtot[0] : 0;
+            hb.pre[i] = i < nb ? first_unit : 0x7fffffff;
+            hb.e[i] = make_uint2((uint32_t)(t_lo - first_unit), es);
+        }
+        __syncthreads();
+        const int total = hb.wtot[0] + hb.wtot[1];
+        const int pre_a = hb.pre[lane], pre_b = hb.pre[32 + lane];
+        for (int ub = warp * HALF_WB_UNITS; ub < total; ub += n_warps * HALF_WB_UNITS) {
+            uint4 va[HALF_WB_UNITS], vb[HALF_WB_UNITS], d[HALF_WB_UNITS];
+            uint32_t off[HALF_WB_UNITS];
+            int lg[HALF_WB_UNITS];
+            bool need[HALF_WB_UNITS], from_src[HALF_WB_UNITS];
+#pragma unroll
+            for (int k = 0; k < HALF_WB_UNITS; ++k) {
+                const int u = ub + k;
                 d[k] = make_uint4(0u, 0u, 0u, 0u);
-                bool lower_too = false;
-                if (t < t_hi && own_row && (unsigned)lx < (unsigned)ww) {
-                    d[k] = win4[(wfirst + lx) >> 3];
-                    if (start_row && (uint32_t)(lx >> 3) < HALF_XCHG_GROUPS) {
-                        const uint4 dl = s_lrow[lx >> 3];
-                        lower_too = (dl.x | dl.y | dl.z | dl.w) != 0u;
+                lg[k] = -1;
+                need[k] = false; from_src[k] = false;
+                off[k] = 0u;
+                if (u < total) {
+                    const int b = __popc(__ballot_sync(0xffffffffu, pre_a <= u)) + __popc(__ballot_sync(0xffffffffu, pre_b <= u)) - 1;
+                    const uint2 e = hb.e[b];
+                    const int t = u + (int)e.x, y = (cb0 + b) * BAND_ROWS + rr, ly = y - wy0;
+                    off[k] = ((uint32_t)(cb0 + b) * tpr + (uint32_t)t) * TILE_CELLS + 8u * (uint32_t)lane;
+                    const bool own_row = y >= own_lo && y < own_hi;
+                    bool lower_too = false;
+                    if (own_row && (unsigned)ly < (unsigned)wh) {
+                        const int2 row = s_row[ly];
+                        const int lx = t * (int)TILE_COLS + 8 * uu - (row.y & 0xffff);
+                        if ((unsigned)lx < (unsigned)(row.y >> 16)) {
+                            uint4* wp = &win4[(row.x + lx) >> 3];
+                            d[k] = *wp;
+                            if ((d[k].x | d[k].y | d[k].z | d[k].w) != 0u) *wp = make_uint4(0u, 0u, 0u, 0u);
+                            if (upper && y == cy0 && (uint32_t)(lx >> 3) < HALF_XCHG_GROUPS) {
+                                const uint4 dl = s_lrow[lx >> 3];
+                                lower_too = (dl.x | dl.y | dl.z | dl.w) != 0u;
+                                lg[k] = lower_too ? lx >> 3 : -1;
+                            }
+                        }
                     }
-                }
-                need[k] = t < t_hi && own_row && (fused || lower_too || (d[k].x | d[k].y | d[k].z | d[k].w) != 0u);
-            }
-#pragma unroll
-            for (int k = 0; k < DEPTH; ++k) {
-                const int t = tt + k;
-                const uint32_t x = (uint32_t)t * TILE_COLS + 8u * (uint32_t)uu;
+                    need[k] = own_row && (fused || lower_too || (d[k].x | d[k].y | d[k].z | d[k].w) != 0u);
+                    const uint32_t x = (uint32_t)t * TILE_COLS + 8u * (uint32_t)uu;
+                    from_src[k] = need[k] && x >= (e.y & 0xffffu) && x < (e.y >> 16);
+                }
+            }
+#pragma unroll
+            for (int k = 0; k < HALF_WB_UNITS; ++k) {
                 va[k] = make_uint4(0u, 0u, 0u, 0u); vb[k] = va[k];
-                if (need[k] && x >= sx0 && x < sx1) {
-                    const V8 s8 = ld_stream_v8(reinterpret_cast<const V8*>(src + band_off + (size_t)t * TILE_CELLS));
+                if (from_src[k]) {
+                    const V8 s8 = ld_stream_v8(reinterpret_cast<const V8*>(src + off[k]));
                     va[k] = s8.a; vb[k] = s8.b;
                     moved += fused ? 1u : 0u;
                 }
             }
 #pragma unroll
-            for (int k = 0; k < DEPTH; ++k) {
+            for (int k = 0; k < HALF_WB_UNITS; ++k) {
                 if (!need[k]) continue;
-                const int t = tt + k;
                 if ((d[k].x | d[k].y | d[k].z | d[k].w) != 0u) merge_window_group(va[k], vb[k], d[k], &saturated);
-                if (start_row) {
-                    const int lx = t * (int)TILE_COLS + 8 * uu - wx0;
-                    if ((unsigned)lx < (unsigned)ww && (uint32_t)(lx >> 3) < HALF_XCHG_GROUPS) {
-                        const uint4 dl = s_lrow[lx >> 3];
-                        if ((dl.x | dl.y | dl.z | dl.w) != 0u) merge_window_group(va[k], vb[k], dl, &saturated);
-                    }
-                }
+                if (lg[k] >= 0) merge_window_group(va[k], vb[k], s_lrow[lg[k]], &saturated);
                 V8 o8; o8.a = va[k]; o8.b = vb[k];
-                st_stream_v8(reinterpret_cast<V8*>(grid + band_off + (size_t)t * TILE_CELLS), o8);
+                st_stream_v8(reinterpret_cast<V8*>(grid + off[k]), o8);
                 moved += fused ? 1u : 0u;
             }
         }
@@ -929,7 +979,7 @@
                   HalfXchg* __restrict__ xchg, uint32_t* __restrict__ spill_scratch, const int32_t* __restrict__ slot_of,
                   uint32_t* __restrict__ cells, SlotMeta* __restrict__ meta, uint32_t* __restrict__ bands_all,
                   size_t cells_per_grid, int radius, uint32_t window_bytes, StepCounters* counters,
-                  uint32_t* __restrict__ xdone, uint32_t n_local, uint32_t signal_epoch) {
+                  uint32_t* __restrict__ xdone, const uint32_t* __restrict__ owned, uint32_t n_local, uint32_t signal_epoch) {
     extern __shared__ __align__(16) uint32_t s_win[];
     uint16_t* s_beam = reinterpret_cast<uint16_t*>(reinterpret_cast<unsigned char*>(s_win) + window_bytes);
     __shared__ uint32_t s_nspill, s_nmine, s_eo_shared;
@@ -939,9 +989,15 @@
     __shared__ int s_ext[4], s_xinfo[2], s_lext[4];
     __shared__ unsigned long long s_next;
     __shared__ RayItem s_item;
+    __shared__ unsigned long long s_item_pos;
     __shared__ float s_pose[3];
     __shared__ uint4 s_lrow[HALF_XCHG_GROUPS];
+    __shared__ int s_rbox[2];
+    __shared__ HalfWbShared s_wb;
     const unsigned long long n_items = counters->n_alive;
+    const unsigned long long n_pulled = clones ? counters->ray_items_front : 0ull;
+    const unsigned long long n_clones = clones ? n_pulled + counters->ray_items_front_local : 0ull;
+    const unsigned long long n_work = 2ull * (n_items + n_clones);
     const int gw = (int)geom.gw, gh = (int)geom.gh;
     const uint32_t win_base = (uint32_t)__cvta_generic_to_shared(s_win);
     const int lane = threadIdx.x & 31, warp = threadIdx.x >> 5, n_warps = blockDim.x >> 5;
@@ -980,18 +1036,32 @@
         }
     };
     auto pop_next = [&]() {
-        const unsigned long long w = atomicAdd(&counters->ray_work_head, 1ull);
-        if (w < 2ull * n_items) {
+        unsigned long long w;
+        for (;;) {
+            w = atomicAdd(&counters->ray_work_head, 1ull);
+            if (w >= n_work) break;
+            const int pass = (w >> 1) < n_clones ? 0 : ((w >> 1) < 2ull * n_clones ? 1 : 2);
+            const unsigned long long k = (w >> 1) - (pass ? n_clones : 0ull);
             RayItem nit;
-            if (clones) nit = ray_item_at(clones, owners, n_local, counters, w >> 1);
-            else { nit.particle = alive_list[w >> 1]; nit.slot = slot_of[nit.particle]; nit.root = nit.slot; nit.old_y0 = nit.old_y1 = 0; nit.pad = 0u; }
+            if (clones) nit = ray_item_at(clones, owners, n_local, counters, k);
+            else { nit.particle = alive_list[k]; nit.slot = slot_of[nit.particle]; nit.root = nit.slot; nit.old_y0 = nit.old_y1 = 0; nit.pad = 0u; }
+            if (pass < 2 && (k < n_pulled || owned[nit.root] != 0u) != (pass == 0)) continue;
             const ParticleResult r = results[first_particle + nit.particle];
+            const SlotMeta rm = meta[nit.root];
             s_item = nit;
             s_pose[0] = r.x; s_pose[1] = r.y; s_pose[2] = r.theta;
+            const bool box = rm.x1 > rm.x0 && rm.y1 > rm.y0;
+            s_rbox[0] = box ? rm.y0 : 0x7fffffff; s_rbox[1] = box ? rm.y1 - 1 : -1;
+            s_item_pos = k;
+            break;
         }
         s_next = w;
     };
     if (threadIdx.x == 0) pop_next();
+    {
+        uint4* w4 = reinterpret_cast<uint4*>(s_win);
+        for (int i = threadIdx.x; i < (int)(window_bytes >> 4); i += blockDim.x) w4[i] = make_uint4(0u, 0u, 0u, 0u);
+    }
 #ifdef SLAMRS_RAY_TRACE
     long long t_prev = clock64();
 #endif
@@ -999,12 +1069,21 @@
     for (;;) {
         __syncthreads();
         const unsigned long long work = s_next;
-        if (work >= 2ull * n_items) break;
+        if (work >= n_work) break;
         RAY_STAMP(0);
+        const unsigned long long item = s_item_pos;
         RAY_LOG(work, 0);
-        const unsigned long long item = work >> 1;
         const bool upper = (work & 1ull) != 0ull;
         const RayItem it = s_item;
+#ifdef SLAMRS_RAY_CHECK_WINDOW
+        {
+            const uint4* w4 = reinterpret_cast<const uint4*>(s_win);
+            for (int i = threadIdx.x; i < (int)(window_bytes >> 4); i += blockDim.x) {
+                const uint4 g = w4[i];
+                assert((g.x | g.y | g.z | g.w) == 0u);
+            }
+        }
+#endif
         const bool fused = it.root != it.slot;
         uint32_t* grid = cells + (size_t)it.slot * cells_per_grid;
         uint32_t* bands = bands_all + (size_t)it.slot * n_bands_slot;
@@ -1035,6 +1114,17 @@
         const int wy0 = upper ? cy0 : max(0, cy0 - rad), wy1 = upper ? min(gh, cy0 + rad + 1) : cy0 + 1;
         const int band0 = wy0 / BAND_ROWS;
         const int wh = walked ? wy1 - wy0 : 0;
+        {
+            const int2 yr = half_wb_rows(s_rbox, it, fused, wy0, wy0 + wh - 1, upper ? cy0 : 0, upper ? gh : cy0);
+            const int pf0 = yr.x / BAND_ROWS, npf = yr.y >= yr.x ? min(HALF_WB_BANDS, yr.y / BAND_ROWS - pf0 + 1) : 0;
+            if ((int)threadIdx.x < npf) {
+                const uint32_t* src_bands = bands_all + (size_t)it.root * n_bands_slot;
+                const uint32_t dst = (uint32_t)__cvta_generic_to_shared(&s_wb.e[threadIdx.x]);
+                asm volatile("cp.async.ca.shared.global [%0], [%1], 4;" ::"r"(dst), "l"(src_bands + pf0 + threadIdx.x) : "memory");
+                if (fused) asm volatile("cp.async.ca.shared.global [%0], [%1], 4;" ::"r"(dst + 4u), "l"(bands + pf0 + threadIdx.x) : "memory");
+            }
+            if (threadIdx.x == 0) { s_wb.pf0 = pf0; s_wb.npf = npf; s_wb.rbox[0] = s_rbox[0]; s_wb.rbox[1] = s_rbox[1]; }
+        }
         for (int ly = threadIdx.x; ly < wh; ly += blockDim.x) {
             const int dy = wy0 + ly - cy0;
             const int hw = isqrt_small(rad * rad - dy * dy);
@@ -1043,10 +1133,6 @@
             s_row[ly].y = x0 | ((x1 - x0) << 16);
         }
         __syncthreads();
-        if (threadIdx.x >= 32) {
-            uint4* w4 = reinterpret_cast<uint4*>(s_win);
-            for (int i = threadIdx.x - 32; i < (int)(window_bytes >> 4); i += blockDim.x - 32) w4[i] = make_uint4(0u, 0u, 0u, 0u);
-        }
         if (threadIdx.x < 32) {
             int carry = 0;
             for (int base = 0; base < wh; base += 32) {
@@ -1117,11 +1203,12 @@
 #ifdef SLAMRS_RAY_TRACE
         if (threadIdx.x == 0) atomicAdd(&g_ray_trace[12], (unsigned long long)(clock64() - t_prev));
 #endif
+        asm volatile("cp.async.wait_all;" ::: "memory");
         __syncthreads();
         RAY_STAMP(3);
         RAY_LOG(work, 3);
 
-        const uint4* win4 = reinterpret_cast<const uint4*>(s_win);
+        uint4* win4 = reinterpret_cast<uint4*>(s_win);
         {
             const int rr = lane & 7, bq = lane >> 3;
             int wxmin = 0x7fffffff, wymin = 0x7fffffff, wxmax = -1, wymax = -1;
@@ -1166,8 +1253,11 @@
             HalfXchg* x = xchg + item;
             const int2 row = s_row[wh - 1];
             const int groups = row.y >> 19;
-            if (threadIdx.x < HALF_XCHG_GROUPS)
-                x->row[threadIdx.x] = (int)threadIdx.x < groups ? win4[(row.x >> 3) + threadIdx.x] : make_uint4(0u, 0u, 0u, 0u);
+            if (threadIdx.x < HALF_XCHG_GROUPS) {
+                uint4 g = make_uint4(0u, 0u, 0u, 0u);
+                if ((int)threadIdx.x < groups) { g = win4[(row.x >> 3) + threadIdx.x]; win4[(row.x >> 3) + threadIdx.x] = make_uint4(0u, 0u, 0u, 0u); }
+                x->row[threadIdx.x] = g;
+            }
             if (threadIdx.x == 0) {
                 const int lb = shared_band - band0;
                 const bool any = shared_band >= 0 && (unsigned)lb < (unsigned)HALF_MAX_BANDS && s_bhi[lb] >= s_blo[lb];
@@ -1182,7 +1272,8 @@
                 }
                 if (nh > HALF_XCHG_HITS) atomicAdd(&counters->fuse_overflow, 1ull);
                 x->n_hits = min(nh, HALF_XCHG_HITS);
-                s_eo_shared = (fused && shared_band >= 0) ? bands[shared_band] : 0u;
+                const int pi = shared_band - s_wb.pf0;
+                s_eo_shared = (fused && shared_band >= 0) ? ((unsigned)pi < (unsigned)s_wb.npf ? s_wb.e[pi].y : bands[shared_band]) : 0u;
             }
             __threadfence();
             __syncthreads();
@@ -1248,8 +1339,8 @@
         }
         RAY_STAMP(6);
         RAY_LOG(work, 6);
-        ray_half_writeback(geom, it, upper, cy0, walked, cells, meta, bands_all, cells_per_grid, s_win, s_row, s_blo, s_bhi, s_ext,
-                           s_lrow, s_xinfo, s_eo_shared, wy0, wh, band0, &saturated, &moved);
+        ray_half_writeback(geom, it, upper, cy0, cells, bands_all, cells_per_grid, s_win, s_row, s_blo, s_bhi, s_ext, s_lrow, s_xinfo,
+                           s_wb, s_eo_shared, wy0, wh, band0, &saturated, &moved);
 #ifdef SLAMRS_RAY_TRACE
         if (threadIdx.x == 0) atomicAdd(&g_ray_trace[13], (unsigned long long)(clock64() - t_prev));
 #endif
@@ -1380,7 +1471,8 @@
                               const RayItem* clones, const RayItem* owners, const uint32_t* readers, uint32_t* done,
                               uint32_t* xflag, void* xchg, uint32_t* spill_scratch, const int32_t* slot_of, uint32_t* cells,
                               SlotMeta* meta, uint32_t* bands, size_t cells_per_grid, int radius_cells, StepCounters* counters,
-                              uint64_t* window_cells, bool force_generic, int num_sms, uint32_t* xdone, uint32_t signal_epoch) {
+                              uint64_t* window_cells, bool force_generic, int num_sms, uint32_t* xdone, const uint32_t* owned,
+                              uint32_t signal_epoch) {
     if (ray_update_can_fuse(geom, scan.n_beams, cells_per_grid, force_generic, radius_cells)) {
         const int radius = ray_packed_radius(radius_cells);
         const size_t wcells = (size_t)ray_window_cells_upper_bound_half(radius);
@@ -1398,7 +1490,8 @@
         if (grid > 2u * n_local) grid = 2u * n_local;
         k_ray_update_half<<<grid, threads, smem, stream>>>(geom, scan, results, first_particle, alive_list, clones, owners, readers, done,
                                                            xflag, (HalfXchg*)xchg, spill_scratch, slot_of, cells, meta, bands,
-                                                           cells_per_grid, radius, (uint32_t)wbytes, counters, xdone, n_local, signal_epoch);
+                                                           cells_per_grid, radius, (uint32_t)wbytes, counters, xdone, owned, n_local,
+                                                           signal_epoch);
 #ifdef SLAMRS_RAY_TRACE
         ray_log_dump_after_launch(stream);
 #endif
diff --git a/slamrs_b200/csrc/kernels_resample.cu b/slamrs_b200/csrc/kernels_resample.cu
--- a/slamrs_b200/csrc/kernels_resample.cu
+++ b/slamrs_b200/csrc/kernels_resample.cu
@@ -689,6 +689,7 @@
     if (alive && clone && !remote) ray.clones[ray.n_local - 1u - (bcl + __popc(mcl & below))] = it;
     if (alive && !clone && remote) ray.owners[bor + __popc(mor & below)] = it;
     if (alive && !clone && !remote) ray.owners[ray.n_local - 1u - (bol + __popc(mol & below))] = it;
+    if (alive && !clone) ray.owned[it.slot] = 1u;
 }
 
 void launch_resample_indices(cudaStream_t stream, const ParticleResult* results, const double* cum,
```
